# andreaskoepf/faster-rcnn.torch

Measured on AMD Instinct MI355X. Metric: images/sec (vgg_small 800x450 fwd+bwd), higher is better.
Workload: dtype f32 (conv / Linear(13824,1024) operands as 2 x fp16 split planes: 22 significand bits, 3 MFMA partial products; fp32 accumulate)

## Files before the change

faster-rcnn.torch_amd/_lib.py:

```python
import ctypes as C
import os

_HERE = os.path.dirname(os.path.abspath(__file__))
SO_PATH = os.environ.get("FRCNN_LIB_PATH") or os.path.join(_HERE, "libfrcnn_hip.so")

KC_NAMES = ["conv_igemm_k3", "conv_igemm_other", "conv_wgrad_k3", "conv_wgrad_other", "gemm", "elemwise",
            "roi", "rpn", "nms", "optim", "image", "conv_x3", "conv_wgradx", "soft_nms", "topk"]


class FrcnnError(RuntimeError):
    pass


class ModelDesc(C.Structure):
    _fields_ = [
        ("nblocks", C.c_int),
        ("filters", C.c_int * 8), ("ksize", C.c_int * 8), ("pad", C.c_int * 8), ("conv_steps", C.c_int * 8),
        ("dropout", C.c_float * 8),
        ("nheads", C.c_int),
        ("head_k", C.c_int * 8), ("head_n", C.c_int * 8), ("head_input", C.c_int * 8),
        ("ncls", C.c_int),
        ("cls_n", C.c_int * 8), ("cls_bn", C.c_int * 8),
        ("cls_dropout", C.c_float * 8),
        ("class_count", C.c_int),
        ("kh", C.c_int), ("kw", C.c_int),
    ]


vp = C.c_void_p
_SIGS = {
    "frcnn_version": ([], C.c_int),
    "frcnn_set_option": ([C.c_char_p, C.c_int], C.c_int),
    "frcnn_get_option": ([C.c_char_p, C.POINTER(C.c_int)], C.c_int),
    "frcnn_last_error": ([], C.c_char_p),
    "frcnn_device_count": ([C.POINTER(C.c_int)], C.c_int),
    "frcnn_set_device": ([C.c_int], C.c_int),
    "frcnn_device_name": ([C.c_char_p, C.c_int], C.c_int),
    "frcnn_malloc": ([C.POINTER(vp), C.c_size_t], C.c_int),
    "frcnn_free": ([vp], C.c_int),
    "frcnn_host_alloc": ([C.POINTER(vp), C.c_size_t], C.c_int),
    "frcnn_host_free": ([vp], C.c_int),
    "frcnn_memcpy_h2d": ([vp, vp, C.c_size_t, vp], C.c_int),
    "frcnn_memcpy_d2h": ([vp, vp, C.c_size_t, vp], C.c_int),
    "frcnn_memcpy_d2d": ([vp, vp, C.c_size_t, vp], C.c_int),
    "frcnn_stream_sync": ([vp], C.c_int),
    "frcnn_zero": ([vp, C.c_size_t, vp], C.c_int),
    "frcnn_scale": ([vp, C.c_longlong, C.c_float, vp], C.c_int),
    "frcnn_add": ([vp, vp, C.c_longlong, vp], C.c_int),
    "frcnn_prof_enable": ([C.c_int], C.c_int),
    "frcnn_prof_collect": ([vp, vp, vp, vp], C.c_int),
    "frcnn_nms_workspace_bytes": ([C.c_int], C.c_size_t),
    "frcnn_nms_device": ([vp, C.c_int, C.c_int, C.c_float, C.c_int, C.c_int, vp, vp, vp, C.c_size_t, vp], C.c_int),
    "frcnn_nms_device_classes": ([vp, C.c_int, C.c_int, C.c_float, C.c_int, C.c_int, vp, vp, vp, vp, C.c_size_t, vp], C.c_int),
    "frcnn_nms_device_n": ([vp, C.c_int, vp, C.c_int, C.c_float, C.c_int, C.c_int, vp, vp, vp, vp, C.c_size_t, vp], C.c_int),
    "frcnn_nms_batch_workspace_bytes": ([C.c_int, C.c_int], C.c_size_t),
    "frcnn_nms_device_batch": ([vp, C.c_int, C.c_longlong, C.c_int, vp, C.c_int, C.c_float, C.c_int, C.c_int, vp, vp, vp, vp, C.c_size_t,
                               vp], C.c_int),
    "frcnn_soft_nms_workspace_bytes": ([C.c_int, C.c_int], C.c_size_t),
    "frcnn_soft_nms_batch": ([vp, C.c_int, C.c_longlong, C.c_int, vp, C.c_int, C.c_int, C.c_int, C.c_float, C.c_float, C.c_float, C.c_int,
                             vp, vp, vp, vp, C.c_longlong, vp, C.c_size_t, vp], C.c_int),
    "frcnn_box_vote_batch": ([vp, C.c_int, C.c_longlong, C.c_int, vp, C.c_int, C.c_int, C.c_int, C.c_float, vp, vp, vp, vp, vp, vp, vp],
                             C.c_int),
    "frcnn_topk_select_workspace_bytes": ([C.c_int, C.c_int], C.c_size_t),
    "frcnn_topk_select": ([vp, C.c_int, C.c_longlong, C.c_int, vp, C.c_int, vp, C.c_longlong, vp, vp, C.c_size_t, vp], C.c_int),
    "frcnn_rpn_gather_rows": ([vp, vp, vp, vp, C.c_int, C.c_longlong, C.c_int, vp, C.c_longlong, vp, C.c_int, vp, vp, vp, vp, vp, vp,
                              C.c_longlong, vp], C.c_int),
    "frcnn_detect_gather_batch": ([vp, vp, C.c_int, C.c_int, vp, vp, vp, vp, vp, C.c_longlong, vp, vp, vp, vp, vp], C.c_int),
    "frcnn_roi_windows": ([vp, vp, C.c_int, vp, C.c_int, C.c_int, C.c_int, vp, vp], C.c_int),
    "frcnn_detect_post": ([vp, vp, vp, vp, vp, C.c_int, C.c_int, C.c_double, vp, vp, vp, vp, vp, vp], C.c_int),
    "frcnn_detect_classes_batch": ([vp, vp, vp, vp, C.c_int, vp, vp, C.c_longlong, C.c_int, C.c_int, C.c_double, C.c_int, vp, vp, vp, vp,
                                    C.c_int, vp, vp, vp], C.c_int),
    "frcnn_detect_merge_views": ([vp, vp, vp, vp, C.c_longlong, vp, vp, C.c_longlong, C.c_int, C.c_int, vp, vp, vp, vp, vp, vp, vp, vp, vp,
                                  vp, vp, vp], C.c_int),
    "frcnn_nms_host": ([vp, C.c_int, C.c_int, C.c_float, C.c_int, C.c_int, vp, vp], C.c_int),
    "frcnn_conv2d_forward": ([vp, C.c_int, C.c_int, C.c_int, vp, vp, vp, vp, C.c_int, C.c_int, C.c_int, vp, vp], C.c_int),
    "frcnn_conv2d_backward_input": ([vp, C.c_int, C.c_int, C.c_int, vp, C.c_int, C.c_int, C.c_int, vp, C.c_int, vp], C.c_int),
    "frcnn_conv2d_backward_weight": ([vp, C.c_int, C.c_int, C.c_int, vp, vp, vp, C.c_int, C.c_int, C.c_int, vp, vp, vp], C.c_int),
    "frcnn_maxpool_act_forward": ([vp, C.c_int, C.c_int, C.c_int, vp, vp, vp, vp, vp], C.c_int),
    "frcnn_maxpool_act_backward": ([vp, vp, vp, C.c_int, C.c_int, C.c_int, vp, vp, vp, vp, vp, vp], C.c_int),
    "frcnn_act_forward": ([vp, C.c_int, C.c_longlong, vp, vp, vp, vp], C.c_int),
    "frcnn_act_backward": ([vp, vp, C.c_int, C.c_longlong, vp, vp, vp, vp, vp, vp], C.c_int),
    "frcnn_amax_record_floats": ([], C.c_int),
    "frcnn_tensor_absmax": ([vp, C.c_longlong, vp, vp], C.c_int),
    "frcnn_maxpool_act_forward_rec": ([vp, C.c_int, C.c_int, C.c_int, vp, vp, vp, vp, vp, vp], C.c_int),
    "frcnn_maxpool_act_backward_rec": ([vp, vp, vp, C.c_int, C.c_int, C.c_int, vp, vp, vp, vp, vp, vp, vp], C.c_int),
    "frcnn_act_backward_rec": ([vp, vp, C.c_int, C.c_longlong, vp, vp, vp, vp, vp, vp, vp], C.c_int),
    "frcnn_conv2d_forward_rec": ([vp, C.c_int, C.c_int, C.c_int, vp, vp, vp, vp, C.c_int, C.c_int, C.c_int, vp, vp, vp, vp], C.c_int),
    "frcnn_conv2d_backward_input_rec": ([vp, C.c_int, C.c_int, C.c_int, vp, C.c_int, C.c_int, C.c_int, vp, C.c_int, vp, vp, vp, vp, vp, vp,
                                         vp], C.c_int),
    "frcnn_roi_pool_forward": ([vp, C.c_int, C.c_int, C.c_int, vp, C.c_int, C.c_int, C.c_int, vp, vp, vp], C.c_int),
    "frcnn_roi_pool_backward": ([vp, C.c_int, C.c_int, C.c_int, vp, vp, C.c_int, C.c_int, C.c_int, vp], C.c_int),
    "frcnn_roi_align_forward": ([vp, C.c_int, C.c_int, C.c_int, vp, vp, C.c_int, C.c_double, C.c_double, C.c_int, C.c_int, C.c_int, vp,
                                 vp], C.c_int),
    "frcnn_roi_align_backward": ([vp, C.c_int, C.c_int, C.c_int, vp, vp, vp, C.c_int, C.c_double, C.c_double, C.c_int, C.c_int, C.c_int,
                                  vp], C.c_int),
    "frcnn_rpn_scan_workspace_bytes": ([vp, vp], C.c_size_t),
    "frcnn_rpn_scan": ([vp, vp, vp, vp, vp, C.c_double, C.c_double, C.c_double, C.c_int, vp, vp, vp, vp, vp, vp, C.c_size_t, vp], C.c_int),
    "frcnn_rpn_scan_batch_workspace_bytes": ([vp, vp, C.c_int], C.c_size_t),
    "frcnn_rpn_scan_batch": ([vp, vp, vp, C.c_int, C.c_longlong, vp, vp, C.c_double, C.c_double, C.c_double, C.c_int, vp, vp, vp, vp, vp,
                             vp, C.c_size_t, vp], C.c_int),
    "frcnn_rpn_scan_ragged_workspace_bytes": ([vp, vp, C.c_int], C.c_size_t),
    "frcnn_rpn_scan_ragged": ([vp, vp, vp, vp, vp, C.c_int, vp, vp, C.c_double, C.c_int, vp, vp, vp, vp, vp, vp, C.c_size_t, vp],
                              C.c_int),
    "frcnn_rpn_loss": ([vp, vp, vp, vp, vp, vp, vp, vp, C.c_int, C.c_int, C.c_int, vp, vp, vp, vp], C.c_int),
    "frcnn_loss_accumulate": ([vp, C.c_int, vp, vp], C.c_int),
    "frcnn_linear_forward": ([vp, C.c_int, C.c_int, vp, vp, C.c_int, vp, vp], C.c_int),
    "frcnn_linear_backward": ([vp, vp, C.c_int, C.c_int, vp, C.c_int, vp, vp, vp, vp], C.c_int),
    "frcnn_rmsprop": ([vp, vp, vp, C.c_longlong, C.c_float, C.c_float, C.c_float, vp], C.c_int),
    "frcnn_scale_rmsprop": ([vp, vp, C.c_float, vp, C.c_longlong, C.c_float, C.c_float, C.c_float, vp], C.c_int),
    "frcnn_scale_rmsprop_dev": ([vp, vp, vp, vp, C.c_longlong, C.c_float, C.c_float, C.c_float, vp], C.c_int),
    "frcnn_scale_rmsprop_slice": ([vp, vp, C.c_float, vp, C.c_longlong, C.c_longlong, C.c_float, C.c_float, C.c_float, vp], C.c_int),
    "frcnn_sgd": ([vp, vp, vp, C.c_longlong, C.c_float, vp, C.c_float, C.c_float, C.c_float, C.c_float, C.c_int, C.c_int, vp], C.c_int),
    "frcnn_sgd_slice": ([vp, vp, vp, C.c_longlong, C.c_longlong, C.c_float, C.c_float, C.c_float, C.c_float, C.c_float, C.c_int, C.c_int,
                         vp], C.c_int),
    "frcnn_nag": ([vp, vp, vp, C.c_longlong, C.c_float, vp, C.c_float, C.c_float, C.c_float, C.c_int, vp], C.c_int),
    "frcnn_nag_slice": ([vp, vp, vp, C.c_longlong, C.c_longlong, C.c_float, C.c_float, C.c_float, C.c_float, C.c_int, vp], C.c_int),
    "frcnn_scale_rmsprop_slice_dev": ([vp, vp, vp, vp, C.c_longlong, C.c_longlong, C.c_float, C.c_float, C.c_float, vp], C.c_int),
    "frcnn_sgd_slice_dev": ([vp, vp, vp, C.c_longlong, C.c_longlong, vp, C.c_float, C.c_float, C.c_float, C.c_float, C.c_int, C.c_int,
                            vp], C.c_int),
    "frcnn_nag_slice_dev": ([vp, vp, vp, C.c_longlong, C.c_longlong, vp, C.c_float, C.c_float, C.c_float, C.c_int, vp], C.c_int),
    "frcnn_grad_clip_workspace_bytes": ([C.c_longlong], C.c_size_t),
    "frcnn_grad_clip": ([vp, C.c_longlong, vp, C.c_int, C.c_double, vp, C.c_double, vp, vp, C.c_size_t, vp], C.c_int),
    "frcnn_nag_lookahead": ([vp, vp, C.c_longlong, C.c_float, vp], C.c_int),
    "frcnn_nag_lookahead_slice": ([vp, vp, C.c_longlong, C.c_longlong, C.c_float, vp], C.c_int),
    "frcnn_model_update_stream": ([vp, C.POINTER(vp)], C.c_int),
    "frcnn_model_update_fork": ([vp, vp], C.c_int),
    "frcnn_model_update_join": ([vp, vp], C.c_int),
    "frcnn_pnet_wait_backward_begun": ([vp, vp], C.c_int),
    "frcnn_pnet_wait_heads_done": ([vp, vp], C.c_int),
    "frcnn_pnet_wait_block_done": ([vp, C.c_int, vp], C.c_int),
    "frcnn_pnet_refresh_packs": ([vp, vp, C.c_int, vp], C.c_int),
    "frcnn_pnet_invalidate_packs": ([vp], C.c_int),
    "frcnn_model_create": ([C.POINTER(ModelDesc), C.POINTER(vp)], C.c_int),
    "frcnn_model_destroy": ([vp], C.c_int),
    "frcnn_model_param_count": ([vp, C.POINTER(C.c_longlong), C.POINTER(C.c_longlong)], C.c_int),
    "frcnn_model_param_table": ([vp, vp, C.c_int, C.POINTER(C.c_int)], C.c_int),
    "frcnn_model_localizer_layers": ([vp, C.c_int, vp, C.c_int, C.POINTER(C.c_int)], C.c_int),
    "frcnn_model_set_trainable": ([vp, C.c_int, C.c_int, C.c_int], C.c_int),
    "frcnn_model_get_trainable": ([vp, C.POINTER(C.c_int), C.POINTER(C.c_int), C.POINTER(C.c_int)], C.c_int),
    "frcnn_model_debug_buffer": ([vp, C.c_int, C.c_int, C.POINTER(vp), C.POINTER(C.c_longlong)], C.c_int),
    "frcnn_pnet_forward": ([vp, vp, vp, C.c_int, C.c_int, C.c_int, vp, C.c_ulonglong, vp], C.c_int),
    "frcnn_pnet_forward_async_heads": ([vp, vp, vp, C.c_int, C.c_int, vp, C.c_ulonglong, vp], C.c_int),
    "frcnn_pnet_output": ([vp, C.c_int, C.POINTER(vp), C.POINTER(C.c_int), C.POINTER(C.c_int), C.POINTER(C.c_int)], C.c_int),
    "frcnn_pnet_delta": ([vp, C.c_int, C.POINTER(vp)], C.c_int),
    "frcnn_pnet_set_sparse_deltas": ([vp, C.c_int, vp, C.c_int], C.c_int),
    "frcnn_pnet_zero_deltas": ([vp, vp], C.c_int),
    "frcnn_pnet_backward_heads_begin": ([vp, vp, vp, vp], C.c_int),
    "frcnn_pnet_anchor_loss_begin": ([vp, vp, vp, vp, vp, vp, vp, C.c_int, C.c_int, C.c_int, vp, vp, vp, vp, vp], C.c_int),
    "frcnn_pnet_anchor_loss_wait": ([vp, vp], C.c_int),
    "frcnn_pnet_backward_heads_join": ([vp, vp, C.POINTER(C.c_int)], C.c_int),
    "frcnn_pnet_backward": ([vp, vp, vp, vp], C.c_int),
    "frcnn_pnet_wait_block_gradients": ([vp, C.c_int, vp], C.c_int),
    "frcnn_cnet_forward": ([vp, vp, vp, C.c_int, C.c_int, vp, C.c_ulonglong, vp, vp, vp, vp], C.c_int),
    "frcnn_cnet_backward": ([vp, vp, vp, vp, vp, vp, vp], C.c_int),
    "frcnn_cnet_backward_join": ([vp, vp], C.c_int),
    "frcnn_cnet_losses": ([vp, vp, vp, vp, C.c_int, C.c_int, C.c_int, vp, vp, vp, vp], C.c_int),
    "frcnn_cnet_decode": ([vp, C.c_int, C.c_int, vp, vp, vp], C.c_int),
    "frcnn_anchors_create": ([vp, vp, vp, vp, C.c_int, C.c_int, C.POINTER(vp)], C.c_int),
    "frcnn_anchors_destroy": ([vp], C.c_int),
    "frcnn_anchors_assemble": ([vp, vp, C.c_int, C.c_double, C.c_double, C.c_double, C.c_double, C.c_int, C.c_int, C.c_int, vp,
                               C.POINTER(C.c_int), vp, vp, C.c_int, C.POINTER(C.c_int), C.POINTER(C.c_int)], C.c_int),
    "frcnn_comm_get_unique_id": ([vp], C.c_int),
    "frcnn_comm_exchange_id_file": ([C.c_char_p, C.c_int, vp, C.c_int], C.c_int),
    "frcnn_comm_init_rank": ([C.POINTER(vp), C.c_int, C.c_int, vp], C.c_int),
    "frcnn_comm_init_rank_timeout": ([C.POINTER(vp), C.c_int, C.c_int, vp, C.c_int], C.c_int),
    "frcnn_comm_init_rank_file": ([C.POINTER(vp), C.c_int, C.c_int, C.c_char_p, C.c_int], C.c_int),
    "frcnn_comm_destroy": ([vp], C.c_int),
    "frcnn_comm_info": ([vp, C.POINTER(C.c_int), C.POINTER(C.c_int)], C.c_int),
    "frcnn_comm_query": ([vp, C.POINTER(C.c_int), C.POINTER(C.c_int), C.POINTER(C.c_int)], C.c_int),
    "frcnn_allreduce_f32": ([vp, vp, C.c_longlong, vp], C.c_int),
    "frcnn_allreduce_f64": ([vp, vp, C.c_longlong, vp], C.c_int),
    "frcnn_broadcast_f32": ([vp, vp, C.c_longlong, C.c_int, vp], C.c_int),
    "frcnn_image_rgb2yuv": ([vp, vp, C.c_int, C.c_int, vp], C.c_int),
# ... 46 lines not shown
```

faster-rcnn.torch_amd/csrc/amax.h:

```cpp
#pragma once
#include <hip/hip_runtime.h>

#include "kernels.h"

namespace frcnn {

__device__ __forceinline__ void amax_store_block(float m, float* rec) {
  __shared__ float amax_part[16];
#pragma unroll
  for (int o = 32; o > 0; o >>= 1) m = fmaxf(m, __shfl_xor(m, o));
  if ((threadIdx.x & 63) == 0) amax_part[threadIdx.x >> 6] = m;
  __syncthreads();
  if (threadIdx.x == 0) {
    const int nw = (blockDim.x + 63) >> 6;
    for (int i = 1; i < nw; ++i) m = fmaxf(m, amax_part[i]);
    rec[1 + blockIdx.x] = m;
    if (blockIdx.x == 0) rec[0] = __builtin_bit_cast(float, (int)gridDim.x);
  }
}

__device__ __forceinline__ float amax_load_block(const float* __restrict__ rec) {
  __shared__ float amax_all[16];
  const int n = __builtin_bit_cast(int, rec[0]);
  float m = 0.f;
  for (int i = threadIdx.x; i < n; i += blockDim.x) m = fmaxf(m, rec[1 + i]);
#pragma unroll
  for (int o = 32; o > 0; o >>= 1) m = fmaxf(m, __shfl_xor(m, o));
  if ((threadIdx.x & 63) == 0) amax_all[threadIdx.x >> 6] = m;
  __syncthreads();
  const int nw = (blockDim.x + 63) >> 6;
  m = amax_all[0];
  for (int i = 1; i < nw; ++i) m = fmaxf(m, amax_all[i]);
  __syncthreads();
  return m;
}

}
```

faster-rcnn.torch_amd/csrc/api.cpp:

```cpp
#include <cmath>
#include <cstring>
#include <vector>
#include <mutex>

#include "kernels.h"

namespace frcnn {

static thread_local std::string g_err;

void set_error(const char* fmt, ...) {
  char buf[1024];
  va_list ap;
  va_start(ap, fmt);
  vsnprintf(buf, sizeof(buf), fmt, ap);
  va_end(ap);
  g_err = buf;
}

struct ProfRec { int klass; double flops, bytes; hipEvent_t a, b; hipStream_t s; };
static hipEvent_t g_prof_base = nullptr;
static unsigned g_prof_mask = 0;
static std::vector<ProfRec> g_recs;
static std::vector<hipEvent_t> g_pool;
// ... 297 lines not shown
  return tensor_absmax(x, (long)n, rec, S(stream));
}
int frcnn_conv2d_forward_rec(const float* in, int C, int H, int W, const float* in_slope, const float* in_scale, const float* weight,
                             const float* bias, int O, int k, int pad, float* out, const float* rec_in, float* rec_out, void* stream) {
  FR_CHECK(in && weight && out, "frcnn_conv2d_forward_rec: NULL argument");
  FR_CHECK(conv_x3_eligible(C, O, k) && (k == 3 || (!in_slope && !in_scale)),
           "frcnn_conv2d_forward_rec: %d channels -> %d filters, %dx%d does not take the split form", C, O, k, k);
  FR_CHECK(get_x3_f16(), "frcnn_conv2d_forward_rec: option x3_f16 is off");
  bool unit = true;
  FR_TRY(scale_fits_f16_form(in_scale, C, S(stream), &unit));
  FR_CHECK(unit, "frcnn_conv2d_forward_rec: an entry of in_scale exceeds 1: the launch would not take the fp16 form");
  return conv2d_split(in, C, H, W, in_slope, in_scale, weight, bias, O, C, O, k, 0, pad, out, OUT_STORE, true, rec_in, rec_out, nullptr,
                      S(stream));
}
int frcnn_conv2d_backward_input_rec(const float* gout, int O, int Ho, int Wo, const float* weight, int C, int k, int pad, float* gin,
                                    int accumulate, const float* rec_g, float* rec_out, const float* post_x, const float* post_slope,
                                    const float* post_scale, float* gslope, void* stream) {
  FR_CHECK(gout && weight && gin, "frcnn_conv2d_backward_input_rec: NULL argument");
  FR_CHECK(conv_x3_eligible(O, C, k), "frcnn_conv2d_backward_input_rec: %d filters -> %d channels, %dx%d does not take the split form",
           O, C, k, k);
  FR_CHECK(get_x3_f16(), "frcnn_conv2d_backward_input_rec: option x3_f16 is off");
  FR_CHECK(post_x || (!post_slope && !post_scale && !gslope), "frcnn_conv2d_backward_input_rec: a fused activation backward needs post_x");
  FR_CHECK(!post_x || (post_slope && k == 3 && !accumulate),
           "frcnn_conv2d_backward_input_rec: the fused activation backward belongs to a storing 3x3 launch with a slope");
  const X3PostAct post{post_x, post_slope, post_scale, gslope};
  return conv2d_split(gout, O, Ho, Wo, nullptr, nullptr, weight, nullptr, O, C, C, k, 1, k - 1 - pad, gin, accumulate ? OUT_ADD : OUT_STORE,
                      true, rec_g, rec_out, post_x ? &post : nullptr, S(stream));
}
int frcnn_conv2d_backward_weight(const float* in, int C, int H, int W, const float* in_slope,
                                 const float* in_scale, const float* gout, int O, int k, int pad,
                                 float* gweight, float* gbias, void* stream) {
  size_t wsb = conv_wgrad_workspace_bytes(C, H, W, O, k, pad);
  void* ws = nullptr;
  FR_HIP(hipMalloc(&ws, wsb));
  int rc = FRCNN_OK;
  float* am = nullptr;
  bool unit = true;
  rc = scale_fits_f16_form(in_scale, C, S(stream), &unit);
  if (rc == FRCNN_OK && unit && k == 3 && conv_wgradx_eligible(C, O, k)) rc = x3_f16_records(&am);
  if (am && rc == FRCNN_OK) {
    rc = tensor_absmax(in, (long)C * H * W, am, S(stream));
    if (rc == FRCNN_OK) rc = tensor_absmax(gout, (long)O * (H + 2 * pad - k + 1) * (W + 2 * pad - k + 1), am + AMAX_REC, S(stream));
  }
  if (rc == FRCNN_OK)
    rc = conv_wgrad(in, C, H, W, in_slope, in_scale, gout, O, k, pad, gweight, ws, wsb, S(stream), gbias, am, am ? am + AMAX_REC : nullptr);
  (void)hipStreamSynchronize(S(stream));
  (void)hipFree(ws); (void)hipFree(am);
  return rc;
}

int frcnn_maxpool_act_forward(const float* x, int C, int H, int W, const float* slope, const float* scale,
                              float* out, unsigned char* idx, void* stream) {
  return maxpool_act_forward(x, C, H, W, slope, scale, out, idx, S(stream));
}
int frcnn_maxpool_act_backward(const float* gpool, const unsigned char* idx, const float* x, int C, int H, int W,
                               const float* slope, const float* scale, float* gx, float* gbias, float* gslope,
                               void* stream) {
  return maxpool_act_backward(gpool, idx, x, C, H, W, slope, scale, gx, gbias, gslope, S(stream));
}
int frcnn_maxpool_act_forward_rec(const float* x, int C, int H, int W, const float* slope, const float* scale, float* out,
                                  unsigned char* idx, void* stream, float* rec) {
  return maxpool_act_forward(x, C, H, W, slope, scale, out, idx, S(stream), rec);
}
int frcnn_maxpool_act_backward_rec(const float* gpool, const unsigned char* idx, const float* x, int C, int H, int W, const float* slope,
                                   const float* scale, float* gx, float* gbias, float* gslope, void* stream, float* rec) {
  return maxpool_act_backward(gpool, idx, x, C, H, W, slope, scale, gx, gbias, gslope, S(stream), rec);
}
int frcnn_act_backward_rec(const float* gy, const float* x, int C, long long hw, const float* slope, const float* scale, float* gx,
                           float* gbias, float* gslope, void* stream, float* rec) {
  return act_backward(gy, x, C, hw, slope, scale, gx, gbias, gslope, S(stream), rec);
}
int frcnn_act_forward(const float* x, int C, long long hw, const float* slope, const float* scale, float* y,
                      void* stream) {
  return act_forward(x, C, hw, slope, scale, y, S(stream));
}
int frcnn_act_backward(const float* gy, const float* x, int C, long long hw, const float* slope,
                       const float* scale, float* gx, float* gbias, float* gslope, void* stream) {
  return act_backward(gy, x, C, hw, slope, scale, gx, gbias, gslope, S(stream));
}

int frcnn_roi_pool_forward(const float* fmap, int C, int H, int W, const int* wins, int R, int kh, int kw,
                           float* out, int* idx, void* stream) {
  return roi_pool_forward(fmap, C, H, W, wins, R, kh, kw, out, idx, S(stream));
}
int frcnn_roi_pool_backward(float* gmap, int C, int H, int W, const float* gout, const int* idx, int R, int kh,
                            int kw, void* stream) {
  return roi_pool_backward(gmap, C, H, W, gout, idx, R, kh, kw, S(stream));
}

static int roi_align_check(const char* who, const void* map, int C, int H, int W, const void* rows, const double* rect, int kh, int kw,
                           int g) {
  FR_CHECK(map && rows && rect, "%s: NULL argument", who);
  FR_CHECK(C >= 1 && H >= 1 && W >= 1 && kh >= 1 && kw >= 1, "%s: map %d x %d x %d, grid %d x %d", who, C, H, W, kh, kw);
  FR_CHECK((long)H * W < (1L << 31), "%s: a plane of %d x %d cells", who, H, W);
  FR_CHECK(g >= 1 && g <= 4, "%s: sampling ratio %d outside 1..4", who, g);
  return FRCNN_OK;
}
int frcnn_roi_align_forward(const float* fmap, int C, int H, int W, const double* rect, const long long* pick, int R, double inv_sx,
                            double inv_sy, int kh, int kw, int g, float* out, void* stream) {
  if (R <= 0) return FRCNN_OK;
  FR_TRY(roi_align_check("frcnn_roi_align_forward", fmap, C, H, W, out, rect, kh, kw, g));
  return roi_align_forward(fmap, C, H, W, rect, pick, R, inv_sx, inv_sy, kh, kw, g, out, S(stream));
}
int frcnn_roi_align_backward(float* gmap, int C, int H, int W, const float* gout, const double* rect, const long long* pick, int R,
                             double inv_sx, double inv_sy, int kh, int kw, int g, void* stream) {
  if (R <= 0) return FRCNN_OK;
  FR_TRY(roi_align_check("frcnn_roi_align_backward", gmap, C, H, W, gout, rect, kh, kw, g));
  return roi_align_backward(gmap, C, H, W, gout, rect, pick, R, inv_sx, inv_sy, kh, kw, g, S(stream));
}

static void to_layers(const float* const* maps, const int* H, const int* W, RpnLayers* L) {
  for (int l = 0; l < 4; ++l) { L->map[l] = maps ? maps[l] : nullptr; L->H[l] = H[l]; L->W[l] = W[l]; }
}
size_t frcnn_rpn_scan_workspace_bytes(const int* H, const int* W) {
  RpnLayers L;
  to_layers(nullptr, H, W, &L);
  return rpn_scan_workspace_bytes(L);
}
int frcnn_rpn_scan(const float* const* maps, const int* H, const int* W, const float* anchor_w,
                   const float* anchor_h, double img_w, double img_h, double p_threshold, int cap,
                   float* match_p, int* match_idx, double* match_rect, float* match_box, int* count,
                   void* ws, size_t ws_bytes, void* stream) {
  RpnLayers L;
  to_layers(maps, H, W, &L);
  return rpn_scan(L, anchor_w, anchor_h, img_w, img_h, p_threshold, cap, match_p, match_idx, match_rect,
                  match_box, count, ws, ws_bytes, S(stream));
}
size_t frcnn_rpn_scan_batch_workspace_bytes(const int* H, const int* W, int B) {
  RpnLayers L;
  to_layers(nullptr, H, W, &L);
  return rpn_scan_batch_workspace_bytes(L, B);
}
int frcnn_rpn_scan_batch(const float* const* maps, const int* H, const int* W, int B, long long slot_stride, const float* anchor_w,
                         const float* anchor_h, double img_w, double img_h, double p_threshold, int cap, float* match_p,
                         int* match_idx, double* match_rect, float* match_box, int* count, void* ws, size_t ws_bytes,
                         void* stream) {
  FR_CHECK(maps && H && W, "frcnn_rpn_scan_batch: NULL argument");
  RpnLayers L;
  to_layers(maps, H, W, &L);
  return rpn_scan_batch(L, B, (long)slot_stride, anchor_w, anchor_h, img_w, img_h, p_threshold, cap, match_p, match_idx,
                        match_rect, match_box, count, ws, ws_bytes, S(stream));
}
size_t frcnn_rpn_scan_ragged_workspace_bytes(const int* Hs, const int* Ws, int B) {
  return rpn_scan_ragged_workspace_bytes(Hs, Ws, B);
}
int frcnn_rpn_scan_ragged(const float* heads, const long long* map_off, const int* Hs, const int* Ws, const double* img_wh, int B,
                          const float* anchor_w, const float* anchor_h, double p_threshold, int cap, float* match_p,
                          int* match_idx, double* match_rect, float* match_box, int* count, void* ws, size_t ws_bytes,
                          void* stream) {
  return rpn_scan_ragged(heads, map_off, Hs, Ws, img_wh, B, anchor_w, anchor_h, p_threshold, cap, match_p, match_idx, match_rect,
                         match_box, count, ws, ws_bytes, S(stream));
}
int frcnn_rpn_loss(const float* const* maps, float* const* deltas, const int* H, const int* W, const int* ex_idx,
                   const double* ex_anchor, const double* ex_roi, const int* ex_class, int npos, int nneg,
                   int bgclass, double* ex_loss, float* crtarget, float* cctarget, void* stream) {
  RpnLayers L;
  to_layers(maps, H, W, &L);
  return rpn_loss(L, deltas, ex_idx, ex_anchor, ex_roi, ex_class, npos, nneg, bgclass, ex_loss, crtarget,
                  cctarget, S(stream));
}

int frcnn_loss_accumulate(const double* ex_loss, int E, double* acc, void* stream) {
  return loss_accumulate(ex_loss, E, acc, S(stream));
}

int frcnn_linear_forward(const float* x, int R, int I, const float* weight, const float* bias, int O, float* y,
// ... 175 lines not shown
```

faster-rcnn.torch_amd/csrc/cnet.hip:

```cpp
#include "kernels.h"

namespace frcnn {

#define BN_EPS 1e-5
#define BN_MOM 0.1

#define BN_CB 16
#define BN_RG 64
template <int CB = BN_CB, int RG = BN_RG>
__device__ __forceinline__ double bn_reduce(double v, double* sh, int tx, int ty) {
  sh[ty * CB + tx] = v;
  __syncthreads();
  for (int stride = RG / 2; stride > 0; stride >>= 1) {
    if (ty < stride) sh[ty * CB + tx] += sh[(ty + stride) * CB + tx];
    __syncthreads();
  }
  const double s = sh[tx];
  __syncthreads();
  return s;
}
template <int NV>
__device__ __forceinline__ void fb_reduce(double (&v)[NV], double* sh, int tx, int ty) {
  const int tid = ty * 4 + tx, lane = tid & 63, wave = tid >> 6;
#pragma unroll
  for (int k = 0; k < NV; ++k) {
#pragma unroll
    for (int o = 4; o < 64; o <<= 1) v[k] += __shfl_xor(v[k], o, 64);
    if (lane < 4) sh[(k * 16 + wave) * 4 + lane] = v[k];
  }
  __syncthreads();
#pragma unroll
  for (int k = 0; k < NV; ++k) {
    double t = 0.0;
#pragma unroll
    for (int w = 0; w < 16; ++w) t += sh[(k * 16 + w) * 4 + tx];
    v[k] = t;
  }
  __syncthreads();
}
#define FB_CB 4
#define FB_RG 256
#define FB_KEEP 4

__global__ __launch_bounds__(1024) void bn_forward_kernel(const float* __restrict__ x, int R, int n,
                                                          const float* __restrict__ gamma, const float* __restrict__ beta,
                                                          float* running, int training, float* __restrict__ xhat,
                                                          float* __restrict__ invstd, float* __restrict__ y) {
  __shared__ double sh[BN_RG * BN_CB];
  const int tx = threadIdx.x, ty = threadIdx.y;
  const int j = blockIdx.x * BN_CB + tx;
  const bool ok = j < n;
  double mean, var;
  if (training) {
    double s = 0.0;
    if (ok) for (int r = ty; r < R; r += BN_RG) s += x[(size_t)r * n + j];
    mean = bn_reduce(s, sh, tx, ty) / R;
    double q = 0.0;
    if (ok) for (int r = ty; r < R; r += BN_RG) { double d = x[(size_t)r * n + j] - mean; q += d * d; }
    var = bn_reduce(q, sh, tx, ty);
    const double unb = R > 1 ? var / (R - 1) : var / R;
    var /= R;
    if (running && ok && ty == 0) {
      running[j] = (float)((1.0 - BN_MOM) * running[j] + BN_MOM * mean);
      running[n + j] = (float)((1.0 - BN_MOM) * running[n + j] + BN_MOM * unb);
    }
  } else {
    mean = ok ? running[j] : 0.0;
    var = ok ? running[n + j] : 1.0;
  }
  if (!ok) return;
  const double is = 1.0 / sqrt(var + BN_EPS);
  if (ty == 0) invstd[j] = (float)is;
  const double g = gamma[j], b = beta[j];
  for (int r = ty; r < R; r += BN_RG) {
    const double xh = (x[(size_t)r * n + j] - mean) * is;
    xhat[(size_t)r * n + j] = (float)xh;
    y[(size_t)r * n + j] = (float)(xh * g + b);
  }
}
int bn_forward(const float* x, int R, int n, const float* gamma, const float* beta, float* running,
               int training, float* xhat, float* invstd, float* y, hipStream_t s) {
  FR_CHECK(training || running, "bn_forward: evaluate mode needs running statistics");
  FR_LAUNCH(KC_ELEMWISE, 0, (double)R * n * 16.0, s, bn_forward_kernel, dim3(cdiv(n, BN_CB)), dim3(BN_CB, BN_RG), 0, x, R, n,
            gamma, beta, running, training, xhat, invstd, y);
  FR_LAUNCH_CHECK();
  return FRCNN_OK;
}

__global__ __launch_bounds__(1024) void bn_backward_kernel(const float* __restrict__ gy, const float* __restrict__ xhat,
                                                           const float* __restrict__ invstd, const float* __restrict__ gamma,
                                                           int R, int n, int training, float* __restrict__ gx, float* ggamma,
                                                           float* gbeta) {
  __shared__ double sh[BN_RG * BN_CB];
  const int tx = threadIdx.x, ty = threadIdx.y;
  const int j = blockIdx.x * BN_CB + tx;
  const bool ok = j < n;
  double sg = 0.0, sgx = 0.0;
  if (ok)
    for (int r = ty; r < R; r += BN_RG) {
      const double g = gy[(size_t)r * n + j];
      sg += g;
      sgx += g * xhat[(size_t)r * n + j];
    }
  sg = bn_reduce(sg, sh, tx, ty);
  sgx = bn_reduce(sgx, sh, tx, ty);
  if (!ok) return;
  if (ty == 0) {
    ggamma[j] = (float)((double)ggamma[j] + sgx);
    gbeta[j] = (float)((double)gbeta[j] + sg);
  }
  const double is = invstd[j], gm = gamma[j];
  for (int r = ty; r < R; r += BN_RG) {
    const double g = gy[(size_t)r * n + j];
    const double xh = xhat[(size_t)r * n + j];
    const double v = training ? (g - sg / R - xh * sgx / R) * gm * is : g * gm * is;
    gx[(size_t)r * n + j] = (float)v;
  }
}
int bn_backward(const float* gy, const float* xhat, const float* invstd, const float* gamma, int R,
                int n, int training, float* gx, float* ggamma, float* gbeta, hipStream_t s) {
  FR_LAUNCH(KC_ELEMWISE, 0, (double)R * n * 16.0, s, bn_backward_kernel, dim3(cdiv(n, BN_CB)), dim3(BN_CB, BN_RG), 0, gy,
            xhat, invstd, gamma, R, n, training, gx, ggamma, gbeta);
  FR_LAUNCH_CHECK();
  return FRCNN_OK;
}

__device__ __forceinline__ float fold_value(const float* __restrict__ x, const GemmFold& src, size_t total, size_t idx, int j) {
  if (src.nSplit == 0) return x[idx];
  float v = src.bias ? src.bias[j] : 0.f;
  for (int sI = 0; sI < src.nSplit; ++sI) v += src.slab[(size_t)sI * total + idx];
  return v;
}

template <bool GEN>
__global__ __launch_bounds__(1024) void cnet_act_forward_kernel(const float* __restrict__ x, GemmFold src, int R, int n,
                                                                const float* __restrict__ gamma, const float* __restrict__ beta,
                                                                float* running, int training, float* __restrict__ lin,
                                                                float* __restrict__ xhat, float* __restrict__ invstd,
                                                                float* __restrict__ pre, const float* slope, float* __restrict__ mask,
                                                                float inv_keep, float p, unsigned long long seed,
                                                                float* __restrict__ post) {
  __shared__ double sh[FB_RG * FB_CB];
  const int tx = threadIdx.x, ty = threadIdx.y;
  const int j = blockIdx.x * FB_CB + tx;
  const bool ok = j < n;
  const size_t total = (size_t)R * n;
  const bool bn = gamma != nullptr;
  const float* v = src.nSplit ? lin : x;
  const bool keep = R <= FB_RG * FB_KEEP;
  float xv[FB_KEEP];
  double s0 = 0.0;
  if (ok) {
#pragma unroll
    for (int i = 0; i < FB_KEEP; ++i) {
      const int r = ty + i * FB_RG;
      xv[i] = 0.f;
      if (keep && r < R) {
        const size_t idx = (size_t)r * n + j;
        xv[i] = fold_value(x, src, total, idx, j);
        if (src.nSplit) lin[idx] = xv[i];
        s0 += xv[i];
      }
    }
    if (!keep && (src.nSplit || (bn && training)))
      for (int r = ty; r < R; r += FB_RG) {
        const size_t idx = (size_t)r * n + j;
        const float t = fold_value(x, src, total, idx, j);
        if (src.nSplit) lin[idx] = t;
        s0 += t;
      }
  }
  double mean = 0.0, is = 1.0, g = 1.0, b = 0.0;
  if (bn) {
    double var;
    if (training) {
      { double t[1] = {s0}; fb_reduce(t, sh, tx, ty); mean = t[0] / R; }
      double q = 0.0;
      if (ok && keep) {
#pragma unroll
        for (int i = 0; i < FB_KEEP; ++i)
          if (ty + i * FB_RG < R) { double d = xv[i] - mean; q += d * d; }
      } else if (ok) {
        for (int r = ty; r < R; r += FB_RG) { double d = v[(size_t)r * n + j] - mean; q += d * d; }
      }
      { double t[1] = {q}; fb_reduce(t, sh, tx, ty); var = t[0]; }
      const double unb = R > 1 ? var / (R - 1) : var / R;
      var /= R;
      if (running && ok && ty == 0) {
        running[j] = (float)((1.0 - BN_MOM) * running[j] + BN_MOM * mean);
        running[n + j] = (float)((1.0 - BN_MOM) * running[n + j] + BN_MOM * unb);
      }
    } else {
      mean = ok ? running[j] : 0.0;
      var = ok ? running[n + j] : 1.0;
    }
    if (!ok) return;
    is = 1.0 / sqrt(var + BN_EPS);
    if (ty == 0) invstd[j] = (float)is;
    g = gamma[j]; b = beta[j];
  }
  if (!ok) return;
  const float a = *slope;
  auto emit = [&](size_t idx, float y) {
    if (bn) {
      const double xh = ((double)y - mean) * is;
      xhat[idx] = (float)xh;
      y = (float)(xh * g + b);
      pre[idx] = y;
    }
    y = y > 0.f ? y : a * y;
    if (GEN) {
      const float mk = frcnn_keep_mask(seed, (unsigned long long)idx, p);
      mask[idx] = mk;
      y = y * (mk * inv_keep);
    } else if (mask) {
      y = y * (mask[idx] * inv_keep);
    }
    post[idx] = y;
  };
  if (keep) {
#pragma unroll
    for (int i = 0; i < FB_KEEP; ++i)
      if (ty + i * FB_RG < R) emit((size_t)(ty + i * FB_RG) * n + j, xv[i]);
  } else {
    for (int r = ty; r < R; r += FB_RG) emit((size_t)r * n + j, v[(size_t)r * n + j]);
  }
}
template <bool GEN>
__global__ void cnet_act_forward_flat_kernel(const float* __restrict__ x, GemmFold src, long total, int n, float* __restrict__ lin,
                                             const float* slope, float* __restrict__ mask, float inv_keep, float p,
                                             unsigned long long seed, float* __restrict__ post) {
  const float a = *slope;
  for (long i = (long)blockIdx.x * blockDim.x + threadIdx.x; i < total; i += (long)gridDim.x * blockDim.x) {
    float y = fold_value(x, src, (size_t)total, (size_t)i, (int)(i % n));
    if (src.nSplit) lin[i] = y;
    y = y > 0.f ? y : a * y;
    if (GEN) {
      const float mk = frcnn_keep_mask(seed, (unsigned long long)i, p);
      mask[i] = mk;
      y = y * (mk * inv_keep);
    } else if (mask) {
      y = y * (mask[i] * inv_keep);
    }
    post[i] = y;
  }
}
int cnet_act_forward(const float* x, GemmFold src, int R, int n, const float* gamma, const float* beta, float* running,
                     int training, float* lin, float* xhat, float* invstd, float* pre, const float* slope, float* mask, bool gen,
                     float inv_keep, float p, unsigned long long seed, float* post, hipStream_t s) {
  FR_CHECK(!gamma || training || running, "cnet_act_forward: evaluate mode needs running statistics");
  if (!gamma) {
    const long total = (long)R * n;
    const int grid = (int)std::min<long>(std::max<long>(1, cdivl(total, 256)), 2048);
    if (gen)
      FR_LAUNCH(KC_ELEMWISE, 0, total * 16.0, s, cnet_act_forward_flat_kernel<true>, dim3(grid), dim3(256), 0, x, src, total, n, lin, slope,
                mask, inv_keep, p, seed, post);
    else
      FR_LAUNCH(KC_ELEMWISE, 0, total * 16.0, s, cnet_act_forward_flat_kernel<false>, dim3(grid), dim3(256), 0, x, src, total, n, lin, slope,
                mask, inv_keep, p, seed, post);
    FR_LAUNCH_CHECK();
    return FRCNN_OK;
  }
  if (gen)
    FR_LAUNCH(KC_ELEMWISE, 0, (double)R * n * 20.0, s, cnet_act_forward_kernel<true>, dim3(cdiv(n, FB_CB)), dim3(FB_CB, FB_RG), 0, x,
              src, R, n, gamma, beta, running, training, lin, xhat, invstd, pre, slope, mask, inv_keep, p, seed, post);
  else
    FR_LAUNCH(KC_ELEMWISE, 0, (double)R * n * 20.0, s, cnet_act_forward_kernel<false>, dim3(cdiv(n, FB_CB)), dim3(FB_CB, FB_RG), 0, x,
              src, R, n, gamma, beta, running, training, lin, xhat, invstd, pre, slope, mask, inv_keep, p, seed, post);
  FR_LAUNCH_CHECK();
  return FRCNN_OK;
}

__global__ __launch_bounds__(1024) void cnet_act_bn_backward_kernel(const float* __restrict__ gy, GemmFold src,
                                                                    const float* __restrict__ pre, const float* __restrict__ xhat,
                                                                    const float* __restrict__ invstd, const float* __restrict__ gamma,
                                                                    const float* slope, const float* __restrict__ mask, float inv_keep,
                                                                    int R, int n, int training, float* __restrict__ gx, float* ggamma,
                                                                    float* gbeta, float* gslope, float* part) {
  __shared__ double sh[FB_RG * FB_CB];
  __shared__ float shs[16];
  const int tx = threadIdx.x, ty = threadIdx.y;
  const int j = blockIdx.x * FB_CB + tx;
  const bool ok = j < n;
  const size_t total = (size_t)R * n;
  const float a = *slope;
  double sg = 0.0, sgx = 0.0;
  float sa = 0.f;
  const bool keep = R <= FB_RG * FB_KEEP;
  float tv[FB_KEEP], xh[FB_KEEP];
  auto first = [&](size_t idx, float& t, float& xhv) {
    float g = fold_value(gy, src, total, idx, j);
    if (mask) g = g * (mask[idx] * inv_keep);
    const float xv = pre[idx];
    t = g;
    if (!(xv > 0.f)) { t = a * g; sa += xv * g; }
    xhv = xhat[idx];
    sg += t;
    sgx += (double)t * xhv;
  };
  if (ok && keep) {
#pragma unroll
    for (int i = 0; i < FB_KEEP; ++i) {
      tv[i] = 0.f; xh[i] = 0.f;
      if (ty + i * FB_RG < R) first((size_t)(ty + i * FB_RG) * n + j, tv[i], xh[i]);
    }
  } else if (ok) {
    for (int r = ty; r < R; r += FB_RG) {
      const size_t idx = (size_t)r * n + j;
      float t, xhv;
      first(idx, t, xhv);
      gx[idx] = t;
    }
  }
  { double t[2] = {sg, sgx}; fb_reduce(t, sh, tx, ty); sg = t[0]; sgx = t[1]; }
  {
    const int tid = ty * FB_CB + tx;
#pragma unroll
    for (int o = 32; o > 0; o >>= 1) sa += __shfl_down(sa, o, 64);
    if ((tid & 63) == 0) shs[tid >> 6] = sa;
    __syncthreads();
    if (tid == 0) {
      float t = 0.f;
      for (int i = 0; i < 16; ++i) t += shs[i];
      if (part) part[blockIdx.x] = t; else unsafeAtomicAdd(gslope, t);
    }
  }
  if (!ok) return;
  if (ty == 0) {
    ggamma[j] = (float)((double)ggamma[j] + sgx);
    gbeta[j] = (float)((double)gbeta[j] + sg);
  }
  const double is = invstd[j], gm = gamma[j];
  auto second = [&](size_t idx, double g, double xhv) {
    const double v = training ? (g - sg / R - xhv * sgx / R) * gm * is : g * gm * is;
    gx[idx] = (float)v;
  };
  if (keep) {
#pragma unroll
    for (int i = 0; i < FB_KEEP; ++i)
      if (ty + i * FB_RG < R) second((size_t)(ty + i * FB_RG) * n + j, tv[i], xh[i]);
  } else {
    for (int r = ty; r < R; r += FB_RG) {
      const size_t idx = (size_t)r * n + j;
      second(idx, gx[idx], xhat[idx]);
    }
  }
}
__global__ void slope_fold_kernel(const float* __restrict__ part, int n, float* gslope);
int cnet_act_bn_backward(const float* gy, GemmFold src, const float* pre, const float* xhat, const float* invstd,
                         const float* gamma, const float* slope, const float* mask, float inv_keep, int R, int n, int training,
                         float* gx, float* ggamma, float* gbeta, float* gslope, hipStream_t s) {
  const int grid = cdiv(n, FB_CB);
  float* part = nullptr;
  if (deterministic()) FR_TRY(det_workspace(s, (size_t)grid, &part));
  FR_LAUNCH(KC_ELEMWISE, 0, (double)R * n * 28.0, s, cnet_act_bn_backward_kernel, dim3(grid), dim3(FB_CB, FB_RG), 0, gy, src, pre, xhat,
            invstd, gamma, slope, mask, inv_keep, R, n, training, gx, ggamma, gbeta, gslope, part);
  if (part) FR_LAUNCH(KC_ELEMWISE, 0, grid * 4.0, s, slope_fold_kernel, dim3(1), dim3(1), 0, (const float*)part, grid, gslope);
  FR_LAUNCH_CHECK();
  return FRCNN_OK;
}

template <bool GEN>
__global__ void prelu_dropout_forward_kernel(const float* __restrict__ x, long n, const float* slope,
                                             float* __restrict__ mask, float inv_keep, float p,
                                             unsigned long long seed, float* __restrict__ y) {
  const float a = *slope;
  for (long i = (long)blockIdx.x * blockDim.x + threadIdx.x; i < n; i += (long)gridDim.x * blockDim.x) {
    float v = x[i];
    v = v > 0.f ? v : a * v;
    if (GEN) {
      const float mk = frcnn_keep_mask(seed, (unsigned long long)i, p);
      mask[i] = mk;
      v = v * (mk * inv_keep);
    } else if (mask) {
      v = v * (mask[i] * inv_keep);
    }
    y[i] = v;
  }
}
int prelu_dropout_forward(const float* x, long n, const float* slope, const float* mask, float inv_keep,
                          float* y, hipStream_t s) {
  int grid = (int)std::min<long>(std::max<long>(1, cdivl(n, 256)), 1024);
  FR_LAUNCH(KC_ELEMWISE, 0, n * 12.0, s, prelu_dropout_forward_kernel<false>, dim3(grid), dim3(256), 0, x, n, slope,
            const_cast<float*>(mask), inv_keep, 0.f, 0ull, y);
  FR_LAUNCH_CHECK();
  return FRCNN_OK;
}
int prelu_dropout_forward_gen(const float* x, long n, const float* slope, float* mask_out, float p,
                              unsigned long long seed, float* y, hipStream_t s) {
  int grid = (int)std::min<long>(std::max<long>(1, cdivl(n, 256)), 1024);
  FR_LAUNCH(KC_ELEMWISE, 0, n * 12.0, s, prelu_dropout_forward_kernel<true>, dim3(grid), dim3(256), 0, x, n, slope,
            mask_out, 1.0f / (1.0f - p), p, seed, y);
  FR_LAUNCH_CHECK();
  return FRCNN_OK;
}

__global__ void prelu_dropout_backward_kernel(const float* __restrict__ gy, const float* __restrict__ x, long n,
                                              const float* slope, const float* __restrict__ mask,
                                              float inv_keep, float* __restrict__ gx, float* gslope, float* part) {
  __shared__ float sh[4];
  const float a = *slope;
  float sa = 0.f;
  for (long i = (long)blockIdx.x * blockDim.x + threadIdx.x; i < n; i += (long)gridDim.x * blockDim.x) {
    float g = gy[i];
    if (mask) g = g * (mask[i] * inv_keep);
    const float xv = x[i];
    float r = g;
    if (!(xv > 0.f)) { r = a * g; sa += xv * g; }
    gx[i] = r;
  }
#pragma unroll
  for (int o = 32; o > 0; o >>= 1) sa += __shfl_down(sa, o, 64);
  if ((threadIdx.x & 63) == 0) sh[threadIdx.x >> 6] = sa;
  __syncthreads();
  if (threadIdx.x == 0) {
    const float t = sh[0] + sh[1] + sh[2] + sh[3];
    if (part) part[blockIdx.x] = t;
    else unsafeAtomicAdd(gslope, t);
  }
}
__global__ void slope_fold_kernel(const float* __restrict__ part, int n, float* gslope) {
  float v = 0.f;
  for (int i = 0; i < n; ++i) v += part[i];
  *gslope += v;
}
int prelu_dropout_backward(const float* gy, const float* x, long n, const float* slope,
                           const float* mask, float inv_keep, float* gx, float* gslope, hipStream_t s) {
  int grid = (int)std::min<long>(std::max<long>(1, cdivl(n, 256)), 256);
  float* part = nullptr;
  if (deterministic()) FR_TRY(det_workspace(s, (size_t)grid, &part));
  FR_LAUNCH(KC_ELEMWISE, 0, n * 16.0, s, prelu_dropout_backward_kernel, dim3(grid), dim3(256), 0, gy, x, n,
            slope, mask, inv_keep, gx, gslope, part);
  if (part) FR_LAUNCH(KC_ELEMWISE, 0, grid * 4.0, s, slope_fold_kernel, dim3(1), dim3(1), 0, (const float*)part, grid, gslope);
  FR_LAUNCH_CHECK();
  return FRCNN_OK;
}

__device__ __forceinline__ double wave_sum_f64(double v) {
#pragma unroll
  for (int o = 32; o > 0; o >>= 1) v += __shfl_xor(v, o, 64);
  return v;
}
__device__ __forceinline__ double wave_max_f64(double v) {
#pragma unroll
  for (int o = 32; o > 0; o >>= 1) { const double w = __shfl_xor(v, o, 64); v = w > v ? w : v; }
  return v;
}
__global__ void log_softmax_rows_fold_kernel(float* __restrict__ x, GemmFold src, int R, int n, float* __restrict__ y,
                                             float* __restrict__ y2) {
  const int r = blockIdx.x * (blockDim.x >> 6) + (threadIdx.x >> 6), lane = threadIdx.x & 63;
  if (r >= R) return;
  float* xr = x + (size_t)r * n;
  const size_t total = (size_t)R * n;
  if (src.nSplit)
    for (int i = lane; i < n; i += 64) xr[i] = fold_value(x, src, total, (size_t)r * n + i, i);
  double m = -1.0e300;
  for (int i = lane; i < n; i += 64) m = xr[i] > m ? (double)xr[i] : m;
  m = wave_max_f64(m);
  double s = 0.0;
  for (int i = lane; i < n; i += 64) s += exp((double)xr[i] - m);
  s = wave_sum_f64(s);
  const double lse = m + log(s);
  for (int i = lane; i < n; i += 64) {
    const float v = (float)((double)xr[i] - lse);
    y[(size_t)r * n + i] = v;
    if (y2) y2[(size_t)r * n + i] = v;
  }
}
int log_softmax_rows_fold(const float* x, GemmFold src, int R, int n, float* y, float* y2, hipStream_t s) {
  if (R <= 0) return FRCNN_OK;
  FR_LAUNCH(KC_ELEMWISE, 0, (double)R * n * 8.0, s, log_softmax_rows_fold_kernel, dim3(cdiv(R, 4)), dim3(256), 0, const_cast<float*>(x),
            src, R, n, y, y2);
  FR_LAUNCH_CHECK();
  return FRCNN_OK;
}

__global__ void log_softmax_rows_kernel(const float* __restrict__ x, int R, int n, float* __restrict__ y) {
  const int r = blockIdx.x * (blockDim.x >> 6) + (threadIdx.x >> 6), lane = threadIdx.x & 63;
  if (r >= R) return;
  const float* xr = x + (size_t)r * n;
  double m = -1.0e300;
  for (int i = lane; i < n; i += 64) m = xr[i] > m ? (double)xr[i] : m;
  m = wave_max_f64(m);
  double s = 0.0;
  for (int i = lane; i < n; i += 64) s += exp((double)xr[i] - m);
  s = wave_sum_f64(s);
  const double lse = m + log(s);
  for (int i = lane; i < n; i += 64) y[(size_t)r * n + i] = (float)((double)xr[i] - lse);
}
int log_softmax_rows(const float* x, int R, int n, float* y, hipStream_t s) {
  if (R <= 0) return FRCNN_OK;
  FR_LAUNCH(KC_ELEMWISE, 0, (double)R * n * 8.0, s, log_softmax_rows_kernel, dim3(cdiv(R, 4)), dim3(256), 0, x, R,
            n, y);
  FR_LAUNCH_CHECK();
  return FRCNN_OK;
}

#define HEADS_PITCH 33
__global__ __launch_bounds__(256) void cnet_heads_forward_kernel(const float* __restrict__ x, int R, int nf, const float* __restrict__ Wb,
                                                                 const float* __restrict__ bb, const float* __restrict__ Wc,
                                                                 const float* __restrict__ bc, int nc, float* __restrict__ bbox_out,
                                                                 float* __restrict__ logits, float* __restrict__ lsm,
                                                                 float* __restrict__ cls_out) {
  extern __shared__ float wt[];
  float* xs = wt + (size_t)nf * HEADS_PITCH + (threadIdx.x >> 6) * nf;
  const int no = 4 + nc;
  for (int k = threadIdx.x; k < nf; k += 256) {
    float* d = wt + k * HEADS_PITCH;
#pragma unroll
    for (int n = 0; n < 4; ++n) d[n] = Wb[(size_t)n * nf + k];
#pragma unroll 8
    for (int n = 0; n < nc; ++n) d[4 + n] = Wc[(size_t)n * nf + k];
  }
  __syncthreads();
  const int lane = threadIdx.x & 63, n = lane & 31, h = lane >> 5;
  const bool isb = n < 4, isc = n >= 4 && n < no;
  const int nn = n < no ? n : 0, kh = nf / 2;
  for (int r = blockIdx.x * 4 + (threadIdx.x >> 6); r < R; r += gridDim.x * 4) {
    for (int k = lane * 4; k < nf; k += 256) *reinterpret_cast<float4*>(xs + k) = *reinterpret_cast<const float4*>(x + (size_t)r * nf + k);
    __builtin_amdgcn_wave_barrier();
    const float* xr = xs + h * kh;
    const float* wk = wt + (size_t)(h * kh) * HEADS_PITCH + nn;
    float a0 = 0.f, a1 = 0.f, a2 = 0.f, a3 = 0.f;
#pragma unroll 4
    for (int k = 0; k < kh; k += 4) {
      const float4 xv = *reinterpret_cast<const float4*>(xr + k);
      a0 = fmaf(xv.x, wk[(k + 0) * HEADS_PITCH], a0); a1 = fmaf(xv.y, wk[(k + 1) * HEADS_PITCH], a1);
      a2 = fmaf(xv.z, wk[(k + 2) * HEADS_PITCH], a2); a3 = fmaf(xv.w, wk[(k + 3) * HEADS_PITCH], a3);
    }
    float v = (a0 + a1) + (a2 + a3);
    v += __shfl_xor(v, 32, 64);
    v += isb ? bb[n] : isc ? bc[n - 4] : 0.f;
    if (isb && h == 0) bbox_out[(size_t)r * 4 + n] = v;
    const bool mine = isc && h == 0;
    double m = mine ? (double)v : -1.0e300;
    m = wave_max_f64(m);
    double e = mine ? exp((double)v - m) : 0.0;
    e = wave_sum_f64(e);
    const double lse = m + log(e);
    if (mine) {
      const size_t o = (size_t)r * nc + n - 4;
      const float l = (float)((double)v - lse);
      logits[o] = v; lsm[o] = l;
      if (cls_out) cls_out[o] = l;
    }
  }
}
__global__ __launch_bounds__(256) void cnet_heads_backward_kernel(const float* __restrict__ g_bbox, const float* __restrict__ g_cls,
                                                                  const float* __restrict__ lsm, int R, int nf,
                                                                  const float* __restrict__ Wb, const float* __restrict__ Wc, int nc,
                                                                  float* __restrict__ glog, float* __restrict__ gfeat, HeadsPostAct post) {
  extern __shared__ float wt[];
  __shared__ float shs[4];
  const float pa = post.pre ? *post.slope : 1.f;
  float sa = 0.f;
  const int no = 4 + nc;
  for (int k = threadIdx.x; k < nf; k += 256) {
#pragma unroll
    for (int n = 0; n < 4; ++n) wt[n * nf + k] = Wb[(size_t)n * nf + k];
#pragma unroll 8
    for (int n = 0; n < nc; ++n) wt[(4 + n) * nf + k] = Wc[(size_t)n * nf + k];
  }
  __syncthreads();
  const int lane = threadIdx.x & 63, wave = threadIdx.x >> 6;
  float* sg = wt + (size_t)no * nf + wave * 64;
  const bool isb = lane < 4, isc = lane >= 4 && lane < no;
  for (int r = blockIdx.x * 4 + wave; r < R; r += gridDim.x * 4) {
    const size_t o = (size_t)r * nc + (isc ? lane - 4 : 0);
    const double gy = isc ? (double)g_cls[o] : 0.0;
    const double sum = wave_sum_f64(gy);
    float g = 0.f;
    if (isc) {
      g = (float)(gy - exp((double)lsm[o]) * sum);
      glog[o] = g;
    } else if (isb) {
      g = g_bbox[(size_t)r * 4 + lane];
    }
    sg[lane] = g;
    __builtin_amdgcn_wave_barrier();
    for (int k = lane; k < nf; k += 64) {
      float a0 = 0.f, a1 = 0.f;
      int n = 0;
      for (; n + 2 <= no; n += 2) {
        a0 = fmaf(sg[n], wt[n * nf + k], a0);
        a1 = fmaf(sg[n + 1], wt[(n + 1) * nf + k], a1);
      }
      if (n < no) a0 = fmaf(sg[n], wt[n * nf + k], a0);
      float g = a0 + a1;
      if (post.pre) {
        const size_t idx = (size_t)r * nf + k;
        if (post.mask) g = g * (post.mask[idx] * post.inv_keep);
        const float xv = post.pre[idx];
        if (!(xv > 0.f)) { sa += xv * g; g = pa * g; }
      }
      gfeat[(size_t)r * nf + k] = g;
    }
    __builtin_amdgcn_wave_barrier();
  }
  if (post.pre) {
#pragma unroll
    for (int o = 32; o > 0; o >>= 1) sa += __shfl_down(sa, o, 64);
    if (lane == 0) shs[wave] = sa;
    __syncthreads();
    if (threadIdx.x == 0) unsafeAtomicAdd(post.gslope, (shs[0] + shs[1]) + (shs[2] + shs[3]));
  }
}
bool cnet_heads_fused_eligible(int nf, int nc) { return 4 + nc <= 32 && nf % 8 == 0 && nf <= 1024; }
int cnet_heads_forward(const float* x, int R, int nf, const float* Wb, const float* bb, const float* Wc, const float* bc, int nc,
                       float* bbox_out, float* logits, float* lsm, float* cls_out, hipStream_t s) {
  if (R <= 0) return FRCNN_OK;
  FR_CHECK(cnet_heads_fused_eligible(nf, nc), "cnet_heads_forward: %d classes", nc);
  FR_CHECK(((uintptr_t)x & 15) == 0, "cnet_heads_forward: input alignment");
  const size_t lds = ((size_t)nf * HEADS_PITCH + 4 * (size_t)nf) * 4;
  static bool attr_set = false;
  if (!attr_set) {
    FR_HIP(hipFuncSetAttribute(reinterpret_cast<const void*>(cnet_heads_forward_kernel), hipFuncAttributeMaxDynamicSharedMemorySize, 160 * 1024));
    attr_set = true;
  }
  FR_LAUNCH(KC_ELEMWISE, 0, (double)R * nf * 4.0, s, cnet_heads_forward_kernel, dim3(std::min(cdiv(R, 4), 256)), dim3(256), lds, x, R, nf, Wb,
            bb, Wc, bc, nc, bbox_out, logits, lsm, cls_out);
  FR_LAUNCH_CHECK();
  return FRCNN_OK;
}
int cnet_heads_backward(const float* g_bbox, const float* g_cls, const float* lsm, int R, int nf, const float* Wb, const float* Wc,
                        int nc, float* glog, float* gfeat, hipStream_t s, const HeadsPostAct* post) {
  if (R <= 0) return FRCNN_OK;
  FR_CHECK(cnet_heads_fused_eligible(nf, nc), "cnet_heads_backward: %d classes", nc);
  const size_t lds = ((size_t)(4 + nc) * nf + 256) * 4;
  static size_t attr_lds = 0;
  if (lds > attr_lds) {
    FR_HIP(hipFuncSetAttribute(reinterpret_cast<const void*>(cnet_heads_backward_kernel), hipFuncAttributeMaxDynamicSharedMemorySize, (int)lds));
    attr_lds = lds;
  }
  FR_LAUNCH(KC_ELEMWISE, 0, (double)R * nf * 4.0, s, cnet_heads_backward_kernel, dim3(std::min(cdiv(R, 4), 256)), dim3(256), lds, g_bbox, g_cls,
            lsm, R, nf, Wb, Wc, nc, glog, gfeat, post ? *post : HeadsPostAct{});
  FR_LAUNCH_CHECK();
  return FRCNN_OK;
}

__global__ void log_softmax_backward_kernel(const float* __restrict__ gy, const float* __restrict__ lsm, int R,
                                            int n, float* __restrict__ gx) {
  const int r = blockIdx.x * (blockDim.x >> 6) + (threadIdx.x >> 6), lane = threadIdx.x & 63;
  if (r >= R) return;
  double sum = 0.0;
  for (int i = lane; i < n; i += 64) sum += gy[(size_t)r * n + i];
  sum = wave_sum_f64(sum);
  for (int i = lane; i < n; i += 64)
    gx[(size_t)r * n + i] = (float)((double)gy[(size_t)r * n + i] - exp((double)lsm[(size_t)r * n + i]) * sum);
}
int log_softmax_backward(const float* gy, const float* lsm, int R, int n, float* gx, hipStream_t s) {
  if (R <= 0) return FRCNN_OK;
  FR_LAUNCH(KC_ELEMWISE, 0, (double)R * n * 12.0, s, log_softmax_backward_kernel, dim3(cdiv(R, 4)), dim3(256), 0,
            gy, lsm, R, n, gx);
  FR_LAUNCH_CHECK();
  return FRCNN_OK;
}

__global__ void cnet_losses_kernel(float* __restrict__ crout, const float* __restrict__ crtarget,
                                   const float* __restrict__ ccout, const float* __restrict__ cctarget, int R,
                                   int npos, int ncls, float* __restrict__ crdelta, float* __restrict__ ccdelta,
                                   double* loss2) {
  __shared__ double shr[256], shc[256];
  double sr = 0.0, sc = 0.0;
  for (int i = threadIdx.x; i < R * 4; i += blockDim.x) {
    float v = crout[i];
    if (i >= npos * 4) { v = 0.f; crout[i] = 0.f; }
    const float z = v - crtarget[i];
    const float az = fabsf(z);
    sr += az < 1.0f ? 0.5 * (double)z * (double)z : (double)az - 0.5;
    crdelta[i] = (az < 1.0f ? z : (z > 0.f ? 1.0f : -1.0f)) * 10.0f;
  }
  for (int i = threadIdx.x; i < R * ncls; i += blockDim.x) ccdelta[i] = 0.f;
  __syncthreads();
  for (int r = threadIdx.x; r < R; r += blockDim.x) {
    const int t = (int)cctarget[r] - 1;
    sc -= (double)ccout[(size_t)r * ncls + t];
    ccdelta[(size_t)r * ncls + t] = (float)(-1.0 / R);
  }
  shr[threadIdx.x] = sr;
  shc[threadIdx.x] = sc;
  __syncthreads();
  for (int o = 128; o > 0; o >>= 1) {
    if (threadIdx.x < o) { shr[threadIdx.x] += shr[threadIdx.x + o]; shc[threadIdx.x] += shc[threadIdx.x + o]; }
    __syncthreads();
  }
  if (threadIdx.x == 0) {
    loss2[0] += (double)(float)shr[0] * 10.0;
    loss2[1] += (double)(float)(shc[0] / R);
  }
}
int cnet_losses(float* crout, const float* crtarget, const float* ccout, const float* cctarget, int R,
                int npos, int ncls, float* crdelta, float* ccdelta, double* loss2, hipStream_t s) {
  if (R <= 0) return FRCNN_OK;
  FR_LAUNCH(KC_ELEMWISE, 0, (double)R * (ncls + 8) * 8.0, s, cnet_losses_kernel, dim3(1), dim3(256), 0, crout,
            crtarget, ccout, cctarget, R, npos, ncls, crdelta, ccdelta, loss2);
  FR_LAUNCH_CHECK();
  return FRCNN_OK;
}

__global__ void cnet_decode_kernel(const float* __restrict__ lsm, int R, int ncls, int* __restrict__ cls,
                                   float* __restrict__ conf) {
  const int r = blockIdx.x * blockDim.x + threadIdx.x;
  if (r >= R) return;
  int best = 0;
  for (int j = 1; j < ncls; ++j)
    if (lsm[(size_t)r * ncls + j] > lsm[(size_t)r * ncls + best]) best = j;
  cls[r] = best + 1;
  conf[r] = lsm[(size_t)r * ncls + best];
}
int cnet_decode(const float* cls_lsm, int R, int ncls, int* cls_out, float* conf_out, hipStream_t s) {
  if (R <= 0) return FRCNN_OK;
  FR_LAUNCH(KC_ELEMWISE, 0, (double)R * ncls * 4.0, s, cnet_decode_kernel, dim3(cdiv(R, 64)), dim3(64), 0,
            cls_lsm, R, ncls, cls_out, conf_out);
  FR_LAUNCH_CHECK();
  return FRCNN_OK;
}

}
// ... 1 lines not shown
```

faster-rcnn.torch_amd/csrc/kernels.h:

```cpp
#pragma once
#include <algorithm>

#include "common.h"

namespace frcnn {

int conv_cc(int k);
int conv_mpad(int M);
size_t conv_pack_floats(int Kchan, int M, int k);
int conv_pack_weights(const float* w, int O, int C, int k, float* wf, float* wd, hipStream_t s);
struct PackJob { long w_off; long total; float* dst; int O, C, k, mode, Mpad, blk_begin, nblk; };
PackJob conv_pack_job(long w_off, int O, int C, int k, int mode, float* dst);
int conv_pack_assign_blocks(PackJob* jobs, int njobs, int total_blocks);
int conv_pack_weights_multi(const float* weights, const PackJob* jobs_dev, int njobs, int grid, hipStream_t s);

enum { OUT_STORE = 0, OUT_ADD = 1 };
struct IgemmPool { float* out; unsigned char* idx; const float* slope; const float* scale; float* amax = nullptr; };
int conv_igemm(const float* in, int Cin, int H, int W, const float* in_slope, const float* in_scale,
               const float* wp, const float* bias, int M, int k, int pad, float* out, int out_mode,
               double algo_flops, hipStream_t s, int ws_slot = 0,
               const IgemmPool* pool = nullptr, bool* pool_fused = nullptr);

void set_split_bf16(int on);
int get_split_bf16();
// ... 61 lines not shown
int maxpool_act_forward(const float* x, int C, int H, int W, const float* slope, const float* scale,
                        float* out, unsigned char* idx, hipStream_t s, float* amax = nullptr);
int maxpool_act_backward(const float* gpool, const unsigned char* idx, const float* x, int C, int H,
                         int W, const float* slope, const float* scale, float* gx, float* gbias,
                         float* gslope, hipStream_t s, float* amax = nullptr);
int act_backward(const float* gy, const float* x, int C, long hw, const float* slope,
                 const float* scale, float* gx, float* gbias, float* gslope, hipStream_t s, float* amax = nullptr);
int channel_sum(const float* g, int C, long hw, float* gbias, hipStream_t s);
int channel_sum_cols(const float* g, int R, int O, float* gb, hipStream_t s);
int gather_positions(const float* src, int C, long hw, const int* pos, int P, float* dst, const float* slope,
                     float* dst_act, hipStream_t s);
int im2col_positions(const float* X, int C, int H, int W, int k, int Wo, const int* pos, int P, float* col, hipStream_t s);
int col2im_positions_add(const float* col, int C, int H, int W, int k, int Wo, const int* pos, int P, float* gX,
                         hipStream_t s);
int dropout_channel_mask(float* scale, int C, float p, unsigned long long seed, hipStream_t s);
int fill_value(float* x, long n, float v, hipStream_t s);
int rmsprop_update(float* x, float* g, float* m, long lo, long hi, bool slice, float gscale, const double* gcount_dev, float lr,
                   float alpha, float eps, hipStream_t s);
int sgd_update(float* x, float* g, float* v, long lo, long hi, bool slice, float gscale, const double* gcount_dev, float clr,
               float wd, float mom, float one_minus_damp, bool nesterov, bool first, hipStream_t s);
int nag_update(float* x, float* g, float* v, long lo, long hi, bool slice, float gscale, const double* gcount_dev, float clr,
               float wd, float mom, bool first, hipStream_t s);
int nag_lookahead(float* x, const float* v, long n, float mom, hipStream_t s);
constexpr int GRAD_CLIP_MAX_RANGES = 16;
size_t grad_clip_workspace_bytes(long n);
int grad_clip(float* g, long n, const long long* ranges_host, int nranges, double divisor, const double* divisor_dev, double clip_norm,
              double* record, void* workspace, size_t workspace_bytes, hipStream_t s);
int nag_lookahead_slice(float* x, const float* v, long lo, long hi, float mom, hipStream_t s);

#define FRCNN_HEAD_OUT 18
struct HeadJob {
  int Cin, H, W, k, Ho, Wo, n;
  int P; const int* pos;
  const float* in; float* gin;
  const float *bias3, *slope, *bias1;
  float *gbias3, *gslope, *gbias1;
  float* out; const float* delta;
  float *COL, *HX, *HY, *OUT, *D, *GH, *DX;
  const float* hx_slab; int hx_splits;
};
struct HeadJobs { HeadJob j[4]; int n; };
int heads_im2col(const HeadJobs& g, hipStream_t s);
int heads_bias_act(const HeadJobs& g, hipStream_t s);
int heads_scatter(const HeadJobs& g, hipStream_t s);
int heads_gather_delta(const HeadJobs& g, hipStream_t s);
int heads_act_backward(const HeadJobs& g, hipStream_t s);
int heads_col2im(const HeadJobs& g, hipStream_t s);

struct GemmFold;
#define GEMM_GROUP_MAX 4
struct GemmJob {
  const float* A; long sAm, sAk; const float* B; long sBk, sBn; float* C; long ldc;
  int M, N, K, out_mode;
  int splits = 1;
  int kPerSplit = 0;
};
int gemm_f32_group(GemmJob* jobs, int n, hipStream_t s);
int gemm_f32(const float* A, long sAm, long sAk, const float* B, long sBk, long sBn, float* C,
             long ldc, int M, int N, int K, int out_mode, const float* bias_n, hipStream_t s, int ws_slot = 0,
             GemmFold* defer = nullptr);
int gemm_workspace_get(size_t need, float** out, int slot);
struct GemmFold {
  const float* slab = nullptr;
  int nSplit = 0;
  const float* bias = nullptr;
};
int gemm_reduce_slabs(const float* slab, int nSplit, int M, int N, const float* bias, float* C, long ldc, bool accumulate,
                      hipStream_t s);
void set_gemm_x_roles(int mask);
int get_gemm_x_roles();
bool linear_x_eligible(int role, int R, int I, int O);
int linear_x_rows_padded(int R);
int split_planes(const float* src, int R, int C, void* P , void* PT ,
                 hipStream_t s, const float* amax = nullptr);
int linear_x_forward(const void* Xp, int R, int I, const float* W, const float* bias, int O, float* y, hipStream_t s, int ws_slot = 0,
                     GemmFold* defer = nullptr, const float* amax_x = nullptr, const float* amax_w = nullptr);
int linear_x_dgrad(const void* Gp, int R, int O, const float* W, int I, float* gx, int out_mode, hipStream_t s, int ws_slot = 0,
                   GemmFold* defer = nullptr, const float* amax_g = nullptr, const float* amax_w = nullptr);
int linear_x_wgrad(const void* GpT, const void* XpT, int R, int O, int I, float* gw, hipStream_t s, int ws_slot = 0,
                   const float* amax_g = nullptr, const float* amax_x = nullptr);


int roi_pool_forward(const float* fmap, int C, int H, int W, const int* wins, int R, int kh, int kw,
                     float* out, int* idx, hipStream_t s);
int roi_pool_backward(float* gmap, int C, int H, int W, const float* gout, const int* idx, int R,
                      int kh, int kw, hipStream_t s);

int roi_align_forward(const float* fmap, int C, int H, int W, const double* rect, const long long* pick, int R, double inv_sx,
                      double inv_sy, int kh, int kw, int g, float* out, hipStream_t s);
int roi_align_backward(float* gmap, int C, int H, int W, const float* gout, const double* rect, const long long* pick, int R,
                       double inv_sx, double inv_sy, int kh, int kw, int g, hipStream_t s);

struct RpnLayers {
  const float* map[4];
  int H[4], W[4];
};
int rpn_scan_batch(const RpnLayers& L, int B, long slot_stride, const float* anchor_w, const float* anchor_h, double img_w,
                   double img_h, double p_threshold, int cap, float* match_p, int* match_idx, double* match_rect,
                   float* match_box, int* count, void* ws, size_t ws_bytes, hipStream_t s);
size_t rpn_scan_batch_workspace_bytes(const RpnLayers& L, int B);
int rpn_scan(const RpnLayers& L, const float* anchor_w, const float* anchor_h, double img_w,
             double img_h, double p_threshold, int cap, float* match_p, int* match_idx,
             double* match_rect, float* match_box, int* count, void* ws, size_t ws_bytes,
             hipStream_t s);
size_t rpn_scan_workspace_bytes(const RpnLayers& L);
int rpn_scan_ragged(const float* heads, const long long* map_off, const int* Hs, const int* Ws, const double* img_wh, int B,
                    const float* anchor_w, const float* anchor_h, double p_threshold, int cap, float* match_p, int* match_idx,
                    double* match_rect, float* match_box, int* count, void* ws, size_t ws_bytes, hipStream_t s);
size_t rpn_scan_ragged_workspace_bytes(const int* Hs, const int* Ws, int B);
int rpn_loss(const RpnLayers& L, float* const* delta, const int* ex_idx, const double* ex_anchor,
             const double* ex_roi, const int* ex_class, int npos, int nneg, int bgclass,
             double* ex_loss, float* crtarget, float* cctarget, hipStream_t s);

int loss_accumulate(const double* ex_loss, int E, double* acc, hipStream_t s);

size_t nms_batch_workspace_bytes(int B, int n);
int nms_device_batch(const float* boxes, int B, long row_stride, int n, const int* n_dev, int ncols, float overlap, int key_mode,
                     int key_col, const int* cls, long long* pick, int* count, void* ws, size_t ws_bytes, hipStream_t s);
size_t nms_workspace_bytes(int n);
int nms_device(const float* boxes, int n, int ncols, float overlap, int key_mode, int key_col,
               long long* pick, int* count, void* ws, size_t ws_bytes, hipStream_t s, const int* cls = nullptr,
               const int* n_dev = nullptr);
size_t soft_nms_workspace_bytes(int B, int n_cap);
int soft_nms_batch(const float* boxes, int B, long row_stride, int n_cap, const int* n_dev, int ncols, int score_col, int method,
                   float overlap, float sigma, float min_score, int log_domain, const int* cls, long long* pick, int* count,
                   float* score_out, long score_stride, void* ws, size_t ws_bytes, hipStream_t s);
int box_vote_batch(const float* boxes, int B, long row_stride, int n_cap, const int* n_dev, int ncols, int score_col,
                   int weight_mode, float overlap, const int* cls, const double* rect, const long long* pick, const int* count,
                   double* rect_out, int* votes_out, hipStream_t s);
size_t topk_select_workspace_bytes(int B, int n_cap);
int topk_select(const float* score, int B, long stride, int n_cap, const int* n_dev, int K, int* sel_row, long sel_stride,
                int* k_dev, void* ws, size_t ws_bytes, hipStream_t s);
int rpn_gather_rows(const float* p, const int* idx, const double* rect, const float* box, int B, long src_stride, int src_rows,
                    const int* sel_row, long sel_stride, const int* k_dev, int k_cap, float* dst_p, int* dst_idx,
                    double* dst_rect, float* dst_box, float* box5, int* row, long dst_stride, hipStream_t s);
int roi_windows(const double* rect, const long long* pick, int k, const int* layers, int nlayers, int fmH, int fmW, int* wins,
                hipStream_t s);
int detect_post(const int* cls, const float* conf, const float* bbox, const double* rect, const long long* pick, int R,
                int bgclass, double min_conf, float* bb, int* kc, int* keep_row, double* r2, int* K_dev, hipStream_t s);
int detect_classes_batch(const float* cls_out, const float* bbox, const int* R, const long long* row0, int B, const double* rect,
                         const long long* pick, long long match_stride, int ncls, int bgclass, double min_conf, int mode, float* bb,
                         int* kc, int* keep_row, double* r2, int row_stride, int* K_dev, int* total_dev, hipStream_t s);
int detect_merge_views(const float* bb, const int* kc, const int* keep_row, const double* r2, long long row_stride,
                       const int* counts, const long long* pick, long long match_stride, int F, int V, const int* flip,
                       const double* Wv, const double* ax, const double* ay, const int* R, float* bb_out, int* kc_out,
                       int* keep_row_out, double* r2_out, long long* pick_out, int* counts_out, hipStream_t s);
int detect_gather_batch(const long long* wpick, const int* counts, int B, int row_stride, const int* keep_row, const int* kc,
                        const float* bb, const double* r2, const long long* pick, long match_stride, const float* mp,
                        const double* rect, const int* midx, double* rec, hipStream_t s);

int bn_forward(const float* x, int R, int n, const float* gamma, const float* beta, float* running,
               int training, float* xhat, float* invstd, float* y, hipStream_t s);
int bn_backward(const float* gy, const float* xhat, const float* invstd, const float* gamma, int R,
                int n, int training, float* gx, float* ggamma, float* gbeta, hipStream_t s);
int prelu_dropout_forward(const float* x, long n, const float* slope, const float* mask, float inv_keep,
                          float* y, hipStream_t s);
int prelu_dropout_forward_gen(const float* x, long n, const float* slope, float* mask_out, float p,
                              unsigned long long seed, float* y, hipStream_t s);
int prelu_dropout_backward(const float* gy, const float* x, long n, const float* slope,
                           const float* mask, float inv_keep, float* gx, float* gslope, hipStream_t s);
int cnet_act_forward(const float* x, GemmFold src, int R, int n, const float* gamma, const float* beta, float* running,
                     int training, float* lin, float* xhat, float* invstd, float* pre, const float* slope, float* mask, bool gen,
                     float inv_keep, float p, unsigned long long seed, float* post, hipStream_t s);
int cnet_act_bn_backward(const float* gy, GemmFold src, const float* pre, const float* xhat, const float* invstd,
                         const float* gamma, const float* slope, const float* mask, float inv_keep, int R, int n, int training,
                         float* gx, float* ggamma, float* gbeta, float* gslope, hipStream_t s);
bool cnet_heads_fused_eligible(int nf, int nc);
int cnet_heads_forward(const float* x, int R, int nf, const float* Wb, const float* bb, const float* Wc, const float* bc, int nc,
                       float* bbox_out, float* logits, float* lsm, float* cls_out, hipStream_t s);
struct HeadsPostAct {
  const float* pre = nullptr;
  const float* mask = nullptr;
  float inv_keep = 1.f;
  const float* slope = nullptr;
  float* gslope = nullptr;
};
int cnet_heads_backward(const float* g_bbox, const float* g_cls, const float* lsm, int R, int nf, const float* Wb, const float* Wc,
                        int nc, float* glog, float* gfeat, hipStream_t s, const HeadsPostAct* post = nullptr);
int log_softmax_rows_fold(const float* x, GemmFold src, int R, int n, float* y, float* y2, hipStream_t s);
int dropout_mask(float* mask, long n, float p, unsigned long long seed, hipStream_t s);
struct DropoutJobs { float* ptr[8]; int C[8]; float p[8]; unsigned long long seed[8]; int n; };
int dropout_channel_masks(const DropoutJobs& j, hipStream_t s);
int log_softmax_rows(const float* x, int R, int n, float* y, hipStream_t s);
int cnet_losses(float* crout, const float* crtarget, const float* ccout, const float* cctarget, int R,
                int npos, int ncls, float* crdelta, float* ccdelta, double* loss2, hipStream_t s);
int log_softmax_backward(const float* gy, const float* lsm, int R, int n, float* gx, hipStream_t s);
int cnet_decode(const float* cls_lsm, int R, int ncls, int* cls_out, float* conf_out, hipStream_t s);

int image_rgb2yuv(const float* rgb, float* yuv, int H, int W, hipStream_t s);
int image_rgb2hsv(const float* rgb, float* hsv, int H, int W, hipStream_t s);
int image_rgb2lab(const float* rgb, float* lab, int H, int W, hipStream_t s);
int image_scale(const float* src, int C, int H, int W, float* dst, int dH, int dW, float* tmp, int rgb2yuv,
                hipStream_t s);
int image_scale_u8(const unsigned char* src_hwc, int H, int W, float* dst, int dH, int dW, float* tmp, int rgb2yuv,
                   hipStream_t s);
int image_crop_flip(const float* src, int C, int H, int W, int x0, int y0, int w, int h, int hflip, int vflip,
                    float* dst, hipStream_t s);
size_t image_normalize_workspace_bytes(int C);
int image_normalize(float* img, int C, int H, int W, int centering, int scaling, void* ws, size_t ws_bytes,
                    hipStream_t s);
int image_contrastive_norm(const float* in, int H, int W, const float* kernel_host, int K, float threshold, float* out,
                           float* tmp, hipStream_t s);

}
```

faster-rcnn.torch_amd/csrc/net.cpp:

```cpp
#include <array>
#include <vector>
#include <cmath>
#include <cstring>
#include <mutex>

#include "kernels.h"
#include "own.h"

namespace frcnn {

static const int HEAD_OUT = 18;
static const int SPARSE_MAX_POS = 512;

struct Conv {
  int Cin, Cout, k, pad;
  int H, W, Ho, Wo;
  long w_off, b_off, a_off;
  int block, step;
  DevBuf wf, wd;
  DevBuf wx, wxd;
  bool x_f = false, x_d = false;
  DevBuf x, gx;
  int am = -1;
};

struct Block {
  int first_conv, nconv;
  bool has_drop;
  float p_drop;
  DevBuf scale;
  DevBuf pooled, gpooled;
  DevBuf pidx;
  int Hp, Wp;
  int am = -1;
  bool dc_on = false;
  int nk = 0, nkM = 0, nkK = 0;
  const int* dc_idx = nullptr;
  DevBuf dc_bias;
};

struct Head {
  Conv c3;
  Conv c1;
  int input;
  DevBuf delta;
  const int* sp_pos = nullptr;
  int sp_count = -1;
  DevBuf spD, spHX, spHY, spGH, spCol, spDX;
  DevBuf spOut, spSlab;
  hipStream_t stream = nullptr;
  Event done;
  Event gin_done;
  bool gin_recorded = false;
};

struct ClsLayer {
  int in, n;
  bool bn;
  float p_drop;
  long w_off, b_off, bnw_off, bnb_off, a_off;
  DevBuf lin, pre, post, xhat, invstd, mask, g;
  DevBuf gin;
  DevBuf xp, xpT, gp, gpT;
  int x_form = 0;
  DevBuf am;
  const float* am_w_of = nullptr;
  long am_w_gen = -1;
};

}

using namespace frcnn;

static bool env_flag(const char* name, bool dflt) {
  const char* e = getenv(name);
  return e ? atoi(e) != 0 : dflt;
}

static int g_drop_compact = -1;
static int drop_compact_on() {
  if (g_drop_compact < 0) g_drop_compact = env_flag("FRCNN_DROP_COMPACT", true);
  return g_drop_compact;
}
static int pool_stream(int slot, hipStream_t* out) {
  static hipStream_t pool[8] = {};
  static std::mutex mu;
  std::lock_guard<std::mutex> lock(mu);
  if (!pool[slot]) FR_HIP(hipStreamCreateWithFlags(&pool[slot], hipStreamNonBlocking));
  *out = pool[slot];
  return FRCNN_OK;
}

static int g_sparse_heads = -1;
static int sparse_heads_on() {
  if (g_sparse_heads < 0) g_sparse_heads = env_flag("FRCNN_SPARSE_HEADS", true);
  return g_sparse_heads;
}
static int g_static_weights = 0;
static long g_static_gen = 0;

struct frcnn_model {
  frcnn_model_desc d;
  std::vector<Conv> convs;
  std::vector<Block> blocks;
  std::vector<Head> heads;
  std::vector<ClsLayer> cls;
  long pnet_params = 0, total_params = 0;
  long bbox_w_off = 0, bbox_b_off = 0, clsw_off = 0, clsb_off = 0;
  int H = 0, W = 0;
  int training = 0;
  DevBuf delta_last;
  DevBuf zero_arena;
  size_t delta_bytes = 0, gpool_bytes = 0;
  DevBuf pack_jobs;
  DevBuf x3_jobs;
  DevBuf amax, amax_ws, amax_jobs;
  int n_amax = 0, n_amax_jobs = 0, amax_grid = 0;
  float* rec(int id) const { return (float*)amax.p + (size_t)id * AMAX_REC; }
  std::vector<unsigned char> am_live;
  float* rec_w(int id) { am_live[id] = 1; return rec(id); }
  void weights_live(bool heads_too) {
    for (auto& c : convs) if (c.x_f || c.x_d) am_live[c.am + 2] = 1;
    for (auto& hd : heads) if (heads_too && (hd.c3.x_f || hd.c3.x_d)) am_live[hd.c3.am + 2] = 1;
  }
  bool f16_packed = false;
  long eval_packs_gen = -1;
  const float* eval_packs_w = nullptr;
  int n_x3_all = 0, n_x3_fwd = 0, x3_grid_all = 0, x3_grid_fwd = 0;
  int n_pack_fwd = 0, n_pack_all = 0, n_pack_heads = 0, pack_grid_fwd = 0, pack_grid_all = 0, pack_grid_heads = 0;
  bool head_packs_fresh = false;
  struct PackGroup { int pk_off = 0, pk_n = 0, pk_grid = 0, am_off = 0, am_n = 0, am_grid = 0, x3_off = 0, x3_off16 = 0, x3_n = 0, x3_grid = 0; };
  std::vector<PackGroup> groups;
  unsigned fresh_mask = 0;
  const float* fresh_w = nullptr;
  bool fresh_f16 = false;
  static const int DC_RING = 4;
  PinBuf dc_pin; DevBuf dc_dev; size_t dc_slot_bytes = 0, dc_idx_off = 0; unsigned dc_step = 0;
  Event dc_ev[DC_RING];
  std::vector<PackXJob> x3_host, x3_host16;
  std::vector<int> x3_conv;
  DevBuf dbg_expand;
  std::vector<Event> block_rd_ev;
  hipStream_t side = nullptr;
  hipStream_t cw = nullptr;
  Event cw_done;
  bool cw_pending = false;
  std::vector<Event> cw_ev;
  std::vector<Event> fork_ev;
  Event join_ev;
  bool update_armed = false;
  Event bwd_ev;
  Event upd_ev, upd_join_ev;
  bool head_x3_fresh = true;
  int am_bb_off = 0, am_bb_n = 0, am_bb_grid = 0;
  int pk_bb_off = 0, pk_bb_n = 0, pk_bb_grid = 0;
  bool heads_deferred = false;
  bool heads_sparse_fwd = false;
  const float* last_w = nullptr;
  Event heads_gin_ev;
  bool heads_gin = false;
  bool heads_begun = false;
  bool heads_joined = false;
  bool side_busy = false;
  Event loss_ev;
  Event chain_ev;
  std::vector<Event> block_ev;
  bool block_ev_valid = false;
  bool loss_pending = false;
  DevBuf wg_ws;
  DevBuf wg_ws_first;
  DevBuf img;
  int frozen_blocks = 0;
  int train_heads = 1, train_cnet = 1;
  int R = 0, D = 0;
  const float* cnet_x = nullptr;
  DevBuf feat_g, logits, lsm, glog, gtmp;
  std::vector<std::array<long long, 4>> table;
};

static int pool_out(int n) { return (n - 2 + 1) / 2 + 1; }
static int refresh_group(frcnn_model* m, const float* w, int group, hipStream_t s);

static void build_layout(frcnn_model* m) {
  const frcnn_model_desc& d = m->d;
  long off = 0;
  int cin = 3;
  for (int b = 0; b < d.nblocks; ++b) {
    Block blk;
    blk.first_conv = (int)m->convs.size();
    blk.nconv = d.conv_steps[b];
    blk.has_drop = d.dropout[b] > 0.f;
    blk.p_drop = d.dropout[b];
    for (int s = 0; s < d.conv_steps[b]; ++s) {
      Conv c;
      c.Cin = cin; c.Cout = d.filters[b]; c.k = d.ksize[b]; c.pad = d.pad[b];
      c.block = b; c.step = s;
      long wsz = (long)c.Cout * c.Cin * c.k * c.k;
      c.w_off = off; c.b_off = off + wsz; c.a_off = off + wsz + c.Cout;
      m->table.push_back({c.w_off, wsz, 0, (long long)c.k * c.k * c.Cout});
      m->table.push_back({c.b_off, c.Cout, 1, 0});
      m->table.push_back({c.a_off, 1, 2, 0});
      off += wsz + c.Cout + 1;
      cin = c.Cout;
      m->convs.push_back(std::move(c));
    }
    m->blocks.push_back(std::move(blk));
  }
  for (int h = 0; h < d.nheads; ++h) {
    Head hd;
    hd.input = d.head_input[h] - 1;
    Conv& a = hd.c3;
    a.Cin = d.filters[hd.input]; a.Cout = d.head_n[h]; a.k = d.head_k[h]; a.pad = 0;
    a.block = -1; a.step = 0;
    long wsz = (long)a.Cout * a.Cin * a.k * a.k;
    a.w_off = off; a.b_off = off + wsz; a.a_off = off + wsz + a.Cout;
    m->table.push_back({a.w_off, wsz, 0, (long long)a.k * a.k * a.Cout});
    m->table.push_back({a.b_off, a.Cout, 1, 0});
    m->table.push_back({a.a_off, 1, 2, 0});
    off += wsz + a.Cout + 1;
    Conv& c = hd.c1;
    c.Cin = a.Cout; c.Cout = HEAD_OUT; c.k = 1; c.pad = 0; c.block = -1; c.step = 1;
    long w1 = (long)HEAD_OUT * c.Cin;
    c.w_off = off; c.b_off = off + w1; c.a_off = -1;
    m->table.push_back({c.w_off, w1, 0, (long long)HEAD_OUT});
    m->table.push_back({c.b_off, HEAD_OUT, 1, 0});
    off += w1 + HEAD_OUT;
    m->heads.push_back(std::move(hd));
  }
  m->pnet_params = off;
  int in = d.kh * d.kw * d.filters[d.nblocks - 1];
  m->D = in;
  for (int l = 0; l < d.ncls; ++l) {
    ClsLayer L;
    L.in = in; L.n = d.cls_n[l]; L.bn = d.cls_bn[l] != 0; L.p_drop = d.cls_dropout[l];
    L.w_off = off; L.b_off = off + (long)in * L.n;
    m->table.push_back({L.w_off, (long long)in * L.n, 3, in});
    m->table.push_back({L.b_off, L.n, 4, in});
    off += (long)in * L.n + L.n;
    L.bnw_off = L.bnb_off = -1;
    if (L.bn) {
      L.bnw_off = off; L.bnb_off = off + L.n;
      m->table.push_back({L.bnw_off, L.n, 5, 0});
      m->table.push_back({L.bnb_off, L.n, 6, 0});
      off += 2L * L.n;
    }
    L.a_off = off;
    m->table.push_back({L.a_off, 1, 2, 0});
    off += 1;
    in = L.n;
    m->cls.push_back(std::move(L));
  }
  m->bbox_w_off = off; m->bbox_b_off = off + (long)in * 4;
  m->table.push_back({m->bbox_w_off, (long long)in * 4, 3, in});
  m->table.push_back({m->bbox_b_off, 4, 4, in});
  off += (long)in * 4 + 4;
  int nc = d.class_count + 1;
  m->clsw_off = off; m->clsb_off = off + (long)in * nc;
  m->table.push_back({m->clsw_off, (long long)in * nc, 3, in});
  m->table.push_back({m->clsb_off, nc, 4, in});
  off += (long)in * nc + nc;
  m->total_params = off;
  m->block_ev.resize(m->blocks.size());
  m->block_rd_ev.resize(m->blocks.size());
// ... 700 lines not shown
  FR_CHECK(m->H > 0, "pnet_output: call frcnn_pnet_forward first");
  FR_CHECK(i >= 1 && i <= (int)m->heads.size() + 1, "pnet_output: index %d out of range", i);
  if (i <= (int)m->heads.size()) {
    Head& h = m->heads[i - 1];
    *ptr = h.c1.x.f(); *C = HEAD_OUT; *H = h.c1.Ho; *W = h.c1.Wo;
  } else {
    Block& b = m->blocks.back();
    *ptr = b.pooled.f(); *C = m->d.filters[m->d.nblocks - 1]; *H = b.Hp; *W = b.Wp;
  }
  return FRCNN_OK;
}

int frcnn_model_debug_buffer(frcnn_model* m, int kind, int index, void** ptr, long long* bytes) {
  FR_CHECK(m && ptr && bytes, "frcnn_model_debug_buffer: NULL argument");
  const DevBuf* b = nullptr;
  size_t n = 0;
  switch (kind) {
    case 0: {
      FR_CHECK(index >= 0 && index < (int)m->convs.size() && m->H > 0, "debug_buffer: backbone convolution %d (after a forward pass)", index);
      const Conv& c = m->convs[index]; b = &c.x; n = (size_t)c.Cout * c.Ho * c.Wo * 4;
      const Block& k = m->blocks[c.block];
      if (k.dc_on && c.step == 0) {
        FR_HIP(hipDeviceSynchronize());
        FR_TRY(m->dbg_expand.ensure(n));
        FR_HIP(hipMemset(m->dbg_expand.p, 0, n));
        std::vector<int> idx(c.Cout);
        FR_HIP(hipMemcpy(idx.data(), k.dc_idx, (size_t)c.Cout * 4, hipMemcpyDeviceToHost));
        const size_t row = (size_t)c.Ho * c.Wo * 4;
        for (int i = 0; i < k.nk; ++i)
          FR_HIP(hipMemcpy((char*)m->dbg_expand.p + (size_t)idx[i] * row, (const char*)c.x.p + (size_t)i * row, row, hipMemcpyDeviceToDevice));
        b = &m->dbg_expand;
      }
    } break;
    case 4: {
      FR_CHECK(index >= 0 && index < (int)m->blocks.size() && m->H > 0 && m->blocks[index].has_drop, "debug_buffer: block %d has no dropout", index);
      const Block& k = m->blocks[index]; b = &k.scale; n = (size_t)m->d.filters[index] * 4;
    } break;
    case 1: {
      FR_CHECK(index >= 0 && index < (int)m->blocks.size() && m->H > 0, "debug_buffer: block %d (after a forward pass)", index);
      const Block& k = m->blocks[index]; b = &k.pidx; n = (size_t)m->d.filters[index] * k.Hp * k.Wp;
    } break;
    case 2: {
      FR_CHECK(index >= 0 && index < (int)m->heads.size() && m->H > 0, "debug_buffer: anchor net %d (after a forward pass)", index);
      const Conv& c = m->heads[index].c3; b = &c.x; n = (size_t)c.Cout * c.Ho * c.Wo * 4;
      if ((m->heads_sparse_fwd || m->heads_deferred) && m->last_w) {
        FR_HIP(hipDeviceSynchronize());
        if (!m->head_x3_fresh) { FR_TRY(refresh_group(m, m->last_w, (int)m->blocks.size(), nullptr)); m->head_x3_fresh = true; }
        FR_TRY(head_forward(m, m->heads[index], m->last_w, nullptr, 0));
        FR_HIP(hipDeviceSynchronize());
      }
    } break;
    case 3: {
      FR_CHECK(index >= 0 && index < (int)m->cls.size() && m->R > 0, "debug_buffer: classification layer %d (after frcnn_cnet_forward)", index);
      const ClsLayer& L = m->cls[index]; b = L.bn ? &L.pre : &L.lin; n = (size_t)m->R * L.n * 4;
    } break;
    case 7: case 11: {
      FR_CHECK(index >= 0 && index < (int)m->convs.size() && m->H > 0, "debug_buffer: backbone convolution %d (after a forward pass)", index);
      const Conv& c = m->convs[index];
      const Block& k = m->blocks[c.block];
      b = kind == 7 ? &c.x : &c.gx; n = (size_t)((k.dc_on && c.step == 0) ? k.nkM : c.Cout) * c.Ho * c.Wo * 4;
    } break;
    case 9: {
      FR_CHECK(index >= 0 && index < (int)m->blocks.size() && m->H > 0, "debug_buffer: block %d (after a forward pass)", index);
      const Block& k = m->blocks[index]; b = &k.pooled; n = (size_t)m->d.filters[index] * k.Hp * k.Wp * 4;
    } break;
    case 5: case 6: case 8: case 10: {
      const int nc = (int)m->convs.size();
      int id = -1;
      FR_CHECK(m->H > 0, "debug_buffer: magnitude records exist after a forward pass");
      if (kind == 6) {
        FR_CHECK(index >= 0 && index < (int)m->blocks.size(), "debug_buffer: block %d out of range", index);
        id = m->blocks[index].am;
      } else if (kind == 10) {
        FR_CHECK(index >= 0 && index < nc + (int)m->heads.size(), "debug_buffer: weight tensor %d out of range", index);
        id = (index < nc ? m->convs[index].am : m->heads[index - nc].c3.am) + 2;
      } else {
        FR_CHECK(index >= 0 && index < nc, "debug_buffer: backbone convolution %d out of range", index);
        id = m->convs[index].am + (kind == 8 ? 1 : 0);
      }
      FR_CHECK(id >= 0 && id < (int)m->am_live.size() && m->am_live[id], "debug_buffer: the last pass kept no magnitude record of kind %d, index %d", kind, index);
      *ptr = m->rec(id); *bytes = (long long)AMAX_REC * 4;
      return FRCNN_OK;
    }
    default: FR_CHECK(false, "debug_buffer: unknown kind %d", kind);
  }
  FR_CHECK(b->p && b->bytes >= n, "debug_buffer: buffer not allocated yet");
  *ptr = b->p; *bytes = (long long)n;
  return FRCNN_OK;
}

int frcnn_pnet_delta(frcnn_model* m, int i, float** ptr) {
  FR_CHECK(m->H > 0, "pnet_delta: call frcnn_pnet_forward first");
  FR_CHECK(i >= 1 && i <= (int)m->heads.size() + 1, "pnet_delta: index %d out of range", i);
  *ptr = i <= (int)m->heads.size() ? m->heads[i - 1].delta.f() : m->delta_last.f();
  return FRCNN_OK;
}

int frcnn_pnet_set_sparse_deltas(frcnn_model* m, int head, const int* positions, int count) {
  FR_CHECK(head >= 1 && head <= (int)m->heads.size(), "pnet_set_sparse_deltas: head %d out of range", head);
  m->heads[head - 1].sp_pos = positions;
  m->heads[head - 1].sp_count = count;
  return FRCNN_OK;
}

int frcnn_pnet_zero_deltas(frcnn_model* m, void* stream) {
  FR_CHECK(m->H > 0, "pnet_zero_deltas: call frcnn_pnet_forward first");
  FR_TRY(fill_zero(m->zero_arena.p, m->delta_bytes, S(stream)));
  return FRCNN_OK;
}

static bool head_is_sparse(const Head& h) { return h.sp_count >= 0 && h.sp_count <= SPARSE_MAX_POS; }
static bool head_needs_gin(const frcnn_model* m, const Head& h) { return h.input >= m->frozen_blocks; }
static bool backbone_trained(const frcnn_model* m) { return m->frozen_blocks < (int)m->blocks.size(); }

static int backward_head(frcnn_model* m, Head& h, const float* w, float* grad, hipStream_t s, int ws_slot) {
  Block& in = m->blocks[h.input];
  Conv &a = h.c3, &c = h.c1;
  const long hw1 = (long)c.Ho * c.Wo;
  if (head_is_sparse(h)) {
    const int P = h.sp_count;
    const int* pos = h.sp_pos;
    h.sp_count = -1; h.sp_pos = nullptr;
    if (P == 0) return FRCNN_OK;
    const int n = a.Cout, ckk = a.Cin * a.k * a.k;
    FR_TRY(h.spD.ensure((size_t)HEAD_OUT * SPARSE_MAX_POS * 4));
    FR_TRY(h.spHX.ensure((size_t)n * SPARSE_MAX_POS * 4));
    FR_TRY(h.spHY.ensure((size_t)n * SPARSE_MAX_POS * 4));
    FR_TRY(h.spGH.ensure((size_t)n * SPARSE_MAX_POS * 4));
    FR_TRY(h.spCol.ensure((size_t)ckk * SPARSE_MAX_POS * 4));
    FR_TRY(h.spDX.ensure((size_t)ckk * SPARSE_MAX_POS * 4));
    float *D = h.spD.f(), *HX = h.spHX.f(), *HY = h.spHY.f(), *GH = h.spGH.f(), *COL = h.spCol.f(), *DX = h.spDX.f();
    FR_TRY(gather_positions(h.delta.f(), HEAD_OUT, hw1, pos, P, D, nullptr, nullptr, s));
    FR_TRY(gather_positions(a.x.f(), n, hw1, pos, P, HX, w + a.a_off, HY, s));
    FR_TRY(gemm_f32(w + c.w_off, 1, n, D, P, 1, GH, P, n, P, HEAD_OUT, OUT_STORE, nullptr, s, ws_slot));
    FR_TRY(act_backward(GH, HX, n, P, w + a.a_off, nullptr, GH, grad + a.b_off, grad + a.a_off, s));
    if (head_needs_gin(m, h)) {
      FR_TRY(gemm_f32(GH, 1, P, w + a.w_off, ckk, 1, DX, ckk, P, ckk, n, OUT_STORE, nullptr, s, ws_slot));
      FR_TRY(col2im_positions_add(DX, a.Cin, a.H, a.W, a.k, a.Wo, pos, P, in.gpooled.f(), s));
    }
    if (h.stream && s == h.stream) {
      FR_TRY(h.gin_done.record(s));
      h.gin_recorded = true;
    }
    FR_TRY(gemm_f32(D, P, 1, HY, 1, P, grad + c.w_off, n, HEAD_OUT, n, P, OUT_ADD, nullptr, s, ws_slot));
    FR_TRY(channel_sum(D, HEAD_OUT, P, grad + c.b_off, s));
    FR_TRY(im2col_positions(in.pooled.f(), a.Cin, a.H, a.W, a.k, a.Wo, pos, P, COL, s));
    FR_TRY(gemm_f32(GH, P, 1, COL, ckk, 1, grad + a.w_off, ckk, n, ckk, P, OUT_ADD, nullptr, s, ws_slot));
    return FRCNN_OK;
  }
  h.sp_count = -1; h.sp_pos = nullptr;
  if (!m->head_packs_fresh) {
    FR_TRY(conv_pack_weights_multi(w, (const PackJob*)m->pack_jobs.p + m->n_pack_all + m->n_pack_fwd, m->n_pack_heads,
                                   m->pack_grid_heads, s));
    m->head_packs_fresh = true;
  }
  FR_TRY(conv_wgrad(a.x.f(), c.Cin, c.H, c.W, w + a.a_off, nullptr, h.delta.f(), HEAD_OUT, 1, 0, grad + c.w_off, m->wg_ws.p, m->wg_ws.bytes, s));
  FR_TRY(channel_sum(h.delta.f(), HEAD_OUT, hw1, grad + c.b_off, s));
  double f1 = 2.0 * HEAD_OUT * c.Cin * (double)hw1;
  FR_TRY(conv_igemm(h.delta.f(), HEAD_OUT, c.Ho, c.Wo, nullptr, nullptr, c.wd.f(), nullptr, c.Cin, 1, 0, a.gx.f(),
                    OUT_STORE, f1, s, ws_slot));
  FR_TRY(act_backward(a.gx.f(), a.x.f(), a.Cout, (long)a.Ho * a.Wo, w + a.a_off, nullptr, a.gx.f(),
                      grad + a.b_off, grad + a.a_off, s));
  FR_TRY(conv_wgrad(in.pooled.f(), a.Cin, a.H, a.W, nullptr, nullptr, a.gx.f(), a.Cout, a.k, 0, grad + a.w_off, m->wg_ws.p, m->wg_ws.bytes, s));
  if (!head_needs_gin(m, h)) return FRCNN_OK;
  double f3 = 2.0 * a.Cout * a.Cin * a.k * a.k * (double)a.Ho * a.Wo;
  FR_TRY(conv_igemm(a.gx.f(), a.Cout, a.Ho, a.Wo, nullptr, nullptr, a.wd.f(), nullptr, a.Cin, a.k, a.k - 1,
                    in.gpooled.f(), OUT_ADD, f3, s, ws_slot));
  return FRCNN_OK;
}

// ... 398 lines not shown
      const bool first_pooled = fuse_act && first_pooled_on && b == 0 && st == 0 && blk.nconv == 1 && scale == nullptr &&
                                conv_wgrad_first_pooled_eligible(c.Cin, c.Cout, c.k, c.Wo);
      if (first_pooled) {
        FR_TRY(conv_wgrad_first_pooled(m->img.f(), c.Cin, c.H, c.W, blk.gpooled.f(), (const unsigned char*)blk.pidx.p, c.x.f(),
                                       w + c.a_off, c.Cout, c.pad, grad + c.w_off, grad + c.b_off, grad + c.a_off,
                                       m->wg_ws_first.p, m->wg_ws_first.bytes, s));
        FR_TRY(mark_block_done(m, b, s));
        break;
      }
      if (fused_here) {
      } else if (st == blk.nconv - 1) {
        FR_TRY(maxpool_act_backward(blk.gpooled.f(), (const unsigned char*)blk.pidx.p, c.x.f(), c.Cout, c.Ho, c.Wo,
                                    w + c.a_off, scale, c.gx.f(), grad + c.b_off, grad + c.a_off, s,
                                    (c.x_d && m->f16_packed) ? m->rec_w(c.am + 1) : nullptr));
      } else {
        FR_TRY(act_backward(c.gx.f(), c.x.f(), c.Cout, (long)c.Ho * c.Wo, w + c.a_off, scale, c.gx.f(),
                            grad + c.b_off, grad + c.a_off, s, (c.x_d && m->f16_packed) ? m->rec_w(c.am + 1) : nullptr));
      }
      const WgradArgs wa = wgrad_args(m, w, b, st);
      const bool dc = wa.mapped;
      const bool on_caller = use_side && b == 0 && st == 0;
      if (use_side && !on_caller) FR_TRY(fork_side(m, s, n_fork++));
      const hipStream_t wgs = on_caller ? s : ws;
      const DevBuf& slabs = on_caller ? m->wg_ws_first : m->wg_ws;
      FR_TRY(conv_wgrad(wa.in, wa.cin, c.H, c.W, wa.in_slope, wa.in_scale, c.gx.f(), wa.o, c.k, c.pad, grad + c.w_off, slabs.p, slabs.bytes, wgs,
                        fused_here ? grad + c.b_off : nullptr, wa.wa_in, wa.wa_g, dc ? &wa.map : nullptr));
      if (on_caller) FR_TRY(join_side_now(m, s));
      if (st == 0) FR_TRY(m->block_ev[b].record(wgs));
      if (b == fb && st == 0) {
        FR_TRY(record_block_read(m, b, s));
        break;
      }
      float* gin = st > 0 ? m->convs[blk.first_conv + st - 1].gx.f() : m->blocks[b - 1].gpooled.f();
      const int gmode = st > 0 ? OUT_STORE : OUT_ADD;
      const float* ag = nullptr;
      const float* aw = nullptr;
      if (c.x_d && m->f16_packed) { ag = m->rec(c.am + 1); aw = m->amax_ws.f() + c.am; }
      const int dg_k = (dc && st == 0) ? blk.nkK : c.Cout, dg_m = (dc && st == 1) ? blk.nkM : c.Cin;
      const double fl = 2.0 * dg_k * dg_m * c.k * c.k * (double)c.Ho * c.Wo;
      if (c.x_d && st > 0 && fuse_act && c.k == 3) {
        Conv& pc = m->convs[blk.first_conv + st - 1];
        X3PostAct post{pc.x.f(), w + pc.a_off, (st - 1 == 0 && blk.has_drop && !dc) ? blk.scale.f() : nullptr, grad + pc.a_off};
        FR_TRY(conv_x3(c.gx.f(), dg_k, c.Ho, c.Wo, nullptr, nullptr, c.wxd.p, nullptr, dg_m, c.k, c.k - 1 - c.pad, gin, gmode, fl, s, 0, &post, ag, aw,
                       (pc.x_d && m->f16_packed) ? m->rec_w(pc.am + 1) : nullptr));
        act_done = true;
      } else if (c.x_d)
        FR_TRY(conv_x3(c.gx.f(), dg_k, c.Ho, c.Wo, nullptr, nullptr, c.wxd.p, nullptr, dg_m, c.k, c.k - 1 - c.pad, gin, gmode, fl, s, 0, nullptr, ag, aw));
      else
        FR_TRY(conv_igemm(c.gx.f(), c.Cout, c.Ho, c.Wo, nullptr, nullptr, c.wd.f(), nullptr, c.Cin, c.k,
                          c.k - 1 - c.pad, gin, gmode, fl, s));
      if (st == 0) FR_TRY(record_block_read(m, b, s));
    }
  }
  m->block_ev_valid = true;
  if (heads_tail && !m->heads_gin) FR_TRY(join_heads(m, s));
  FR_TRY(cw_join(m, s));
  if (use_side) {
    FR_TRY(join_side_now(m, s));
    m->side_busy = false;
  }
  return FRCNN_OK;
}

static bool cnet_fuse() { return env_flag("FRCNN_CNET_FUSE", true); }
static bool gemm_f16_on() {
  static const bool env_on = env_flag("FRCNN_GEMM_F16", true);
  return env_on && get_x3_f16();
}
static int ensure_cnet(frcnn_model* m, int R) {
  for (auto& L : m->cls) {
    size_t n = (size_t)R * L.n * 4;
    FR_TRY(L.lin.ensure(n));
    if (L.bn) { FR_TRY(L.pre.ensure(n)); FR_TRY(L.xhat.ensure(n)); FR_TRY(L.invstd.ensure((size_t)L.n * 4)); }
    FR_TRY(L.post.ensure(n));
    FR_TRY(L.g.ensure(n));
    FR_TRY(L.gin.ensure((size_t)R * L.in * 4));
    if (L.p_drop > 0.f) FR_TRY(L.mask.ensure(n));
    L.x_form = 0;
    for (int role : {1, 2, 4}) if (linear_x_eligible(role, R, L.in, L.n)) L.x_form |= role;
    const size_t Rp = (size_t)linear_x_rows_padded(R);
    if (L.x_form & 1) FR_TRY(L.xp.ensure((size_t)3 * R * L.in * 2));
    if (L.x_form & 2) FR_TRY(L.gp.ensure((size_t)3 * R * L.n * 2));
    if (L.x_form & 4) { FR_TRY(L.xpT.ensure((size_t)3 * L.in * Rp * 2)); FR_TRY(L.gpT.ensure((size_t)3 * L.n * Rp * 2)); }
    if (L.x_form & 7) FR_TRY(L.am.ensure((size_t)5 * AMAX_REC * 4));
  }
  int nc = m->d.class_count + 1;
  int nf = m->cls.empty() ? m->D : m->cls.back().n;
  FR_TRY(m->feat_g.ensure((size_t)R * nf * 4));
  FR_TRY(m->logits.ensure((size_t)R * nc * 4));
  FR_TRY(m->lsm.ensure((size_t)R * nc * 4));
  FR_TRY(m->glog.ensure((size_t)R * nc * 4));
  return FRCNN_OK;
}

int frcnn_cnet_forward(frcnn_model* m, const float* weights, const float* x, int R, int training,
                       const float* const* drop_masks, unsigned long long seed, float* bn_running,
                       float* bbox_out, float* cls_out, void* stream) {
  hipStream_t s = S(stream);
  FR_CHECK(R > 0, "cnet_forward: empty batch");
  FR_TRY(cw_join(m, s));
  FR_TRY(ensure_cnet(m, R));
  m->R = R; m->cnet_x = x; m->training = training;
  const float* w = weights;
  const float* cur = x;
  float* bnr = bn_running;
  for (size_t l = 0; l < m->cls.size(); ++l) {
    ClsLayer& L = m->cls[l];
    GemmFold fold;
    GemmFold* defer = cnet_fuse() ? &fold : nullptr;
    if ((L.x_form & 3) && gemm_f16_on()) {
      float* rw = L.am.f() + 2 * AMAX_REC;
      const bool have = !training && g_static_weights && L.am_w_gen == g_static_gen && L.am_w_of == w;
      if (!have) FR_TRY(tensor_absmax(w + L.w_off, (long)L.n * L.in, rw, s));
      L.am_w_of = w; L.am_w_gen = training ? -1 : g_static_gen;
    } else {
      L.am_w_of = nullptr;
    }
    if ((L.x_form & 1) && gemm_f16_on()) {
      float* rx = L.am.f();
      FR_TRY(tensor_absmax(cur, (long)R * L.in, rx, s));
      FR_TRY(split_planes(cur, R, L.in, L.xp.p, nullptr, s, rx));
      FR_TRY(linear_x_forward(L.xp.p, R, L.in, w + L.w_off, w + L.b_off, L.n, L.lin.f(), s, 0, defer, rx, rx + 2 * AMAX_REC));
    } else if (L.x_form & 1) {
      FR_TRY(split_planes(cur, R, L.in, L.xp.p, nullptr, s));
      FR_TRY(linear_x_forward(L.xp.p, R, L.in, w + L.w_off, w + L.b_off, L.n, L.lin.f(), s, 0, defer));
    } else {
      FR_TRY(gemm_f32(cur, L.in, 1, w + L.w_off, 1, L.in, L.lin.f(), L.n, R, L.n, L.in, OUT_STORE, w + L.b_off, s, 0, defer));
    }
    if (L.bn) FR_CHECK(training || bnr, "cnet_forward: evaluate mode needs bn_running");
    const float* mask = nullptr;
    float inv_keep = 1.f;
    bool draw = false;
    if (training && L.p_drop > 0.f) {
      inv_keep = 1.0f / (1.0f - L.p_drop);
      if (drop_masks && drop_masks[l])
        FR_HIP(hipMemcpyAsync(L.mask.p, drop_masks[l], (size_t)R * L.n * 4, hipMemcpyDeviceToDevice, s));
      else
        draw = true;
      mask = L.mask.f();
    }
    if (defer) {
      FR_TRY(cnet_act_forward(L.lin.f(), fold, R, L.n, L.bn ? w + L.bnw_off : nullptr, L.bn ? w + L.bnb_off : nullptr, L.bn ? bnr : nullptr,
                              training, L.lin.f(), L.xhat.f(), L.invstd.f(), L.pre.f(), w + L.a_off, const_cast<float*>(mask), draw,
                              inv_keep, L.p_drop, seed * 977 + l + 17, L.post.f(), s));
      if (L.bn && bnr) bnr += 2 * L.n;
      cur = L.post.f();
      continue;
    }
    const float* pre = L.lin.f();
    if (L.bn) {
      FR_TRY(bn_forward(L.lin.f(), R, L.n, w + L.bnw_off, w + L.bnb_off, bnr, training, L.xhat.f(), L.invstd.f(),
                        L.pre.f(), s));
      if (bnr) bnr += 2 * L.n;
      pre = L.pre.f();
    }
    if (draw)
      FR_TRY(prelu_dropout_forward_gen(pre, (long)R * L.n, w + L.a_off, L.mask.f(), L.p_drop, seed * 977 + l + 17,
                                       L.post.f(), s));
    else
      FR_TRY(prelu_dropout_forward(pre, (long)R * L.n, w + L.a_off, mask, inv_keep, L.post.f(), s));
    cur = L.post.f();
  }
  const int nf = m->cls.empty() ? m->D : m->cls.back().n;
  const int nc = m->d.class_count + 1;
  if (cnet_fuse() && cnet_heads_fused_eligible(nf, nc)) {
    return cnet_heads_forward(cur, R, nf, w + m->bbox_w_off, w + m->bbox_b_off, w + m->clsw_off, w + m->clsb_off, nc, bbox_out,
                              m->logits.f(), m->lsm.f(), cls_out, s);
  }
  FR_TRY(gemm_f32(cur, nf, 1, w + m->bbox_w_off, 1, nf, bbox_out, 4, R, 4, nf, OUT_STORE, w + m->bbox_b_off, s));
  if (cnet_fuse()) {
    GemmFold fold;
    FR_TRY(gemm_f32(cur, nf, 1, w + m->clsw_off, 1, nf, m->logits.f(), nc, R, nc, nf, OUT_STORE, w + m->clsb_off, s, 0, &fold));
    FR_TRY(log_softmax_rows_fold(m->logits.f(), fold, R, nc, m->lsm.f(), cls_out, s));
    return FRCNN_OK;
  }
  FR_TRY(gemm_f32(cur, nf, 1, w + m->clsw_off, 1, nf, m->logits.f(), nc, R, nc, nf, OUT_STORE, w + m->clsb_off, s));
  FR_TRY(log_softmax_rows(m->logits.f(), R, nc, m->lsm.f(), s));
  FR_HIP(hipMemcpyAsync(cls_out, m->lsm.p, (size_t)R * nc * 4, hipMemcpyDeviceToDevice, s));
  return FRCNN_OK;
}

int frcnn_cnet_backward(frcnn_model* m, const float* weights, const float* g_bbox, const float* g_cls, float* gx,
                        float* grad, void* stream) {
  hipStream_t s = S(stream);
  FR_CHECK(m->R > 0, "cnet_backward: call frcnn_cnet_forward first");
  const int R = m->R;
  const float* w = weights;
  const int nf = m->cls.empty() ? m->D : m->cls.back().n;
  const int nc = m->d.class_count + 1;
  const float* feat = m->cls.empty() ? m->cnet_x : m->cls.back().post.f();
  if (m->frozen_blocks >= (int)m->blocks.size()) gx = nullptr;
  FR_TRY(cw_join(m, s));
  const bool async = g_cnet_wgrad_async && !deterministic();
  if (async) FR_TRY(ensure_update_stream(m));
  hipStream_t ws = async ? m->cw : s;
  const int wslot = async ? 7 : 0;
  size_t nfork = 0;
  auto fork = [&]() -> int {
    return async ? chain(s, ws, m->cw_ev[nfork++]) : FRCNN_OK;
  };
  bool top_act_done = false;
  if (cnet_fuse() && cnet_heads_fused_eligible(nf, nc)) {
    HeadsPostAct post;
    float* dst = m->feat_g.f();
    if (!m->cls.empty() && !m->cls.back().bn && !deterministic()) {
      ClsLayer& T = m->cls.back();
      const bool drop = m->training && T.p_drop > 0.f;
      post.pre = T.lin.f(); post.mask = drop ? T.mask.f() : nullptr; post.inv_keep = drop ? 1.0f / (1.0f - T.p_drop) : 1.f;
      post.slope = w + T.a_off; post.gslope = grad + T.a_off;
      dst = T.g.f();
      top_act_done = true;
    }
    FR_TRY(cnet_heads_backward(g_bbox, g_cls, m->lsm.f(), R, nf, w + m->bbox_w_off, w + m->clsw_off, nc, m->glog.f(), dst, s,
                               top_act_done ? &post : nullptr));
    FR_TRY(fork());
  } else {
    FR_TRY(log_softmax_backward(g_cls, m->lsm.f(), R, nc, m->glog.f(), s));
    FR_TRY(fork());
    FR_TRY(gemm_f32(g_bbox, 4, 1, w + m->bbox_w_off, nf, 1, m->feat_g.f(), nf, R, nf, 4, OUT_STORE, nullptr, s));
    FR_TRY(gemm_f32(m->glog.f(), nc, 1, w + m->clsw_off, nf, 1, m->feat_g.f(), nf, R, nf, nc, OUT_ADD, nullptr, s));
  }
  FR_TRY(gemm_f32(g_bbox, 1, 4, feat, nf, 1, grad + m->bbox_w_off, nf, 4, nf, R, OUT_ADD, nullptr, ws, wslot));
  FR_TRY(channel_sum_cols(g_bbox, R, 4, grad + m->bbox_b_off, ws));
  FR_TRY(gemm_f32(m->glog.f(), 1, nc, feat, nf, 1, grad + m->clsw_off, nf, nc, nf, R, OUT_ADD, nullptr, ws, wslot));
  FR_TRY(channel_sum_cols(m->glog.f(), R, nc, grad + m->clsb_off, ws));
  const float* g = m->feat_g.f();
  GemmFold gfold;
  for (int l = (int)m->cls.size() - 1; l >= 0; --l) {
    ClsLayer& L = m->cls[l];
    const float* pre = L.bn ? L.pre.f() : L.lin.f();
    const bool drop = m->training && L.p_drop > 0.f;
    if (top_act_done && l == (int)m->cls.size() - 1) {
    } else if (L.bn && cnet_fuse()) {
      FR_TRY(cnet_act_bn_backward(g, gfold, pre, L.xhat.f(), L.invstd.f(), w + L.bnw_off, w + L.a_off, drop ? L.mask.f() : nullptr,
                                  drop ? 1.0f / (1.0f - L.p_drop) : 1.f, R, L.n, m->training, L.g.f(), grad + L.bnw_off,
                                  grad + L.bnb_off, grad + L.a_off, s));
    } else {
      FR_TRY(prelu_dropout_backward(g, pre, (long)R * L.n, w + L.a_off, drop ? L.mask.f() : nullptr,
                                    drop ? 1.0f / (1.0f - L.p_drop) : 1.f, L.g.f(), grad + L.a_off, s));
      if (L.bn)
        FR_TRY(bn_backward(L.g.f(), L.xhat.f(), L.invstd.f(), w + L.bnw_off, R, L.n, m->training, L.g.f(),
                           grad + L.bnw_off, grad + L.bnb_off, s));
    }
    gfold = GemmFold{};
    GemmFold* gdefer = (cnet_fuse() && async && l > 0 && m->cls[l - 1].bn) ? &gfold : nullptr;
    FR_TRY(fork());
    const float* in = l == 0 ? m->cnet_x : m->cls[l - 1].post.f();
    float* gin = l == 0 ? gx : L.gin.f();
    const bool xw = (L.x_form & 4) != 0, xd = (L.x_form & 2) != 0 && gin;
    if (xd && gemm_f16_on() && L.am_w_of == w) {
      float* rg = L.am.f() + AMAX_REC;
      FR_TRY(tensor_absmax(L.g.f(), (long)R * L.n, rg, s));
      FR_TRY(split_planes(L.g.f(), R, L.n, L.gp.p, nullptr, s, rg));
      FR_TRY(linear_x_dgrad(L.gp.p, R, L.n, w + L.w_off, L.in, gin, OUT_STORE, s, 0, gdefer, rg, L.am.f() + 2 * AMAX_REC));
    } else if (xd) {
      FR_TRY(split_planes(L.g.f(), R, L.n, L.gp.p, nullptr, s));
      FR_TRY(linear_x_dgrad(L.gp.p, R, L.n, w + L.w_off, L.in, gin, OUT_STORE, s, 0, gdefer));
    } else if (gin) {
      FR_TRY(gemm_f32(L.g.f(), L.n, 1, w + L.w_off, L.in, 1, gin, L.in, R, L.in, L.n, OUT_STORE, nullptr, s, 0, gdefer));
    }
    static const bool wgrad_f16 = env_flag("FRCNN_GEMM_WGRAD_F16", true);
    if (xw && wgrad_f16 && gemm_f16_on() && L.am.bytes >= (size_t)5 * AMAX_REC * 4) {
      float *rgT = L.am.f() + 3 * AMAX_REC, *rxT = L.am.f() + 4 * AMAX_REC;
      FR_TRY(tensor_absmax(L.g.f(), (long)R * L.n, rgT, ws));
      if ((L.x_form & 1) && L.am_w_of == w) rxT = L.am.f();
      else FR_TRY(tensor_absmax(in, (long)R * L.in, rxT, ws));
      FR_TRY(split_planes(L.g.f(), R, L.n, nullptr, L.gpT.p, ws, rgT));
      FR_TRY(split_planes(in, R, L.in, nullptr, L.xpT.p, ws, rxT));
      FR_TRY(linear_x_wgrad(L.gpT.p, L.xpT.p, R, L.n, L.in, grad + L.w_off, ws, wslot, rgT, rxT));
    } else if (xw) {
      FR_TRY(split_planes(L.g.f(), R, L.n, nullptr, L.gpT.p, ws));
      FR_TRY(split_planes(in, R, L.in, nullptr, L.xpT.p, ws));
      FR_TRY(linear_x_wgrad(L.gpT.p, L.xpT.p, R, L.n, L.in, grad + L.w_off, ws, wslot));
    } else {
      FR_TRY(gemm_f32(L.g.f(), 1, L.n, in, L.in, 1, grad + L.w_off, L.in, L.n, L.in, R, OUT_ADD, nullptr, ws, wslot));
    }
    FR_TRY(channel_sum_cols(L.g.f(), R, L.n, grad + L.b_off, ws));
    g = gin;
  }
  if (m->cls.empty() && gx) FR_HIP(hipMemcpyAsync(gx, g, (size_t)R * m->D * 4, hipMemcpyDeviceToDevice, s));
  if (async) {
    FR_TRY(m->cw_done.record(ws));
    m->cw_pending = true;
  }
  return FRCNN_OK;
}

}
```

faster-rcnn.torch_amd/csrc/roi.hip:

```cpp
#include "kernels.h"
#include "roi_fix.h"

namespace frcnn {

__global__ void roi_pool_forward_kernel(const float* __restrict__ fmap, int C, int H, int W,
                                        const int* __restrict__ wins, int R, int kh, int kw,
                                        float* __restrict__ out, int* __restrict__ idx) {
  const long total = (long)R * C * kh * kw;
  for (long t = (long)blockIdx.x * blockDim.x + threadIdx.x; t < total; t += (long)gridDim.x * blockDim.x) {
    int j = (int)(t % kw);
    long q = t / kw;
    int i = (int)(q % kh);
    q /= kh;
    int c = (int)(q % C);
    int r = (int)(q / C);
    const int* wn = wins + 4 * r;
    const int r0 = wn[0] - 1, c0 = wn[2] - 1;
    const int h = wn[1] - wn[0] + 1, w = wn[3] - wn[2] + 1;
    const int ys = (i * h) / kh, ye = ((i + 1) * h + kh - 1) / kh;
    const int xs = (j * w) / kw, xe = ((j + 1) * w + kw - 1) / kw;
    const float* ip = fmap + (size_t)c * H * W;
    float best = -3.402823466e+38f;
    int bi = -1;
    for (int y = ys; y < ye; ++y)
      for (int x = xs; x < xe; ++x) {
        float v = ip[(size_t)(r0 + y) * W + (c0 + x)];
        if (v > best) { best = v; bi = (r0 + y) * W + (c0 + x); }
      }
    out[t] = best;
    if (idx) idx[t] = bi;
  }
}

__global__ __launch_bounds__(256) void roi_pool_forward_cells_kernel(const float* __restrict__ fmap, int C, int H, int W,
                                                                     const int* __restrict__ wins, int kh, int kw,
                                                                     float* __restrict__ out, int* __restrict__ idx) {
  const int r = blockIdx.x, cells = kh * kw, groups = blockDim.x / cells;
  const int tid = threadIdx.x;
  if (tid >= groups * cells) return;
  const int cg = tid / cells, cell = tid - cg * cells;
  const int i = cell / kw, j = cell - i * kw;
  const int* wn = wins + 4 * r;
  const int r0 = wn[0] - 1, c0 = wn[2] - 1;
  const int h = wn[1] - wn[0] + 1, w = wn[3] - wn[2] + 1;
  const int ys = (i * h) / kh, ye = ((i + 1) * h + kh - 1) / kh;
  const int xs = (j * w) / kw, xe = ((j + 1) * w + kw - 1) / kw;
  const int HW = H * W;
  const int base = (r0 + ys) * W + c0 + xs, nx = xe - xs, ny = ye - ys;
  if (HW >= 4) {
    for (int c = blockIdx.y * groups + cg; c < C; c += gridDim.y * groups) {
      const float* ip = fmap + (size_t)c * HW;
      float best = -3.402823466e+38f;
      int bi = -1;
      for (int y = 0, o = base; y < ny; ++y, o += W)
        for (int x = 0; x < nx; x += 4) {
          const int q = min(o + x, HW - 4);
          float v[4];
          __builtin_memcpy(v, ip + q, 16);
#pragma unroll
          for (int e = 0; e < 4; ++e) {
            const int at = q + e;
            if (at >= o && at < o + nx && v[e] > best) { best = v[e]; bi = at; }
          }
        }
      const size_t t = ((size_t)r * C + c) * cells + cell;
      out[t] = best;
      if (idx) idx[t] = bi;
    }
    return;
  }
  for (int c = blockIdx.y * groups + cg; c < C; c += gridDim.y * groups) {
    const float* ip = fmap + (size_t)c * HW;
    float best = -3.402823466e+38f;
    int bi = -1;
    for (int y = 0, o = base; y < ny; ++y, o += W)
      for (int x = 0; x < nx; ++x) {
        const float v = ip[o + x];
        if (v > best) { best = v; bi = o + x; }
      }
    const size_t t = ((size_t)r * C + c) * cells + cell;
    out[t] = best;
    if (idx) idx[t] = bi;
  }
}

int roi_pool_forward(const float* fmap, int C, int H, int W, const int* wins, int R, int kh, int kw,
                     float* out, int* idx, hipStream_t s) {
  if (R <= 0) return FRCNN_OK;
  long total = (long)R * C * kh * kw;
  if (kh * kw <= 256) {
    const int groups = 256 / (kh * kw);
    const int slices = std::max(1, std::min(cdiv(C, groups), (int)cdivl(4096, R)));
    FR_LAUNCH(KC_ROI, 0, total * 8.0, s, roi_pool_forward_cells_kernel, dim3(R, slices), dim3(256), 0, fmap, C, H, W,
              wins, kh, kw, out, idx);
    FR_LAUNCH_CHECK();
    return FRCNN_OK;
  }
  int grid = (int)std::min<long>(cdivl(total, 256), 4096);
  FR_LAUNCH(KC_ROI, 0, total * 8.0, s, roi_pool_forward_kernel, dim3(grid), dim3(256), 0, fmap, C, H, W,
            wins, R, kh, kw, out, idx);
  FR_LAUNCH_CHECK();
  return FRCNN_OK;
}

__global__ void roi_pool_backward_lds_kernel(float* __restrict__ gmap, int C, int HW, const float* __restrict__ gout,
                                             const int* __restrict__ idx, int R, int cell) {
  extern __shared__ float plane[];
  const int c = blockIdx.x;
  for (int i = threadIdx.x; i < HW; i += blockDim.x) plane[i] = 0.f;
  __syncthreads();
  const long D = (long)C * cell;
  const int total = R * cell;
  for (int e = threadIdx.x; e < total; e += blockDim.x) {
    const int r = e / cell, j = e - r * cell;
    const long t = (long)r * D + (long)c * cell + j;
    const int bi = idx[t];
    const float g = gout[t];
    if (bi >= 0 && g != 0.f) atomicAdd(&plane[bi], g);
  }
  __syncthreads();
  float* gp = gmap + (size_t)c * HW;
  for (int i = threadIdx.x; i < HW; i += blockDim.x) {
    const float v = plane[i];
    if (v != 0.f) gp[i] += v;
  }
}

__global__ void roi_pool_backward_lds_det_kernel(float* __restrict__ gmap, int C, int HW, const float* __restrict__ gout,
                                                 const int* __restrict__ idx, int R, int cell) {
  extern __shared__ unsigned long long fplane[];
  const int c = blockIdx.x;
  for (int i = threadIdx.x; i < HW; i += blockDim.x) fplane[i] = 0ull;
  __syncthreads();
  const long D = (long)C * cell;
  const int total = R * cell;
  for (int e = threadIdx.x; e < total; e += blockDim.x) {
    const int r = e / cell, j = e - r * cell;
    const long t = (long)r * D + (long)c * cell + j;
    const int bi = idx[t];
    const float g = gout[t];
    if (bi >= 0 && g != 0.f) atomicAdd(&fplane[bi], (unsigned long long)roi_to_fix(g));
  }
  __syncthreads();
  float* gp = gmap + (size_t)c * HW;
  for (int i = threadIdx.x; i < HW; i += blockDim.x) {
    const long long v = (long long)fplane[i];
    if (v != 0) gp[i] += (float)((double)v / ROI_FIX_SCALE);
  }
}
__global__ void roi_pool_backward_det_kernel(unsigned long long* __restrict__ fix, int C, long HW,
                                             const float* __restrict__ gout, const int* __restrict__ idx,
                                             long total, int cell) {
  for (long t = (long)blockIdx.x * blockDim.x + threadIdx.x; t < total; t += (long)gridDim.x * blockDim.x) {
    int c = (int)((t / cell) % C);
    int bi = idx[t];
    float g = gout[t];
    if (bi >= 0 && g != 0.f) atomicAdd(fix + (size_t)c * HW + bi, (unsigned long long)roi_to_fix(g));
  }
}
__global__ void roi_fix_apply_kernel(const unsigned long long* __restrict__ fix, long n, float* __restrict__ gmap) {
  for (long t = (long)blockIdx.x * blockDim.x + threadIdx.x; t < n; t += (long)gridDim.x * blockDim.x) {
    const long long v = (long long)fix[t];
    if (v != 0) gmap[t] += (float)((double)v / ROI_FIX_SCALE);
  }
}

int roi_fix_apply(const unsigned long long* fix, long n, float* gmap, hipStream_t s) {
  FR_LAUNCH(KC_ROI, 0, n * 16.0, s, roi_fix_apply_kernel, dim3((int)std::min<long>(cdivl(n, 256), 4096)), dim3(256), 0, fix, n, gmap);
  FR_LAUNCH_CHECK();
  return FRCNN_OK;
}

__global__ void roi_pool_backward_kernel(float* __restrict__ gmap, int C, long HW,
                                         const float* __restrict__ gout, const int* __restrict__ idx,
                                         long total, int cell) {
  for (long t = (long)blockIdx.x * blockDim.x + threadIdx.x; t < total; t += (long)gridDim.x * blockDim.x) {
    int c = (int)((t / cell) % C);
// ... 43 lines not shown
```

faster-rcnn.torch_amd/objective.py:

```python
import ctypes as C
import os
import sys

import numpy as np

from . import _lib
from .Anchors import Anchors
from .Localizer import Localizer
from .Rect import Rect
from .tensor import DeviceTensor, ptr, stream_ptr, to_device


def roi_window(input_rect, localizer, fm_h, fm_w):
    r = localizer.inputToFeatureRect(input_rect)
    r = r.clip(Rect(0, 0, fm_w, fm_h))
    return (int(min(r.minY + 1, r.maxY)), int(r.maxY), int(min(r.minX + 1, r.maxX)), int(r.maxX))


def roi_windows(rects, localizer, fm_h, fm_w):
    r = localizer.inputToFeatureRectBatch(rects)
    minX = np.minimum(np.maximum(r[:, 0], 0), fm_w); minY = np.minimum(np.maximum(r[:, 1], 0), fm_h)
    maxX = np.maximum(np.minimum(r[:, 2], fm_w), 0); maxY = np.maximum(np.minimum(r[:, 3], fm_h), 0)
    return np.stack([np.minimum(minY + 1, maxY), maxY, np.minimum(minX + 1, maxX), maxX], 1).astype(np.int32)

# ... 342 lines not shown
                n_ex = len(held0[1]["p"]) + len(held0[1]["n"])
            else:
                sizes0 = output_map_sizes(model, x0["img"].shape[1], x0["img"].shape[2])
                n_ex = len(clean_examples(x0["positive"], sizes0)) + len(clean_examples(x0["negative"], sizes0))
            eager["gscale"] = (1.0 / n_ex) if n_ex > 0 else 1.0
            eager["done"] = []
            eager["ranges"] = ranges
            us = C.c_void_p()
            _lib.call("frcnn_model_update_stream", native.h, C.byref(us))
            nblk = int(native.desc.nblocks)

            def eager_slice(lo, hi, on, group=None):
                eager["update"](weights, gradient, lo, hi, eager["gscale"], on)
                eager["done"].append((int(lo), int(hi)))
                if group is not None:
                    _lib.call("frcnn_pnet_refresh_packs", native.h, ptr(weights), group, on)
                    eager["groups"].add(group)
            eager["groups"] = set()
            eager["slice"] = eager_slice
        dev_tail = (dev_tail_ok and defer == "fold" and _dist() is not None and getattr(gradient, "is_cuda", False)
                    and ranges is None)
        c4 = None
        if dev_tail:
            from .synthetic import clean_examples, output_map_sizes
            c4 = [0.0, 0.0, 0.0, 0.0]
            for x in batch:
                shp = x["img"].shape
                sizes = output_map_sizes(model, shp[1], shp[2])
                np_, nn_ = len(clean_examples(x["positive"], sizes)), len(clean_examples(x["negative"], sizes))
                c4[0] += np_ + nn_; c4[1] += np_; c4[2] += np_; c4[3] += 1
            init = np.array([0.0, 0.0, c4[0], c4[1], 0.0, 0.0, c4[2], c4[3]], dtype=np.float64)
            hinit, staged = pinned.stage(init.view(np.uint8))
            _lib.call("frcnn_memcpy_h2d", ptr(acc_dev), C.c_void_p(hinit), 64, s)
            staged()
        else:
            acc_dev.zero_()
        for bi, x in enumerate(batch):
            last = bi == len(batch) - 1
            held = prepared.pop(id(x), None)
            prep = held[1] if held is not None and held[0] is x else prepare_examples(x)
            img = to_device(x["img"])
            outputs = pnet.forward(img, async_heads=True)
            if prep["sizes"] != [tuple(o.shape[1:]) for o in outputs[:len(prep["sizes"])]] or prep["fm"] != tuple(outputs[-1].shape[1:]):
                raise _lib.FrcnnError("lossAndGradient: the example tables were packed for other map sizes than this image's")
            p, n = prep["p"], prep["n"]
            delta_outputs = pnet.delta_outputs(zero=True)
            npos, nneg = len(p), len(n)
            E = npos + nneg
            fm = outputs[-1]
            fmC, fmH, fmW = fm.shape
            if E > 0:
                ex_anchor, ex_roi, ex_idx, ex_class, wins, sp, blob = (prep[k] for k in ("ex_anchor", "ex_roi", "ex_idx", "ex_class", "wins", "sp", "blob"))
                dblob = scratch.get("blob", (blob.size,), np.uint8)
                hblob, staged = pinned.stage(blob)
                _lib.call("frcnn_memcpy_h2d", ptr(dblob), C.c_void_p(hblob), blob.nbytes, s)
                staged()
                o = 0
                d_anchor = dblob.ptr + o; o += ex_anchor.nbytes
                d_roi = dblob.ptr + o; o += ex_roi.nbytes
                d_idx = dblob.ptr + o; o += ex_idx.nbytes
                d_class = dblob.ptr + o; o += ex_class.nbytes
                if align:
                    o += -o % 8
                d_wins = dblob.ptr + o; o += wins.nbytes
                for l in range(4):
                    _lib.call("frcnn_pnet_set_sparse_deltas", native.h, l + 1, C.c_void_p(dblob.ptr + o), len(sp[l]))
                    o += sp[l].nbytes
                ex_loss = scratch.get("ex_loss", (E, 2), np.float64)
                crtarget = scratch.get("crtarget", (E, 4))
                cctarget = scratch.get("cctarget", (E,))
                pnet.anchor_loss_begin(d_idx, d_anchor, d_roi, d_class, npos, nneg, bgclass, ex_loss, crtarget,
                                       cctarget, acc_dev)
            if E > 0 and not classification:
                native.seed += 1
                pnet.anchor_loss_wait()
            elif E > 0:
                cinput = scratch.get("cinput", (E, D))
                if align:
                    debug["rects"] = wins
                    _lib.call("frcnn_roi_align_forward", ptr(fm), fmC, fmH, fmW, C.c_void_p(d_wins), None, E, inv_sx, inv_sy,
                              kh, kw, sampling, ptr(cinput), s)
                else:
                    pidx = scratch.get("pidx", (E, D), np.int32)
                    _lib.call("frcnn_roi_pool_forward", ptr(fm), fmC, fmH, fmW, C.c_void_p(d_wins), E, kh, kw,
                              ptr(cinput), ptr(pidx), s)
                coutputs = cnet.forward(cinput)
                crout, ccout = coutputs
                crdelta = scratch.get("crdelta", (E, 4))
                ccdelta = scratch.get("ccdelta", (E, ncls))
                pnet.anchor_loss_wait()
                _lib.call("frcnn_cnet_losses", ptr(crout), ptr(crtarget), ptr(ccout), ptr(cctarget), E, npos, ncls,
                          ptr(crdelta), ptr(ccdelta), C.c_void_p(acc_dev.ptr + 4 * 8), s)
                post_roi_delta = cnet.backward(cinput, [crdelta, ccdelta])
                if not trunk_frozen and align:
                    _lib.call("frcnn_roi_align_backward", ptr(delta_outputs[4]), fmC, fmH, fmW, ptr(post_roi_delta),
                              C.c_void_p(d_wins), None, E, inv_sx, inv_sy, kh, kw, sampling, s)
                elif not trunk_frozen:
                    _lib.call("frcnn_roi_pool_backward", ptr(delta_outputs[4]), fmC, fmH, fmW, ptr(post_roi_delta),
                              ptr(pidx), E, kh, kw, s)
            if E == 0:
                for l in range(4):
                    _lib.call("frcnn_pnet_set_sparse_deltas", native.h, l + 1, None, 0)
            if last and _dist() is not None:
                _lib.call("frcnn_cnet_backward_join", native.h, stream_ptr())
                if classification:
                    pending.append(allreduce_begin(gradient, native.pnet_params, gradient.numel()))
                side = C.c_int(0)
                _lib.call("frcnn_get_option", b"side_stream", C.byref(side))
                if len(batch) == 1 and side.value and proposal:
                    pnet.backward_heads_join()
                    lo, hi = pnet.heads_param_range()
                    pending.append(allreduce_begin(gradient, lo, hi))
            if last and probing:
                _lib.call("frcnn_cnet_backward_join", native.h, stream_ptr())
                _probe_mark("classification net", native.pnet_params, gradient.numel(), "frcnn_cnet_backward_join (its weight-gradient stream)")
                side = C.c_int(0)
                _lib.call("frcnn_get_option", b"side_stream", C.byref(side))
                if len(batch) == 1 and side.value:
                    pnet.backward_heads_join()
                    lo, hi = pnet.heads_param_range()
                    _probe_mark("anchor nets", lo, hi, "frcnn_pnet_backward_heads_join (the anchor nets' streams)")
            if last and defer and _dist() is None and not guarded:
                acc_pin.copy_(acc_t, non_blocking=True)
                acc_event.record()
                early_copy = True
            debug["E"] = E
            pnet.backward(img, delta_outputs)
            if eager is not None:
                _lib.call("frcnn_pnet_wait_backward_begun", native.h, us)
                if classification:
                    eager_slice(native.pnet_params, gradient.numel(), us)
                _lib.call("frcnn_pnet_wait_heads_done", native.h, us)
                lo, hi = pnet.heads_param_range()
                if proposal:
                    eager_slice(lo, hi, us, nblk)
                for b in range(nblk, max(frozen_blocks, 1), -1):
                    _lib.call("frcnn_pnet_wait_block_done", native.h, b, us)
                    lo, hi = pnet.block_param_range(b - 1)
                    eager_slice(lo, hi, us, b - 1)
                _lib.call("frcnn_model_update_join", native.h, stream_ptr())
            if last and _dist() is not None and early_blocks and getattr(gradient, "is_cuda", False):
                if aux_stream[0] is None:
                    aux_stream[0] = torch.cuda.Stream()
                for b in [b for b in early_blocks if b >= frozen_blocks]:
                    lo, hi = pnet.block_param_range(b)
                    with torch.cuda.stream(aux_stream[0]):
                        pnet.wait_block_gradients(b)
                        pending.append(allreduce_begin(gradient, lo, hi))
            if last and probing:
                covered = []
                if early_blocks:
                    if aux_stream[0] is None:
                        aux_stream[0] = torch.cuda.Stream()
                    for b in early_blocks:
                        lo, hi = pnet.block_param_range(b)
                        with torch.cuda.stream(aux_stream[0]):
                            pnet.wait_block_gradients(b)
                            _probe_mark("backbone block %d" % (b + 1), lo, hi, "frcnn_pnet_wait_block_gradients(%d) on an auxiliary stream" % (b + 1))
                        covered.append((lo, hi))
                _probe_mark("backward_end", 0, 0, "")
                lo_rest = 0
                hi_rest = min([c[0] for c in covered] + [pnet.heads_param_range()[0]])
                _probe_mark("rest of the backbone", lo_rest, hi_rest, "end of frcnn_pnet_backward on the caller's stream")
            reg_count += npos
            cls_count += npos + nneg
            creg_count += npos
            ccls_count += 1
# ... 139 lines not shown
```

include/frcnn_hip.h:

```cpp
#ifndef FRCNN_HIP_H
#define FRCNN_HIP_H

#include <stddef.h>

#ifdef __cplusplus
extern "C" {
#endif

#define FRCNN_OK 0
#define FRCNN_ERR_ARG 1
#define FRCNN_ERR_HIP 2
#define FRCNN_ERR_STATE 3

int frcnn_version(void);
const char *frcnn_last_error(void);
int frcnn_device_count(int *n);
int frcnn_set_device(int device);
int frcnn_device_name(char *buf_host, int len);
int frcnn_set_option(const char *name, int value);
int frcnn_get_option(const char *name, int *value_host);

int frcnn_malloc(void **ptr_out_host, size_t bytes);
int frcnn_free(void *ptr);
int frcnn_host_alloc(void **ptr_out_host, size_t bytes);
// ... 24 lines not shown
#define FRCNN_KC_COUNT 15
int frcnn_prof_enable(int class_mask);
int frcnn_prof_collect(long long *launches_host, double *ms_host, double *flops_host,
                       double *bytes_host);

size_t frcnn_nms_workspace_bytes(int n);
int frcnn_nms_device(const float *boxes, int n, int ncols, float overlap, int key_mode,
                     int key_col, long long *pick, int *count, void *workspace,
                     size_t workspace_bytes, void *stream);
int frcnn_nms_device_classes(const float *boxes, int n, int ncols, float overlap, int key_mode, int key_col,
                             const int *cls, long long *pick, int *count, void *workspace,
                             size_t workspace_bytes, void *stream);
int frcnn_nms_device_n(const float *boxes, int n_cap, const int *n_dev, int ncols, float overlap, int key_mode, int key_col,
                       const int *cls, long long *pick, int *count, void *workspace, size_t workspace_bytes, void *stream);
size_t frcnn_nms_batch_workspace_bytes(int B, int n_cap);
int frcnn_nms_device_batch(const float *boxes, int B, long long row_stride, int n_cap, const int *n_dev, int ncols, float overlap,
                           int key_mode, int key_col, const int *cls, long long *pick, int *count, void *workspace,
                           size_t workspace_bytes, void *stream);
size_t frcnn_soft_nms_workspace_bytes(int B, int n_cap);
int frcnn_soft_nms_batch(const float *boxes, int B, long long row_stride, int n_cap, const int *n_dev, int ncols, int score_col,
                         int method, float overlap, float sigma, float min_score, int log_domain, const int *cls,
                         long long *pick, int *count, float *score_out, long long score_stride, void *workspace,
                         size_t workspace_bytes, void *stream);
int frcnn_box_vote_batch(const float *boxes, int B, long long row_stride, int n_cap, const int *n_dev, int ncols, int score_col,
                         int weight_mode, float overlap, const int *cls, const double *rect, const long long *pick,
                         const int *count, double *rect_out, int *votes_out, void *stream);
int frcnn_roi_windows(const double *rect, const long long *pick, int k, const int *layers_host, int nlayers, int fmH, int fmW,
                      int *wins, void *stream);
int frcnn_detect_post(const int *cls, const float *conf, const float *bbox, const double *rect, const long long *pick, int R,
                      int bgclass, double min_conf, float *bb, int *kc, int *keep_row, double *r2, int *K_dev, void *stream);
int frcnn_detect_classes_batch(const float *cls_out, const float *bbox, const int *R_host, const long long *row0_host, int B,
                               const double *rect, const long long *pick, long long match_stride, int ncls, int bgclass,
                               double min_conf, int mode, float *bb, int *kc, int *keep_row, double *r2, int row_stride, int *K_dev,
                               int *total_dev, void *stream);
int frcnn_detect_gather_batch(const long long *wpick, const int *counts, int B, int row_stride, const int *keep_row,
                              const int *kc, const float *bb, const double *r2, const long long *pick, long long match_stride,
                              const float *match_p, const double *match_rect, const int *match_idx, double *rec, void *stream);
int frcnn_detect_merge_views(const float *bb, const int *kc, const int *keep_row, const double *r2, long long row_stride,
                             const int *counts, const long long *pick, long long match_stride, int F, int V,
                             const int *flip_host, const double *wv_host, const double *ax_host, const double *ay_host,
                             const int *R_host, float *bb_out, int *kc_out, int *keep_row_out, double *r2_out,
                             long long *pick_out, int *counts_out, void *stream);
int frcnn_nms_host(const float *boxes_host, int n, int ncols, float overlap, int key_mode,
                   int key_col, long long *pick_host, int *count_host);

int frcnn_conv2d_forward(const float *in, int C, int H, int W, const float *in_slope,
                         const float *in_scale, const float *weight, const float *bias, int O,
                         int k, int pad, float *out, void *stream);
int frcnn_conv2d_backward_input(const float *gout, int O, int Ho, int Wo, const float *weight,
                                int C, int k, int pad, float *gin, int accumulate, void *stream);
int frcnn_conv2d_backward_weight(const float *in, int C, int H, int W, const float *in_slope,
                                 const float *in_scale, const float *gout, int O, int k, int pad,
                                 float *gweight, float *gbias, void *stream);

int frcnn_maxpool_act_forward(const float *x, int C, int H, int W, const float *slope,
                              const float *scale, float *out, unsigned char *idx, void *stream);
int frcnn_maxpool_act_backward(const float *gpool, const unsigned char *idx, const float *x, int C,
                               int H, int W, const float *slope, const float *scale, float *gx,
                               float *gbias, float *gslope, void *stream);
int frcnn_act_forward(const float *x, int C, long long hw, const float *slope, const float *scale,
                      float *y, void *stream);
int frcnn_act_backward(const float *gy, const float *x, int C, long long hw, const float *slope,
                       const float *scale, float *gx, float *gbias, float *gslope, void *stream);

int frcnn_amax_record_floats(void);
int frcnn_tensor_absmax(const float *x, long long n, float *rec, void *stream);
int frcnn_maxpool_act_forward_rec(const float *x, int C, int H, int W, const float *slope,
                                  const float *scale, float *out, unsigned char *idx, void *stream, float *rec);
int frcnn_maxpool_act_backward_rec(const float *gpool, const unsigned char *idx, const float *x, int C,
                                   int H, int W, const float *slope, const float *scale, float *gx,
                                   float *gbias, float *gslope, void *stream, float *rec);
int frcnn_act_backward_rec(const float *gy, const float *x, int C, long long hw, const float *slope,
                           const float *scale, float *gx, float *gbias, float *gslope, void *stream, float *rec);
int frcnn_conv2d_forward_rec(const float *in, int C, int H, int W, const float *in_slope,
                             const float *in_scale, const float *weight, const float *bias, int O,
                             int k, int pad, float *out, const float *rec_in, float *rec_out, void *stream);
int frcnn_conv2d_backward_input_rec(const float *gout, int O, int Ho, int Wo, const float *weight,
                                    int C, int k, int pad, float *gin, int accumulate, const float *rec_g,
                                    float *rec_out, const float *post_x, const float *post_slope,
                                    const float *post_scale, float *gslope, void *stream);

int frcnn_roi_pool_forward(const float *fmap, int C, int H, int W, const int *wins, int R, int kh,
                           int kw, float *out, int *idx, void *stream);
int frcnn_roi_pool_backward(float *gmap, int C, int H, int W, const float *gout, const int *idx,
                            int R, int kh, int kw, void *stream);

int frcnn_roi_align_forward(const float *fmap, int C, int H, int W, const double *rect, const long long *pick, int R,
                            double inv_sx, double inv_sy, int kh, int kw, int g, float *out, void *stream);
int frcnn_roi_align_backward(float *gmap, int C, int H, int W, const float *gout, const double *rect, const long long *pick,
                             int R, double inv_sx, double inv_sy, int kh, int kw, int g, void *stream);

size_t frcnn_rpn_scan_workspace_bytes(const int *H_host, const int *W_host);
int frcnn_rpn_scan(const float *const *maps_host, const int *H_host, const int *W_host,
                   const float *anchor_w, const float *anchor_h, double img_w, double img_h,
                   double p_threshold, int cap, float *match_p, int *match_idx,
                   double *match_rect, float *match_box, int *count, void *workspace,
                   size_t workspace_bytes, void *stream);
size_t frcnn_rpn_scan_batch_workspace_bytes(const int *H_host, const int *W_host, int B);
int frcnn_rpn_scan_batch(const float *const *maps_host, const int *H_host, const int *W_host, int B, long long slot_stride,
                         const float *anchor_w, const float *anchor_h, double img_w, double img_h, double p_threshold,
                         int cap, float *match_p, int *match_idx, double *match_rect, float *match_box, int *count,
                         void *workspace, size_t workspace_bytes, void *stream);
size_t frcnn_rpn_scan_ragged_workspace_bytes(const int *H_host, const int *W_host, int B);
int frcnn_rpn_scan_ragged(const float *heads, const long long *map_off_host, const int *H_host, const int *W_host,
                          const double *img_wh_host, int B, const float *anchor_w, const float *anchor_h, double p_threshold,
                          int cap, float *match_p, int *match_idx, double *match_rect, float *match_box, int *count,
                          void *workspace, size_t workspace_bytes, void *stream);

size_t frcnn_topk_select_workspace_bytes(int B, int n_cap);
int frcnn_topk_select(const float *score, int B, long long stride, int n_cap, const int *n_dev, int K, int *sel_row,
                      long long sel_stride, int *k_dev, void *workspace, size_t workspace_bytes, void *stream);
int frcnn_rpn_gather_rows(const float *match_p, const int *match_idx, const double *match_rect, const float *match_box, int B,
                          long long src_stride, int src_rows, const int *sel_row, long long sel_stride, const int *k_dev,
                          int k_cap, float *dst_p, int *dst_idx, double *dst_rect, float *dst_box, float *box5, int *row,
                          long long dst_stride, void *stream);

int frcnn_rpn_loss(const float *const *maps_host, float *const *deltas_host, const int *H_host,
                   const int *W_host, const int *ex_idx, const double *ex_anchor,
                   const double *ex_roi, const int *ex_class, int npos, int nneg, int bgclass,
                   double *ex_loss, float *crtarget, float *cctarget, void *stream);

int frcnn_loss_accumulate(const double *ex_loss, int E, double *acc, void *stream);

int frcnn_linear_forward(const float *x, int R, int I, const float *weight, const float *bias,
                         int O, float *y, void *stream);
int frcnn_linear_backward(const float *x, const float *gy, int R, int I, const float *weight,
                          int O, float *gx, float *gweight, float *gbias, void *stream);

int frcnn_rmsprop(float *x, const float *g, float *m, long long n, float lr, float alpha,
                  float eps, void *stream);
int frcnn_scale_rmsprop(float *x, float *g, float gscale, float *m, long long n, float lr, float alpha,
                        float eps, void *stream);
int frcnn_scale_rmsprop_dev(float *x, float *g, const double *gcount_dev, float *m, long long n, float lr,
                            float alpha, float eps, void *stream);
int frcnn_scale_rmsprop_slice(float *x, float *g, float gscale, float *m, long long lo, long long hi, float lr,
                              float alpha, float eps, void *stream);

int frcnn_sgd(float *x, float *g, float *v, long long n, float gscale, const double *gcount_dev, float clr, float wd,
              float mom, float one_minus_damp, int nesterov, int first, void *stream);
int frcnn_sgd_slice(float *x, float *g, float *v, long long lo, long long hi, float gscale, float clr, float wd, float mom,
                    float one_minus_damp, int nesterov, int first, void *stream);
int frcnn_nag(float *x, float *g, float *v, long long n, float gscale, const double *gcount_dev, float clr, float wd,
              float mom, int first, void *stream);
int frcnn_nag_slice(float *x, float *g, float *v, long long lo, long long hi, float gscale, float clr, float wd, float mom,
                    int first, void *stream);
int frcnn_scale_rmsprop_slice_dev(float *x, float *g, const double *gcount_dev, float *m, long long lo, long long hi,
                                  float lr, float alpha, float eps, void *stream);
int frcnn_sgd_slice_dev(float *x, float *g, float *v, long long lo, long long hi, const double *gcount_dev, float clr,
                        float wd, float mom, float one_minus_damp, int nesterov, int first, void *stream);
int frcnn_nag_slice_dev(float *x, float *g, float *v, long long lo, long long hi, const double *gcount_dev, float clr,
                        float wd, float mom, int first, void *stream);

size_t frcnn_grad_clip_workspace_bytes(long long n);
int frcnn_grad_clip(float *g, long long n, const long long *ranges_host, int nranges, double divisor,
                    const double *divisor_dev, double clip_norm, double *record_dev, void *workspace,
                    size_t workspace_bytes, void *stream);

int frcnn_nag_lookahead(float *x, const float *v, long long n, float mom, void *stream);
int frcnn_nag_lookahead_slice(float *x, const float *v, long long lo, long long hi, float mom, void *stream);

typedef struct {
  int nblocks;
  int filters[8], ksize[8], pad[8], conv_steps[8];
  float dropout[8];
  int nheads;
  int head_k[8], head_n[8], head_input[8];
  int ncls;
  int cls_n[8], cls_bn[8];
  float cls_dropout[8];
  int class_count;
  int kh, kw;
} frcnn_model_desc;

typedef struct frcnn_model frcnn_model;

int frcnn_model_create(const frcnn_model_desc *desc_host, frcnn_model **out_host);
int frcnn_model_destroy(frcnn_model *);
int frcnn_model_param_count(const frcnn_model *, long long *total_host, long long *pnet_host);
int frcnn_model_param_table(const frcnn_model *, long long *table_host, int cap, int *n_host);
int frcnn_model_localizer_layers(const frcnn_model *, int output_index, int *layers_host, int cap,
                                 int *n_host);
int frcnn_model_set_trainable(frcnn_model *, int frozen_blocks, int heads, int cnet);
int frcnn_model_get_trainable(const frcnn_model *, int *frozen_blocks_host, int *heads_host, int *cnet_host);

int frcnn_pnet_forward(frcnn_model *, const float *weights, const float *img, int H, int W,
                       int training, const float *const *drop_masks_host, unsigned long long seed,
                       void *stream);
int frcnn_pnet_forward_async_heads(frcnn_model *, const float *weights, const float *img, int H, int W,
                                   const float *const *drop_masks_host, unsigned long long seed,
                                   void *stream);
int frcnn_pnet_output(frcnn_model *, int i, float **ptr_host, int *C_host, int *H_host,
                      int *W_host);
int frcnn_model_debug_buffer(frcnn_model *, int kind, int index, void **ptr_host, long long *bytes_host);
int frcnn_pnet_delta(frcnn_model *, int i, float **ptr_host);
int frcnn_pnet_zero_deltas(frcnn_model *, void *stream);
int frcnn_pnet_set_sparse_deltas(frcnn_model *, int head, const int *positions, int count);
int frcnn_pnet_backward_heads_begin(frcnn_model *, const float *weights, float *grad, void *stream);
int frcnn_pnet_anchor_loss_begin(frcnn_model *, const float *weights, float *grad, const int *ex_idx,
                                 const double *ex_anchor, const double *ex_roi, const int *ex_class,
                                 int npos, int nneg, int bgclass, double *ex_loss, float *crtarget,
                                 float *cctarget, double *acc, void *stream);
int frcnn_pnet_anchor_loss_wait(frcnn_model *, void *stream);
int frcnn_pnet_backward_heads_join(frcnn_model *, void *stream, int *joined_host);
int frcnn_pnet_backward(frcnn_model *, const float *weights, float *grad, void *stream);

int frcnn_pnet_wait_block_gradients(frcnn_model *, int block, void *stream);

int frcnn_model_update_stream(frcnn_model *, void **stream_host);
int frcnn_model_update_fork(frcnn_model *, void *stream);
int frcnn_model_update_join(frcnn_model *, void *stream);
int frcnn_pnet_wait_backward_begun(frcnn_model *, void *stream);
int frcnn_pnet_wait_heads_done(frcnn_model *, void *stream);
int frcnn_pnet_wait_block_done(frcnn_model *, int block, void *stream);
int frcnn_pnet_refresh_packs(frcnn_model *, const float *weights, int group, void *stream);
int frcnn_pnet_invalidate_packs(frcnn_model *);

int frcnn_cnet_forward(frcnn_model *, const float *weights, const float *x, int R, int training,
                       const float *const *drop_masks_host, unsigned long long seed,
                       float *bn_running, float *bbox_out, float *cls_out, void *stream);
int frcnn_cnet_backward_join(frcnn_model *, void *stream);
int frcnn_cnet_backward(frcnn_model *, const float *weights, const float *g_bbox,
                        const float *g_cls, float *gx, float *grad, void *stream);
int frcnn_cnet_losses(float *crout, const float *crtarget, const float *ccout,
                      const float *cctarget, int R, int npos, int ncls, float *crdelta,
                      float *ccdelta, double *loss2, void *stream);
int frcnn_cnet_decode(const float *cls_out, int R, int ncls, int *cls, float *conf, void *stream);

int frcnn_image_rgb2yuv(const float *rgb, float *yuv, int H, int W, void *stream);
int frcnn_image_rgb2hsv(const float *rgb, float *hsv, int H, int W, void *stream);
int frcnn_image_rgb2lab(const float *rgb, float *lab, int H, int W, void *stream);
int frcnn_image_scale(const float *src, int C, int H, int W, float *dst, int dH, int dW, float *tmp,
                      int rgb2yuv, void *stream);
int frcnn_image_scale_u8(const unsigned char *src_hwc, int H, int W, float *dst, int dH, int dW,
                         float *tmp, int rgb2yuv, void *stream);
int frcnn_image_crop_flip(const float *src, int C, int H, int W, int x0, int y0, int w, int h, int hflip,
                          int vflip, float *dst, void *stream);
size_t frcnn_image_normalize_workspace_bytes(int C);
int frcnn_image_normalize(float *img, int C, int H, int W, int centering, int scaling, void *workspace,
                          size_t workspace_bytes, void *stream);
int frcnn_image_contrastive_norm(const float *in, int H, int W, const float *kernel_host, int K,
                                 float threshold, float *out, float *tmp, void *stream);

typedef struct frcnn_anchors frcnn_anchors;
int frcnn_anchors_create(const float *w_tab_host, const float *h_tab_host, const double *cx_host,
                         const double *cy_host, int nscales, int width, frcnn_anchors **out_host);
int frcnn_anchors_destroy(frcnn_anchors *);
int frcnn_anchors_assemble(frcnn_anchors *, const double *rois_host, int nroi, double img_w, double img_h,
                           double pos_thr, double neg_thr, int best_match, int nearby_aversion,
                           int negatives, unsigned int *mt_state_host, int *mt_index_host, int *ex_host,
                           double *ex_rect_host, int cap, int *npos_host, int *nneg_host);

#define FRCNN_COMM_ID_BYTES 128
typedef struct frcnn_comm frcnn_comm;
int frcnn_comm_get_unique_id(void *id_host);
int frcnn_comm_exchange_id_file(const char *path, int rank, void *id_host, int timeout_ms);
int frcnn_comm_init_rank(frcnn_comm **out_host, int nranks, int rank, const void *id_host);
int frcnn_comm_init_rank_timeout(frcnn_comm **out_host, int nranks, int rank, const void *id_host, int timeout_ms);
int frcnn_comm_init_rank_file(frcnn_comm **out_host, int nranks, int rank, const char *path, int timeout_ms);
int frcnn_comm_destroy(frcnn_comm *);
int frcnn_comm_info(const frcnn_comm *, int *nranks_host, int *rank_host);
int frcnn_comm_query(const frcnn_comm *, int *count_host, int *user_rank_host, int *device_host);
int frcnn_allreduce_f32(frcnn_comm *, float *buf, long long n, void *stream);
int frcnn_allreduce_f64(frcnn_comm *, double *buf, long long n, void *stream);
int frcnn_broadcast_f32(frcnn_comm *, float *buf, long long n, int root, void *stream);

#ifdef __cplusplus
}
#endif
#endif
```

Baseline: 524.0.

## Fuse absmax recording into classifier backward and ROI pool forward kernels

Folds the per-block absolute-max reduction, used to scale the fp16 split planes, into the epilogues of the BN, PReLU/dropout, heads-backward and ROI-pool kernels, so the separate tensor_absmax passes over gradients and ROI-pooled inputs are skipped. A model-level ROI pool entry point records the amax of the pooled classifier input, letting the first linear layer reuse it. When a launch has more blocks than the amax record can hold, the code falls back to a separate absmax pass. The cost is an extra reduction and a barrier in each fused kernel, plus more plumbing of record pointers.

```diff
diff --git a/faster-rcnn.torch_amd/_lib.py b/faster-rcnn.torch_amd/_lib.py
--- a/faster-rcnn.torch_amd/_lib.py
+++ b/faster-rcnn.torch_amd/_lib.py
@@ -89,6 +89,8 @@
     "frcnn_conv2d_backward_input_rec": ([vp, C.c_int, C.c_int, C.c_int, vp, C.c_int, C.c_int, C.c_int, vp, C.c_int, vp, vp, vp, vp, vp, vp,
                                          vp], C.c_int),
     "frcnn_roi_pool_forward": ([vp, C.c_int, C.c_int, C.c_int, vp, C.c_int, C.c_int, C.c_int, vp, vp, vp], C.c_int),
+    "frcnn_roi_pool_forward_rec": ([vp, C.c_int, C.c_int, C.c_int, vp, C.c_int, C.c_int, C.c_int, vp, vp, vp, C.POINTER(C.c_int), vp], C.c_int),
+    "frcnn_model_roi_pool_forward": ([vp, vp, C.c_int, C.c_int, C.c_int, vp, C.c_int, C.c_int, C.c_int, vp, vp, vp], C.c_int),
     "frcnn_roi_pool_backward": ([vp, C.c_int, C.c_int, C.c_int, vp, vp, C.c_int, C.c_int, C.c_int, vp], C.c_int),
     "frcnn_roi_align_forward": ([vp, C.c_int, C.c_int, C.c_int, vp, vp, C.c_int, C.c_double, C.c_double, C.c_int, C.c_int, C.c_int, vp,
                                  vp], C.c_int),
diff --git a/faster-rcnn.torch_amd/csrc/amax.h b/faster-rcnn.torch_amd/csrc/amax.h
--- a/faster-rcnn.torch_amd/csrc/amax.h
+++ b/faster-rcnn.torch_amd/csrc/amax.h
@@ -19,6 +19,20 @@
   }
 }
 
+__device__ __forceinline__ void amax_store_block_flat(float m, float* rec, int tid, int nthreads, int blk, int nblk) {
+  __shared__ float amax_part_flat[16];
+#pragma unroll
+  for (int o = 32; o > 0; o >>= 1) m = fmaxf(m, __shfl_xor(m, o));
+  if ((tid & 63) == 0) amax_part_flat[tid >> 6] = m;
+  __syncthreads();
+  if (tid == 0) {
+    const int nw = (nthreads + 63) >> 6;
+    for (int i = 1; i < nw; ++i) m = fmaxf(m, amax_part_flat[i]);
+    rec[1 + blk] = m;
+    if (blk == 0) rec[0] = __builtin_bit_cast(float, nblk);
+  }
+}
+
 __device__ __forceinline__ float amax_load_block(const float* __restrict__ rec) {
   __shared__ float amax_all[16];
   const int n = __builtin_bit_cast(int, rec[0]);
diff --git a/faster-rcnn.torch_amd/csrc/api.cpp b/faster-rcnn.torch_amd/csrc/api.cpp
--- a/faster-rcnn.torch_amd/csrc/api.cpp
+++ b/faster-rcnn.torch_amd/csrc/api.cpp
@@ -403,6 +403,13 @@
 int frcnn_roi_pool_forward(const float* fmap, int C, int H, int W, const int* wins, int R, int kh, int kw,
                            float* out, int* idx, void* stream) {
   return roi_pool_forward(fmap, C, H, W, wins, R, kh, kw, out, idx, S(stream));
+}
+int frcnn_roi_pool_forward_rec(const float* fmap, int C, int H, int W, const int* wins, int R, int kh, int kw,
+                               float* out, int* idx, void* stream, int* kept, float* rec) {
+  bool k = false;
+  const int rc = roi_pool_forward(fmap, C, H, W, wins, R, kh, kw, out, idx, S(stream), rec, &k);
+  if (kept) *kept = k ? 1 : 0;
+  return rc;
 }
 int frcnn_roi_pool_backward(float* gmap, int C, int H, int W, const float* gout, const int* idx, int R, int kh,
                             int kw, void* stream) {
diff --git a/faster-rcnn.torch_amd/csrc/cnet.hip b/faster-rcnn.torch_amd/csrc/cnet.hip
--- a/faster-rcnn.torch_amd/csrc/cnet.hip
+++ b/faster-rcnn.torch_amd/csrc/cnet.hip
@@ -1,4 +1,5 @@
 #include "kernels.h"
+#include "amax.h"
 
 namespace frcnn {
 
@@ -90,7 +91,7 @@
 __global__ __launch_bounds__(1024) void bn_backward_kernel(const float* __restrict__ gy, const float* __restrict__ xhat,
                                                            const float* __restrict__ invstd, const float* __restrict__ gamma,
                                                            int R, int n, int training, float* __restrict__ gx, float* ggamma,
-                                                           float* gbeta) {
+                                                           float* gbeta, float* __restrict__ amax) {
   __shared__ double sh[BN_RG * BN_CB];
   const int tx = threadIdx.x, ty = threadIdx.y;
   const int j = blockIdx.x * BN_CB + tx;
@@ -104,24 +105,32 @@
     }
   sg = bn_reduce(sg, sh, tx, ty);
   sgx = bn_reduce(sgx, sh, tx, ty);
-  if (!ok) return;
-  if (ty == 0) {
-    ggamma[j] = (float)((double)ggamma[j] + sgx);
-    gbeta[j] = (float)((double)gbeta[j] + sg);
-  }
-  const double is = invstd[j], gm = gamma[j];
-  for (int r = ty; r < R; r += BN_RG) {
-    const double g = gy[(size_t)r * n + j];
-    const double xh = xhat[(size_t)r * n + j];
-    const double v = training ? (g - sg / R - xh * sgx / R) * gm * is : g * gm * is;
-    gx[(size_t)r * n + j] = (float)v;
-  }
+  if (!ok && !amax) return;
+  float am = 0.f;
+  if (ok) {
+    if (ty == 0) {
+      ggamma[j] = (float)((double)ggamma[j] + sgx);
+      gbeta[j] = (float)((double)gbeta[j] + sg);
+    }
+    const double is = invstd[j], gm = gamma[j];
+    for (int r = ty; r < R; r += BN_RG) {
+      const double g = gy[(size_t)r * n + j];
+      const double xh = xhat[(size_t)r * n + j];
+      const double v = training ? (g - sg / R - xh * sgx / R) * gm * is : g * gm * is;
+      gx[(size_t)r * n + j] = (float)v;
+      am = fmaxf(am, fabsf((float)v));
+    }
+  }
+  if (amax) amax_store_block_flat(am, amax, ty * BN_CB + tx, BN_CB * BN_RG, blockIdx.x, gridDim.x);
 }
 int bn_backward(const float* gy, const float* xhat, const float* invstd, const float* gamma, int R,
-                int n, int training, float* gx, float* ggamma, float* gbeta, hipStream_t s) {
+                int n, int training, float* gx, float* ggamma, float* gbeta, hipStream_t s, float* amax) {
+  float* const amax_after = (amax && cdiv(n, BN_CB) > AMAX_MAX_BLOCKS) ? amax : nullptr;
+  if (amax_after) amax = nullptr;
   FR_LAUNCH(KC_ELEMWISE, 0, (double)R * n * 16.0, s, bn_backward_kernel, dim3(cdiv(n, BN_CB)), dim3(BN_CB, BN_RG), 0, gy,
-            xhat, invstd, gamma, R, n, training, gx, ggamma, gbeta);
-  FR_LAUNCH_CHECK();
+            xhat, invstd, gamma, R, n, training, gx, ggamma, gbeta, amax);
+  FR_LAUNCH_CHECK();
+  if (amax_after) return tensor_absmax(gx, (long)R * n, amax_after, s);
   return FRCNN_OK;
 }
 
@@ -276,7 +285,8 @@
                                                                     const float* __restrict__ invstd, const float* __restrict__ gamma,
                                                                     const float* slope, const float* __restrict__ mask, float inv_keep,
                                                                     int R, int n, int training, float* __restrict__ gx, float* ggamma,
-                                                                    float* gbeta, float* gslope, float* part) {
+                                                                    float* gbeta, float* gslope, float* part,
+                                                                    float* __restrict__ amax) {
   __shared__ double sh[FB_RG * FB_CB];
   __shared__ float shs[16];
   const int tx = threadIdx.x, ty = threadIdx.y;
@@ -325,38 +335,46 @@
       if (part) part[blockIdx.x] = t; else unsafeAtomicAdd(gslope, t);
     }
   }
-  if (!ok) return;
-  if (ty == 0) {
-    ggamma[j] = (float)((double)ggamma[j] + sgx);
-    gbeta[j] = (float)((double)gbeta[j] + sg);
-  }
-  const double is = invstd[j], gm = gamma[j];
-  auto second = [&](size_t idx, double g, double xhv) {
-    const double v = training ? (g - sg / R - xhv * sgx / R) * gm * is : g * gm * is;
-    gx[idx] = (float)v;
-  };
-  if (keep) {
-#pragma unroll
-    for (int i = 0; i < FB_KEEP; ++i)
-      if (ty + i * FB_RG < R) second((size_t)(ty + i * FB_RG) * n + j, tv[i], xh[i]);
-  } else {
-    for (int r = ty; r < R; r += FB_RG) {
-      const size_t idx = (size_t)r * n + j;
-      second(idx, gx[idx], xhat[idx]);
-    }
-  }
+  if (!ok && !amax) return;
+  float am = 0.f;
+  if (ok) {
+    if (ty == 0) {
+      ggamma[j] = (float)((double)ggamma[j] + sgx);
+      gbeta[j] = (float)((double)gbeta[j] + sg);
+    }
+    const double is = invstd[j], gm = gamma[j];
+    auto second = [&](size_t idx, double g, double xhv) {
+      const double v = training ? (g - sg / R - xhv * sgx / R) * gm * is : g * gm * is;
+      gx[idx] = (float)v;
+      am = fmaxf(am, fabsf((float)v));
+    };
+    if (keep) {
+#pragma unroll
+      for (int i = 0; i < FB_KEEP; ++i)
+        if (ty + i * FB_RG < R) second((size_t)(ty + i * FB_RG) * n + j, tv[i], xh[i]);
+    } else {
+      for (int r = ty; r < R; r += FB_RG) {
+        const size_t idx = (size_t)r * n + j;
+        second(idx, gx[idx], xhat[idx]);
+      }
+    }
+  }
+  if (amax) amax_store_block_flat(am, amax, ty * FB_CB + tx, FB_CB * FB_RG, blockIdx.x, gridDim.x);
 }
 __global__ void slope_fold_kernel(const float* __restrict__ part, int n, float* gslope);
 int cnet_act_bn_backward(const float* gy, GemmFold src, const float* pre, const float* xhat, const float* invstd,
                          const float* gamma, const float* slope, const float* mask, float inv_keep, int R, int n, int training,
-                         float* gx, float* ggamma, float* gbeta, float* gslope, hipStream_t s) {
+                         float* gx, float* ggamma, float* gbeta, float* gslope, hipStream_t s, float* amax) {
   const int grid = cdiv(n, FB_CB);
   float* part = nullptr;
   if (deterministic()) FR_TRY(det_workspace(s, (size_t)grid, &part));
+  float* const amax_after = (amax && grid > AMAX_MAX_BLOCKS) ? amax : nullptr;
+  if (amax_after) amax = nullptr;
   FR_LAUNCH(KC_ELEMWISE, 0, (double)R * n * 28.0, s, cnet_act_bn_backward_kernel, dim3(grid), dim3(FB_CB, FB_RG), 0, gy, src, pre, xhat,
-            invstd, gamma, slope, mask, inv_keep, R, n, training, gx, ggamma, gbeta, gslope, part);
+            invstd, gamma, slope, mask, inv_keep, R, n, training, gx, ggamma, gbeta, gslope, part, amax);
   if (part) FR_LAUNCH(KC_ELEMWISE, 0, grid * 4.0, s, slope_fold_kernel, dim3(1), dim3(1), 0, (const float*)part, grid, gslope);
   FR_LAUNCH_CHECK();
+  if (amax_after) return tensor_absmax(gx, (long)R * n, amax_after, s);
   return FRCNN_OK;
 }
 
@@ -397,10 +415,12 @@
 
 __global__ void prelu_dropout_backward_kernel(const float* __restrict__ gy, const float* __restrict__ x, long n,
                                               const float* slope, const float* __restrict__ mask,
-                                              float inv_keep, float* __restrict__ gx, float* gslope, float* part) {
+                                              float inv_keep, float* __restrict__ gx, float* gslope, float* part,
+                                              float* __restrict__ amax) {
   __shared__ float sh[4];
   const float a = *slope;
   float sa = 0.f;
+  float am = 0.f;
   for (long i = (long)blockIdx.x * blockDim.x + threadIdx.x; i < n; i += (long)gridDim.x * blockDim.x) {
     float g = gy[i];
     if (mask) g = g * (mask[i] * inv_keep);
@@ -408,6 +428,7 @@
     float r = g;
     if (!(xv > 0.f)) { r = a * g; sa += xv * g; }
     gx[i] = r;
+    am = fmaxf(am, fabsf(r));
   }
 #pragma unroll
   for (int o = 32; o > 0; o >>= 1) sa += __shfl_down(sa, o, 64);
@@ -418,6 +439,7 @@
     if (part) part[blockIdx.x] = t;
     else unsafeAtomicAdd(gslope, t);
   }
+  if (amax) amax_store_block(am, amax);
 }
 __global__ void slope_fold_kernel(const float* __restrict__ part, int n, float* gslope) {
   float v = 0.f;
@@ -425,12 +447,12 @@
   *gslope += v;
 }
 int prelu_dropout_backward(const float* gy, const float* x, long n, const float* slope,
-                           const float* mask, float inv_keep, float* gx, float* gslope, hipStream_t s) {
+                           const float* mask, float inv_keep, float* gx, float* gslope, hipStream_t s, float* amax) {
   int grid = (int)std::min<long>(std::max<long>(1, cdivl(n, 256)), 256);
   float* part = nullptr;
   if (deterministic()) FR_TRY(det_workspace(s, (size_t)grid, &part));
   FR_LAUNCH(KC_ELEMWISE, 0, n * 16.0, s, prelu_dropout_backward_kernel, dim3(grid), dim3(256), 0, gy, x, n,
-            slope, mask, inv_keep, gx, gslope, part);
+            slope, mask, inv_keep, gx, gslope, part, amax);
   if (part) FR_LAUNCH(KC_ELEMWISE, 0, grid * 4.0, s, slope_fold_kernel, dim3(1), dim3(1), 0, (const float*)part, grid, gslope);
   FR_LAUNCH_CHECK();
   return FRCNN_OK;
@@ -549,11 +571,13 @@
 __global__ __launch_bounds__(256) void cnet_heads_backward_kernel(const float* __restrict__ g_bbox, const float* __restrict__ g_cls,
                                                                   const float* __restrict__ lsm, int R, int nf,
                                                                   const float* __restrict__ Wb, const float* __restrict__ Wc, int nc,
-                                                                  float* __restrict__ glog, float* __restrict__ gfeat, HeadsPostAct post) {
+                                                                  float* __restrict__ glog, float* __restrict__ gfeat, HeadsPostAct post,
+                                                                  float* __restrict__ amax) {
   extern __shared__ float wt[];
   __shared__ float shs[4];
   const float pa = post.pre ? *post.slope : 1.f;
   float sa = 0.f;
+  float am = 0.f;
   const int no = 4 + nc;
   for (int k = threadIdx.x; k < nf; k += 256) {
 #pragma unroll
@@ -594,6 +618,7 @@
         if (!(xv > 0.f)) { sa += xv * g; g = pa * g; }
       }
       gfeat[(size_t)r * nf + k] = g;
+      am = fmaxf(am, fabsf(g));
     }
     __builtin_amdgcn_wave_barrier();
   }
@@ -604,6 +629,7 @@
     __syncthreads();
     if (threadIdx.x == 0) unsafeAtomicAdd(post.gslope, (shs[0] + shs[1]) + (shs[2] + shs[3]));
   }
+  if (amax) amax_store_block(am, amax);
 }
 bool cnet_heads_fused_eligible(int nf, int nc) { return 4 + nc <= 32 && nf % 8 == 0 && nf <= 1024; }
 int cnet_heads_forward(const float* x, int R, int nf, const float* Wb, const float* bb, const float* Wc, const float* bc, int nc,
@@ -623,7 +649,7 @@
   return FRCNN_OK;
 }
 int cnet_heads_backward(const float* g_bbox, const float* g_cls, const float* lsm, int R, int nf, const float* Wb, const float* Wc,
-                        int nc, float* glog, float* gfeat, hipStream_t s, const HeadsPostAct* post) {
+                        int nc, float* glog, float* gfeat, hipStream_t s, const HeadsPostAct* post, float* amax) {
   if (R <= 0) return FRCNN_OK;
   FR_CHECK(cnet_heads_fused_eligible(nf, nc), "cnet_heads_backward: %d classes", nc);
   const size_t lds = ((size_t)(4 + nc) * nf + 256) * 4;
@@ -633,7 +659,7 @@
     attr_lds = lds;
   }
   FR_LAUNCH(KC_ELEMWISE, 0, (double)R * nf * 4.0, s, cnet_heads_backward_kernel, dim3(std::min(cdiv(R, 4), 256)), dim3(256), lds, g_bbox, g_cls,
-            lsm, R, nf, Wb, Wc, nc, glog, gfeat, post ? *post : HeadsPostAct{});
+            lsm, R, nf, Wb, Wc, nc, glog, gfeat, post ? *post : HeadsPostAct{}, amax);
   FR_LAUNCH_CHECK();
   return FRCNN_OK;
 }
diff --git a/faster-rcnn.torch_amd/csrc/kernels.h b/faster-rcnn.torch_amd/csrc/kernels.h
--- a/faster-rcnn.torch_amd/csrc/kernels.h
+++ b/faster-rcnn.torch_amd/csrc/kernels.h
@@ -167,7 +167,7 @@
 
 
 int roi_pool_forward(const float* fmap, int C, int H, int W, const int* wins, int R, int kh, int kw,
-                     float* out, int* idx, hipStream_t s);
+                     float* out, int* idx, hipStream_t s, float* rec = nullptr, bool* kept = nullptr);
 int roi_pool_backward(float* gmap, int C, int H, int W, const float* gout, const int* idx, int R,
                       int kh, int kw, hipStream_t s);
 
@@ -237,19 +237,19 @@
 int bn_forward(const float* x, int R, int n, const float* gamma, const float* beta, float* running,
                int training, float* xhat, float* invstd, float* y, hipStream_t s);
 int bn_backward(const float* gy, const float* xhat, const float* invstd, const float* gamma, int R,
-                int n, int training, float* gx, float* ggamma, float* gbeta, hipStream_t s);
+                int n, int training, float* gx, float* ggamma, float* gbeta, hipStream_t s, float* amax = nullptr);
 int prelu_dropout_forward(const float* x, long n, const float* slope, const float* mask, float inv_keep,
                           float* y, hipStream_t s);
 int prelu_dropout_forward_gen(const float* x, long n, const float* slope, float* mask_out, float p,
                               unsigned long long seed, float* y, hipStream_t s);
 int prelu_dropout_backward(const float* gy, const float* x, long n, const float* slope,
-                           const float* mask, float inv_keep, float* gx, float* gslope, hipStream_t s);
+                           const float* mask, float inv_keep, float* gx, float* gslope, hipStream_t s, float* amax = nullptr);
 int cnet_act_forward(const float* x, GemmFold src, int R, int n, const float* gamma, const float* beta, float* running,
                      int training, float* lin, float* xhat, float* invstd, float* pre, const float* slope, float* mask, bool gen,
                      float inv_keep, float p, unsigned long long seed, float* post, hipStream_t s);
 int cnet_act_bn_backward(const float* gy, GemmFold src, const float* pre, const float* xhat, const float* invstd,
                          const float* gamma, const float* slope, const float* mask, float inv_keep, int R, int n, int training,
-                         float* gx, float* ggamma, float* gbeta, float* gslope, hipStream_t s);
+                         float* gx, float* ggamma, float* gbeta, float* gslope, hipStream_t s, float* amax = nullptr);
 bool cnet_heads_fused_eligible(int nf, int nc);
 int cnet_heads_forward(const float* x, int R, int nf, const float* Wb, const float* bb, const float* Wc, const float* bc, int nc,
                        float* bbox_out, float* logits, float* lsm, float* cls_out, hipStream_t s);
@@ -261,7 +261,7 @@
   float* gslope = nullptr;
 };
 int cnet_heads_backward(const float* g_bbox, const float* g_cls, const float* lsm, int R, int nf, const float* Wb, const float* Wc,
-                        int nc, float* glog, float* gfeat, hipStream_t s, const HeadsPostAct* post = nullptr);
+                        int nc, float* glog, float* gfeat, hipStream_t s, const HeadsPostAct* post = nullptr, float* amax = nullptr);
 int log_softmax_rows_fold(const float* x, GemmFold src, int R, int n, float* y, float* y2, hipStream_t s);
 int dropout_mask(float* mask, long n, float p, unsigned long long seed, hipStream_t s);
 struct DropoutJobs { float* ptr[8]; int C[8]; float p[8]; unsigned long long seed[8]; int n; };
diff --git a/faster-rcnn.torch_amd/csrc/net.cpp b/faster-rcnn.torch_amd/csrc/net.cpp
--- a/faster-rcnn.torch_amd/csrc/net.cpp
+++ b/faster-rcnn.torch_amd/csrc/net.cpp
@@ -66,7 +66,10 @@
   DevBuf am;
   const float* am_w_of = nullptr;
   long am_w_gen = -1;
+  const float* rx = nullptr;
+  bool x_live = false, g_live = false;
 };
+#define CLS_AM_RECS 4
 
 }
 
@@ -175,10 +178,15 @@
   int R = 0, D = 0;
   const float* cnet_x = nullptr;
   DevBuf feat_g, logits, lsm, glog, gtmp;
+  DevBuf xrec[2];
+  int xrec_w = 0;
+  const float* xrec_of = nullptr;
+  long xrec_n = 0;
   std::vector<std::array<long long, 4>> table;
 };
 
 static int pool_out(int n) { return (n - 2 + 1) / 2 + 1; }
+static bool gemm_f16_on();
 static int refresh_group(frcnn_model* m, const float* w, int group, hipStream_t s);
 
 static void build_layout(frcnn_model* m) {
@@ -1045,10 +1053,39 @@
       *ptr = m->rec(id); *bytes = (long long)AMAX_REC * 4;
       return FRCNN_OK;
     }
+    case 15: {
+      FR_CHECK(index >= 0 && index < (int)m->cls.size() && m->R > 0, "debug_buffer: classification layer %d (after frcnn_cnet_backward)", index);
+      const ClsLayer& L = m->cls[index]; b = &L.g; n = (size_t)m->R * L.n * 4;
+    } break;
+    case 12: case 13: {
+      FR_CHECK(index >= 0 && index < (int)m->cls.size() && m->R > 0, "debug_buffer: classification layer %d (after frcnn_cnet_forward)", index);
+      const ClsLayer& L = m->cls[index];
+      const bool live = kind == 12 ? L.x_live : L.g_live;
+      FR_CHECK(live, "debug_buffer: the last pass kept no magnitude record of kind %d, index %d", kind, index);
+      *ptr = kind == 12 ? const_cast<float*>(L.rx) : L.am.f() + AMAX_REC;
+      *bytes = (long long)AMAX_REC * 4;
+      return FRCNN_OK;
+    }
     default: FR_CHECK(false, "debug_buffer: unknown kind %d", kind);
   }
   FR_CHECK(b->p && b->bytes >= n, "debug_buffer: buffer not allocated yet");
   *ptr = b->p; *bytes = (long long)n;
+  return FRCNN_OK;
+}
+
+int frcnn_model_roi_pool_forward(frcnn_model* m, const float* fmap, int C, int H, int W, const int* wins, int R, int kh, int kw,
+                                 float* out, int* idx, void* stream) {
+  FR_CHECK(m, "frcnn_model_roi_pool_forward: NULL model");
+  m->xrec_of = nullptr;
+  float* rec = nullptr;
+  if (!m->cls.empty() && gemm_f16_on() && R > 0 && linear_x_eligible(1, R, m->cls[0].in, m->cls[0].n) &&
+      (long)C * kh * kw == m->cls[0].in) {
+    FR_TRY(m->xrec[m->xrec_w].ensure((size_t)AMAX_REC * 4));
+    rec = m->xrec[m->xrec_w].f();
+  }
+  bool kept = false;
+  FR_TRY(roi_pool_forward(fmap, C, H, W, wins, R, kh, kw, out, idx, S(stream), rec, &kept));
+  if (kept) { m->xrec_of = out; m->xrec_n = (long)R * C * kh * kw; }
   return FRCNN_OK;
 }
 
@@ -1613,7 +1650,7 @@
     if (L.x_form & 1) FR_TRY(L.xp.ensure((size_t)3 * R * L.in * 2));
     if (L.x_form & 2) FR_TRY(L.gp.ensure((size_t)3 * R * L.n * 2));
     if (L.x_form & 4) { FR_TRY(L.xpT.ensure((size_t)3 * L.in * Rp * 2)); FR_TRY(L.gpT.ensure((size_t)3 * L.n * Rp * 2)); }
-    if (L.x_form & 7) FR_TRY(L.am.ensure((size_t)5 * AMAX_REC * 4));
+    if (L.x_form & 7) FR_TRY(L.am.ensure((size_t)CLS_AM_RECS * AMAX_REC * 4));
   }
   int nc = m->d.class_count + 1;
   int nf = m->cls.empty() ? m->D : m->cls.back().n;
@@ -1622,6 +1659,11 @@
   FR_TRY(m->lsm.ensure((size_t)R * nc * 4));
   FR_TRY(m->glog.ensure((size_t)R * nc * 4));
   return FRCNN_OK;
+}
+
+static bool cls_wgrad_f16() {
+  static const bool on = env_flag("FRCNN_GEMM_WGRAD_F16", true);
+  return on;
 }
 
 int frcnn_cnet_forward(frcnn_model* m, const float* weights, const float* x, int R, int training,
@@ -1635,10 +1677,14 @@
   const float* w = weights;
   const float* cur = x;
   float* bnr = bn_running;
+  const float* x_from_pool = (m->xrec_of && m->xrec_of == x && !m->cls.empty() && m->xrec_n == (long)R * m->cls[0].in) ? m->xrec[m->xrec_w].f() : nullptr;
+  m->xrec_of = nullptr;
   for (size_t l = 0; l < m->cls.size(); ++l) {
     ClsLayer& L = m->cls[l];
     GemmFold fold;
     GemmFold* defer = cnet_fuse() ? &fold : nullptr;
+    L.x_live = L.g_live = false;
+    L.rx = nullptr;
     if ((L.x_form & 3) && gemm_f16_on()) {
       float* rw = L.am.f() + 2 * AMAX_REC;
       const bool have = !training && g_static_weights && L.am_w_gen == g_static_gen && L.am_w_of == w;
@@ -1648,10 +1694,17 @@
       L.am_w_of = nullptr;
     }
     if ((L.x_form & 1) && gemm_f16_on()) {
-      float* rx = L.am.f();
-      FR_TRY(tensor_absmax(cur, (long)R * L.in, rx, s));
+      const float* rx = L.am.f();
+      if (l == 0 && x_from_pool) {
+        rx = x_from_pool;
+        m->xrec_w ^= 1;
+        L.x_live = true;
+      } else {
+        FR_TRY(tensor_absmax(cur, (long)R * L.in, L.am.f(), s));
+      }
+      L.rx = rx;
       FR_TRY(split_planes(cur, R, L.in, L.xp.p, nullptr, s, rx));
-      FR_TRY(linear_x_forward(L.xp.p, R, L.in, w + L.w_off, w + L.b_off, L.n, L.lin.f(), s, 0, defer, rx, rx + 2 * AMAX_REC));
+      FR_TRY(linear_x_forward(L.xp.p, R, L.in, w + L.w_off, w + L.b_off, L.n, L.lin.f(), s, 0, defer, rx, L.am.f() + 2 * AMAX_REC));
     } else if (L.x_form & 1) {
       FR_TRY(split_planes(cur, R, L.in, L.xp.p, nullptr, s));
       FR_TRY(linear_x_forward(L.xp.p, R, L.in, w + L.w_off, w + L.b_off, L.n, L.lin.f(), s, 0, defer));
@@ -1721,6 +1774,15 @@
   const int nc = m->d.class_count + 1;
   const float* feat = m->cls.empty() ? m->cnet_x : m->cls.back().post.f();
   if (m->frozen_blocks >= (int)m->blocks.size()) gx = nullptr;
+  auto g_rec = [&](ClsLayer& L, int l) -> float* {
+    L.g_live = false;
+    if (!gemm_f16_on() || L.am.bytes < (size_t)CLS_AM_RECS * AMAX_REC * 4) return nullptr;
+    const bool xd = (L.x_form & 2) != 0 && (l > 0 || gx) && L.am_w_of == weights;
+    const bool xw = (L.x_form & 4) != 0 && cls_wgrad_f16();
+    if (!xd && !xw) return nullptr;
+    L.g_live = true;
+    return L.am.f() + AMAX_REC;
+  };
   FR_TRY(cw_join(m, s));
   const bool async = g_cnet_wgrad_async && !deterministic();
   if (async) FR_TRY(ensure_update_stream(m));
@@ -1743,7 +1805,7 @@
       top_act_done = true;
     }
     FR_TRY(cnet_heads_backward(g_bbox, g_cls, m->lsm.f(), R, nf, w + m->bbox_w_off, w + m->clsw_off, nc, m->glog.f(), dst, s,
-                               top_act_done ? &post : nullptr));
+                               top_act_done ? &post : nullptr, top_act_done ? g_rec(m->cls.back(), (int)m->cls.size() - 1) : nullptr));
     FR_TRY(fork());
   } else {
     FR_TRY(log_softmax_backward(g_cls, m->lsm.f(), R, nc, m->glog.f(), s));
@@ -1761,17 +1823,18 @@
     ClsLayer& L = m->cls[l];
     const float* pre = L.bn ? L.pre.f() : L.lin.f();
     const bool drop = m->training && L.p_drop > 0.f;
+    float* const rg = (top_act_done && l == (int)m->cls.size() - 1) ? (L.g_live ? L.am.f() + AMAX_REC : nullptr) : g_rec(L, l);
     if (top_act_done && l == (int)m->cls.size() - 1) {
     } else if (L.bn && cnet_fuse()) {
       FR_TRY(cnet_act_bn_backward(g, gfold, pre, L.xhat.f(), L.invstd.f(), w + L.bnw_off, w + L.a_off, drop ? L.mask.f() : nullptr,
                                   drop ? 1.0f / (1.0f - L.p_drop) : 1.f, R, L.n, m->training, L.g.f(), grad + L.bnw_off,
-                                  grad + L.bnb_off, grad + L.a_off, s));
+                                  grad + L.bnb_off, grad + L.a_off, s, rg));
     } else {
       FR_TRY(prelu_dropout_backward(g, pre, (long)R * L.n, w + L.a_off, drop ? L.mask.f() : nullptr,
-                                    drop ? 1.0f / (1.0f - L.p_drop) : 1.f, L.g.f(), grad + L.a_off, s));
+                                    drop ? 1.0f / (1.0f - L.p_drop) : 1.f, L.g.f(), grad + L.a_off, s, L.bn ? nullptr : rg));
       if (L.bn)
         FR_TRY(bn_backward(L.g.f(), L.xhat.f(), L.invstd.f(), w + L.bnw_off, R, L.n, m->training, L.g.f(),
-                           grad + L.bnw_off, grad + L.bnb_off, s));
+                           grad + L.bnw_off, grad + L.bnb_off, s, rg));
     }
     gfold = GemmFold{};
     GemmFold* gdefer = (cnet_fuse() && async && l > 0 && m->cls[l - 1].bn) ? &gfold : nullptr;
@@ -1779,9 +1842,7 @@
     const float* in = l == 0 ? m->cnet_x : m->cls[l - 1].post.f();
     float* gin = l == 0 ? gx : L.gin.f();
     const bool xw = (L.x_form & 4) != 0, xd = (L.x_form & 2) != 0 && gin;
-    if (xd && gemm_f16_on() && L.am_w_of == w) {
-      float* rg = L.am.f() + AMAX_REC;
-      FR_TRY(tensor_absmax(L.g.f(), (long)R * L.n, rg, s));
+    if (xd && rg && L.am_w_of == w) {
       FR_TRY(split_planes(L.g.f(), R, L.n, L.gp.p, nullptr, s, rg));
       FR_TRY(linear_x_dgrad(L.gp.p, R, L.n, w + L.w_off, L.in, gin, OUT_STORE, s, 0, gdefer, rg, L.am.f() + 2 * AMAX_REC));
     } else if (xd) {
@@ -1790,12 +1851,14 @@
     } else if (gin) {
       FR_TRY(gemm_f32(L.g.f(), L.n, 1, w + L.w_off, L.in, 1, gin, L.in, R, L.in, L.n, OUT_STORE, nullptr, s, 0, gdefer));
     }
-    static const bool wgrad_f16 = env_flag("FRCNN_GEMM_WGRAD_F16", true);
-    if (xw && wgrad_f16 && gemm_f16_on() && L.am.bytes >= (size_t)5 * AMAX_REC * 4) {
-      float *rgT = L.am.f() + 3 * AMAX_REC, *rxT = L.am.f() + 4 * AMAX_REC;
-      FR_TRY(tensor_absmax(L.g.f(), (long)R * L.n, rgT, ws));
-      if ((L.x_form & 1) && L.am_w_of == w) rxT = L.am.f();
-      else FR_TRY(tensor_absmax(in, (long)R * L.in, rxT, ws));
+    if (xw && rg && cls_wgrad_f16()) {
+      const float* rgT = rg;
+      const float* rxT = L.rx;
+      if (!((L.x_form & 1) && L.am_w_of == w && rxT)) {
+        float* own = L.am.f() + 3 * AMAX_REC;
+        FR_TRY(tensor_absmax(in, (long)R * L.in, own, ws));
+        rxT = own;
+      }
       FR_TRY(split_planes(L.g.f(), R, L.n, nullptr, L.gpT.p, ws, rgT));
       FR_TRY(split_planes(in, R, L.in, nullptr, L.xpT.p, ws, rxT));
       FR_TRY(linear_x_wgrad(L.gpT.p, L.xpT.p, R, L.n, L.in, grad + L.w_off, ws, wslot, rgT, rxT));
diff --git a/faster-rcnn.torch_amd/csrc/roi.hip b/faster-rcnn.torch_amd/csrc/roi.hip
--- a/faster-rcnn.torch_amd/csrc/roi.hip
+++ b/faster-rcnn.torch_amd/csrc/roi.hip
@@ -1,4 +1,5 @@
 #include "kernels.h"
+#include "amax.h"
 #include "roi_fix.h"
 
 namespace frcnn {
@@ -32,12 +33,10 @@
   }
 }
 
-__global__ __launch_bounds__(256) void roi_pool_forward_cells_kernel(const float* __restrict__ fmap, int C, int H, int W,
-                                                                     const int* __restrict__ wins, int kh, int kw,
-                                                                     float* __restrict__ out, int* __restrict__ idx) {
-  const int r = blockIdx.x, cells = kh * kw, groups = blockDim.x / cells;
-  const int tid = threadIdx.x;
-  if (tid >= groups * cells) return;
+template <bool REC>
+__device__ __forceinline__ void roi_pool_cells_body(const float* __restrict__ fmap, int C, int H, int W, const int* __restrict__ wins,
+                                                    int kh, int kw, float* __restrict__ out, int* __restrict__ idx, int r, int cells,
+                                                    int groups, int tid, float& am) {
   const int cg = tid / cells, cell = tid - cg * cells;
   const int i = cell / kw, j = cell - i * kw;
   const int* wn = wins + 4 * r;
@@ -66,6 +65,7 @@
       const size_t t = ((size_t)r * C + c) * cells + cell;
       out[t] = best;
       if (idx) idx[t] = bi;
+      if (REC) am = fmaxf(am, fabsf(best));
     }
     return;
   }
@@ -81,18 +81,39 @@
     const size_t t = ((size_t)r * C + c) * cells + cell;
     out[t] = best;
     if (idx) idx[t] = bi;
-  }
+    if (REC) am = fmaxf(am, fabsf(best));
+  }
+}
+template <bool REC>
+__global__ __launch_bounds__(256) void roi_pool_forward_cells_kernel(const float* __restrict__ fmap, int C, int H, int W,
+                                                                     const int* __restrict__ wins, int kh, int kw,
+                                                                     float* __restrict__ out, int* __restrict__ idx,
+                                                                     float* __restrict__ rec) {
+  const int r = blockIdx.x, cells = kh * kw, groups = blockDim.x / cells;
+  const int tid = threadIdx.x;
+  const bool live = tid < groups * cells;
+  if (!REC && !live) return;
+  float am = 0.f;
+  if (live) roi_pool_cells_body<REC>(fmap, C, H, W, wins, kh, kw, out, idx, r, cells, groups, tid, am);
+  if (REC) amax_store_block_flat(am, rec, tid, blockDim.x, blockIdx.y * gridDim.x + blockIdx.x, gridDim.x * gridDim.y);
 }
 
 int roi_pool_forward(const float* fmap, int C, int H, int W, const int* wins, int R, int kh, int kw,
-                     float* out, int* idx, hipStream_t s) {
+                     float* out, int* idx, hipStream_t s, float* rec, bool* kept) {
+  if (kept) *kept = false;
   if (R <= 0) return FRCNN_OK;
   long total = (long)R * C * kh * kw;
   if (kh * kw <= 256) {
     const int groups = 256 / (kh * kw);
     const int slices = std::max(1, std::min(cdiv(C, groups), (int)cdivl(4096, R)));
-    FR_LAUNCH(KC_ROI, 0, total * 8.0, s, roi_pool_forward_cells_kernel, dim3(R, slices), dim3(256), 0, fmap, C, H, W,
-              wins, kh, kw, out, idx);
+    if (rec && (long)R * slices <= AMAX_MAX_BLOCKS) {
+      FR_LAUNCH(KC_ROI, 0, total * 8.0, s, roi_pool_forward_cells_kernel<true>, dim3(R, slices), dim3(256), 0, fmap, C, H, W,
+                wins, kh, kw, out, idx, rec);
+      if (kept) *kept = true;
+    } else {
+      FR_LAUNCH(KC_ROI, 0, total * 8.0, s, roi_pool_forward_cells_kernel<false>, dim3(R, slices), dim3(256), 0, fmap, C, H, W,
+                wins, kh, kw, out, idx, (float*)nullptr);
+    }
     FR_LAUNCH_CHECK();
     return FRCNN_OK;
   }
diff --git a/faster-rcnn.torch_amd/objective.py b/faster-rcnn.torch_amd/objective.py
--- a/faster-rcnn.torch_amd/objective.py
+++ b/faster-rcnn.torch_amd/objective.py
@@ -448,7 +448,7 @@
                               kh, kw, sampling, ptr(cinput), s)
                 else:
                     pidx = scratch.get("pidx", (E, D), np.int32)
-                    _lib.call("frcnn_roi_pool_forward", ptr(fm), fmC, fmH, fmW, C.c_void_p(d_wins), E, kh, kw,
+                    _lib.call("frcnn_model_roi_pool_forward", native.h, ptr(fm), fmC, fmH, fmW, C.c_void_p(d_wins), E, kh, kw,
                               ptr(cinput), ptr(pidx), s)
                 coutputs = cnet.forward(cinput)
                 crout, ccout = coutputs
diff --git a/include/frcnn_hip.h b/include/frcnn_hip.h
--- a/include/frcnn_hip.h
+++ b/include/frcnn_hip.h
@@ -130,6 +130,8 @@
 
 int frcnn_roi_pool_forward(const float *fmap, int C, int H, int W, const int *wins, int R, int kh,
                            int kw, float *out, int *idx, void *stream);
+int frcnn_roi_pool_forward_rec(const float *fmap, int C, int H, int W, const int *wins, int R, int kh,
+                               int kw, float *out, int *idx, void *stream, int *kept_host, float *rec);
 int frcnn_roi_pool_backward(float *gmap, int C, int H, int W, const float *gout, const int *idx,
                             int R, int kh, int kw, void *stream);
 
@@ -240,6 +242,8 @@
 int frcnn_pnet_output(frcnn_model *, int i, float **ptr_host, int *C_host, int *H_host,
                       int *W_host);
 int frcnn_model_debug_buffer(frcnn_model *, int kind, int index, void **ptr_host, long long *bytes_host);
+int frcnn_model_roi_pool_forward(frcnn_model *, const float *fmap, int C, int H, int W, const int *wins,
+                                 int R, int kh, int kw, float *out, int *idx, void *stream);
 int frcnn_pnet_delta(frcnn_model *, int i, float **ptr_host);
 int frcnn_pnet_zero_deltas(frcnn_model *, void *stream);
 int frcnn_pnet_set_sparse_deltas(frcnn_model *, int head, const int *positions, int count);
```

Measured after the change: 525.5, median of 3. About the same (+0.3%).
